# automl/TransformersCanDoBayesianInference

Hardware: AMD Instinct MI355X
Metric: synthetic datasets/sec (GP prior, bptt=2000) (higher is better)
Workload: dtype fp16; 1 GPU; priors.fast_gp, bptt=2000, num_features=18, emsize=512, nhead=4, nhid=1024, nlayers=6, 1000 bars (BASELINE.json configs[1]); per_gpu_batch=64, global_batch=64, aggregate_k_gradients=1, aggregate_streams=0, aggregate_stacked=False, seq_len=2000, parallelism=dp1, micro_batch_streams=2, eval_pos=weighted sampler(2000)

## Files before the change

include/pfn_hip.h:

```cpp
#ifndef PFN_HIP_H
#define PFN_HIP_H

#include <stddef.h>
#include <stdint.h>

#ifdef __cplusplus
extern "C" {
#endif

#define PFN_ABI_VERSION 10

enum {
  PFN_OK = 0,
  PFN_ERR_UNSUPPORTED = -1,
  PFN_ERR_ALIGNMENT = -2,
  PFN_ERR_LAUNCH = -3,
  PFN_ERR_ARGUMENT = -4,
};

enum { PFN_PREC_BF16 = 0,
       PFN_PREC_F32 = 1,
       PFN_PREC_FP16 = 2   };

typedef struct pfn_model_desc {
  int32_t num_features;
  int32_t emsize;
  int32_t nhead;
  int32_t nhid;
  int32_t nlayers;
  int32_t n_out;
  int32_t precision;
  float ln_eps;
  float dropout;
  int32_t schedule;
} pfn_model_desc;
enum { PFN_SCHED_TOP_LAYER_ALL_ROWS = 1,
       PFN_SCHED_FUSE_LN_WIDE = 2,
       PFN_SCHED_SEPARATE_LNBWD = 4,
       PFN_SCHED_NO_KEY_CENTERING = 16,
       PFN_SCHED_KEY_CENTERING = 64,
       PFN_SCHED_F32_RESIDUAL = 128,
       PFN_SCHED_FUSE_Q_PROJECTION = 32,
       PFN_SCHED_DETERMINISTIC = 8        };
int pfn_default_schedule(void);

int pfn_abi_version(void);
const char* pfn_last_error_string(void);
enum { PFN_TUNE_GEMM_NT_KERNEL = 0,
       PFN_TUNE_GEMM_TN_WRAP = 1,
       PFN_TUNE_FUSE_LNBWD = 2,
       PFN_TUNE_ATTN_PINGPONG = 4,
       PFN_TUNE_FUSE_LN_WIDE = 5,
       PFN_TUNE_GP_PLANES = 8,
       PFN_TUNE_FUSE_DELTA = 9,
       PFN_TUNE_GEMM_LN_ROWS = 7,
       PFN_TUNE_ATTN_BWD_GROUP = 10,
       PFN_TUNE_WGRAD_SPLITS = 11,
       PFN_TUNE_WGRAD_WAVES = 14,
       PFN_TUNE_LOSS_SCALE_TARGET = 15,
       PFN_TUNE_RESIDUAL16 = 16,
       PFN_TUNE_FUSE_Q_PROJECTION = 12,
       PFN_TUNE_KEY_CENTERING = 13,
       PFN_TUNE_ATTN_CACHE_SPLITS = 17,
       PFN_TUNE_TOP_LAYER_TEST_ROWS = 6  };
int pfn_set_tuning(int key, int value);
enum { PFN_PROF_ATTN_FWD = 0, PFN_PROF_ATTN_BWD_DELTA = 2, PFN_PROF_ATTN_BWD_KV = 4, PFN_PROF_ATTN_BWD_DQ = 6, PFN_PROF_GEMM_QKV = 8,
       PFN_PROF_GEMM_OUT_LN = 10, PFN_PROF_GEMM_LIN1 = 12, PFN_PROF_GEMM_LIN2_LN = 14, PFN_PROF_GEMM_DHPRE = 16, PFN_PROF_GEMM_DY1 = 18,
       PFN_PROF_GEMM_DCTX = 20, PFN_PROF_GEMM_DX = 22, PFN_PROF_WGRAD = 24, PFN_PROF_SLOTS = 26 };
int pfn_profile_enable(int on);
int pfn_profile_read(int slot, double* total_ms, int64_t* launches);

int pfn_param_layout(const pfn_model_desc* d, int64_t* offsets, int64_t* numels, int max_tensors);
int64_t pfn_param_count(const pfn_model_desc* d);
int64_t pfn_shadow_bytes(const pfn_model_desc* d);
int pfn_prepare_params(const pfn_model_desc* d, const float* params, void* shadow, void* stream);

int64_t pfn_workspace_bytes(const pfn_model_desc* d, int B, int S);
int64_t pfn_top_layer_rows(const pfn_model_desc* d, int B, int S, int sep, int use_dropout);
int pfn_stack_forward(const pfn_model_desc* d, const float* params, const void* shadow,
                      const float* x, int64_t x_st, int64_t x_sb,
                      const float* y, int64_t y_st, int64_t y_sb,
                      const float* src_sbe,
                      int B, int S, int sep,
                      void* workspace, int64_t workspace_bytes,
                      float* logits, void* stream);
int pfn_stack_forward_dropout(const pfn_model_desc* d, const float* params, const void* shadow,
                              const float* x, int64_t x_st, int64_t x_sb,
                              const float* y, int64_t y_st, int64_t y_sb,
                              const float* src_sbe,
                              int B, int S, int sep,
                              void* workspace, int64_t workspace_bytes,
                              float* logits, void* stream, uint64_t dropout_seed);
int pfn_stack_backward(const pfn_model_desc* d, const float* params, const void* shadow,
                       const float* x, int64_t x_st, int64_t x_sb,
                       const float* y, int64_t y_st, int64_t y_sb,
                       int B, int S, int sep,
                       void* workspace, int64_t workspace_bytes,
                       const float* dlogits, float* grads, float* dsrc_sbe, void* stream);
typedef void (*pfn_host_callback)(void* user);
int pfn_stack_backward_split(const pfn_model_desc* d, const float* params, const void* shadow,
                             const float* x, int64_t x_st, int64_t x_sb,
                             const float* y, int64_t y_st, int64_t y_sb,
                             int B, int S, int sep,
                             void* workspace, int64_t workspace_bytes,
                             const float* dlogits, float* grads, float* dsrc_sbe, void* stream,
                             int first_group_layers, pfn_host_callback on_first_group, void* user,
                             int use_dropout, uint64_t dropout_seed);

int pfn_stack_forward_ragged(const pfn_model_desc* d, const float* params, const void* shadow,
                             const float* x, int64_t x_st, int64_t x_sb,
                             const float* y, int64_t y_st, int64_t y_sb,
                             int B, int S, const int32_t* sep_of, const int64_t* row_off, int sep_min, int sep_max, int64_t test_rows,
                             void* workspace, int64_t workspace_bytes, float* logits, void* stream,
                             int use_dropout, uint64_t dropout_seed);
int pfn_stack_backward_ragged(const pfn_model_desc* d, const float* params, const void* shadow,
                              const float* x, int64_t x_st, int64_t x_sb,
                              const float* y, int64_t y_st, int64_t y_sb,
                              int B, int S, const int32_t* sep_of, const int64_t* row_off, int sep_min, int sep_max, int64_t test_rows,
                              void* workspace, int64_t workspace_bytes,
                              const float* dlogits, float* grads, void* stream,
                              int first_group_layers, pfn_host_callback on_first_group, void* user,
                              int use_dropout, uint64_t dropout_seed);

int64_t pfn_context_bytes(const pfn_model_desc* d, int B, int sep);
int pfn_stack_condition(const pfn_model_desc* d, const float* params, const void* shadow,
                        const float* x, int64_t x_st, int64_t x_sb,
                        const float* y, int64_t y_st, int64_t y_sb,
                        int B, int sep,
                        void* workspace, int64_t workspace_bytes,
                        void* context, int64_t context_bytes, void* stream);
int64_t pfn_predict_workspace_bytes(const pfn_model_desc* d, int B, int n);
int pfn_stack_predict(const pfn_model_desc* d, const float* params, const void* shadow,
                      const void* context, int64_t context_bytes, int sep,
                      const float* x, int64_t x_st, int64_t x_sb,
                      int B, int n,
                      void* workspace, int64_t workspace_bytes, float* logits, void* stream);

int64_t pfn_predict_grad_workspace_bytes(const pfn_model_desc* d, int B, int n);
int pfn_stack_predict_saved(const pfn_model_desc* d, const float* params, const void* shadow,
                            const void* context, int64_t context_bytes, int sep,
                            const float* x, int64_t x_st, int64_t x_sb,
                            int B, int n,
                            void* workspace, int64_t workspace_bytes, float* logits, void* stream);
int pfn_stack_predict_backward(const pfn_model_desc* d, const float* params, const void* shadow,
                               const void* context, int64_t context_bytes, int sep, int B, int n,
                               void* workspace, int64_t workspace_bytes, const float* dlogits,
                               float* dx, int64_t dx_st, int64_t dx_sb, void* stream);
int pfn_stack_input_grads(const pfn_model_desc* d, const float* params, int B, int S, int sep,
                          const void* workspace, int64_t workspace_bytes,
                          float* dx, int64_t dx_st, int64_t dx_sb, float* dy, int64_t dy_st, int64_t dy_sb, void* stream);

int pfn_stack_condition_ragged(const pfn_model_desc* d, const float* params, const void* shadow,
                               const float* x, int64_t x_st, int64_t x_sb,
                               const float* y, int64_t y_st, int64_t y_sb,
                               int B, int sep_max, const int32_t* sep_of,
                               void* workspace, int64_t workspace_bytes,
                               void* context, int64_t context_bytes, void* stream);
int pfn_stack_predict_ragged(const pfn_model_desc* d, const float* params, const void* shadow,
                             const void* context, int64_t context_bytes, int sep_max, const int32_t* sep_of,
                             const float* x, int64_t x_st, int64_t x_sb,
                             int B, int n,
                             void* workspace, int64_t workspace_bytes, float* logits, void* stream);
int pfn_stack_predict_saved_ragged(const pfn_model_desc* d, const float* params, const void* shadow,
                                   const void* context, int64_t context_bytes, int sep_max, const int32_t* sep_of,
                                   const float* x, int64_t x_st, int64_t x_sb,
                                   int B, int n,
                                   void* workspace, int64_t workspace_bytes, float* logits, void* stream);
int pfn_stack_predict_backward_ragged(const pfn_model_desc* d, const float* params, const void* shadow,
                                      const void* context, int64_t context_bytes, int sep_max, const int32_t* sep_of, int B, int n,
                                      void* workspace, int64_t workspace_bytes, const float* dlogits,
                                      float* dx, int64_t dx_st, int64_t dx_sb, void* stream);

int pfn_bar_nll_forward(const float* logits, int64_t ld, const float* y, const float* borders,
                        int64_t R, int nbars, int full_support,
                        float* nll, float* lse, int32_t* bucket, void* stream);
int pfn_bar_nll_backward(const float* logits, int64_t ld, const float* lse, const int32_t* bucket,
                         const float* gout, int64_t R, int nbars, float* dlogits, void* stream);
int pfn_bar_mean(const float* logits, int64_t ld, const float* borders, int64_t R, int nbars,
                 int full_support, float* mean, void* stream);
int pfn_bar_mean_backward(const float* logits, int64_t ld, const float* borders, int64_t R, int nbars, int full_support,
                          const float* mean, const float* gout, float* dlogits, void* stream);

#define PFN_BAR_STATS_MAX 16
#define PFN_BAR_STAT_MEAN 0
#define PFN_BAR_STAT_VARIANCE 1
#define PFN_BAR_STAT_MODE 2
#define PFN_BAR_STAT_CDF 3
#define PFN_BAR_STAT_ICDF 4
#define PFN_BAR_STAT_EI_MAX 5
#define PFN_BAR_STAT_EI_MIN 6
int pfn_bar_stats(const float* logits, int64_t ld, const float* borders, int64_t R, int nbars, int full_support,
                  const int32_t* kinds, int K, const float* args, int64_t arg_ld, float* out, void* stream);
int pfn_bar_stats_backward(const float* logits, int64_t ld, const float* borders, int64_t R, int nbars, int full_support,
                           const int32_t* kinds, int K, const float* args, int64_t arg_ld, const float* out, const float* gout,
                           float* dlogits, void* stream);
int pfn_bar_sample(const float* logits, int64_t ld, const float* borders, int64_t R, int nbars, int full_support,
                   int n_samples, uint64_t seed, float* out, void* stream);

int pfn_clip_adam_step(float* params, float* grads, float* exp_avg, float* exp_avg_sq, int64_t n,
                       float lr, float beta1, float beta2, float eps, float max_norm,
                       float grad_scale, int step, int zero_grad, float* scratch, void* stream);

int64_t pfn_gp_workspace_bytes(int B, int S);
int pfn_gp_prior_sample(float* x, float* z, float* y, float* K_ws, int64_t K_ws_bytes,
                        const float* lengthscale, const float* outputscale, const float* noise,
                        int B, int S, int nf, int kernel, int gen_x, int gen_z,
                        uint64_t seed, uint64_t offset, int32_t* info, void* stream);

int pfn_gp_posterior(const float* x, const float* y, float* K_ws, int64_t K_ws_bytes, float* resid_ws, float* w_ws,
                     const float* lengthscale, const float* outputscale, const float* noise,
                     int B, int S, int nf, int kernel, float* nll, float* mean, float* var,
                     int32_t* info, void* stream);

int64_t pfn_gp_fit_workspace_bytes(int P, int S);
int pfn_gp_mll_grad(const float* x, const float* y, const int32_t* n_of, const float* theta, const float* prior,
                    int P, int S, int nf, int kernel, int flags, void* ws, int64_t ws_bytes,
                    float* value, float* grad, int32_t* info, void* stream);
int pfn_gp_fit_predict(const float* x, const float* y, const int32_t* n_of, const float* theta, const float* prior,
                       int P, int S, int nf, int kernel, const float* x_test, int m, void* ws, int64_t ws_bytes,
                       float* mean, float* var, int32_t* info, void* stream);

#define PFN_NUTS_ADAPT_MASS 1
#define PFN_NUTS_KEEP_WARMUP 2
#define PFN_NUTS_MAX_WINDOWS 16
#define PFN_NUTS_INV_MASS_OFFSET 256
int64_t pfn_nuts_workspace_bytes(int C, int D, int max_tree_depth);
int pfn_nuts_init(void* ws, int64_t ws_bytes, int C, int D, int64_t ld, int max_tree_depth, int num_warmup, int num_samples, int flags,
                  const int32_t* window_ends, int n_windows, int window_start, float step_size, float target_accept, uint64_t seed,
                  const int64_t* chain_ids, const float* theta0, const float* inv_mass0, float* trial, int32_t* done_count, void* stream);
int pfn_nuts_advance(void* ws, int64_t ws_bytes, int C, int D, int64_t ld, int max_tree_depth, int num_warmup, int num_samples,
                     const float* value, const float* grad, const int32_t* info, const float* scale, const float* shift, float* trial,
                     float* samples, float* stats, float* warm, int32_t* done_count, void* stream);

int pfn_bnn_logp_grad(const float* x, const float* y, const int32_t* n_of, const float* theta, int64_t ld,
                      int P, int K, int S, int F, int H, int activation,
                      float* value, float* grad, void* stream);
int pfn_bnn_predict(const float* x_test, const float* theta, int64_t ld, int P, int K, int m, int F, int H, int activation,
                    float* prob1, void* stream);

int pfn_bnn_svi_steps(const float* x, const float* y, const int32_t* n_of, float* state, int64_t ld, int P, int S, int F, int H, int activation,
                      int num_particles, int64_t step0, int num_steps, float lr, float beta1, float beta2, float eps, uint64_t seed,
                      const int64_t* problem_ids, float* loss, void* stream);

#define PFN_BNN_SVGD_MAX_PARTICLES 64
int64_t pfn_bnn_svgd_workspace_bytes(int P, int num_particles, int F, int H);
int pfn_bnn_svgd_steps(const float* x, const float* y, const int32_t* n_of, float* state, int64_t ld, int P, int S, int F, int H, int activation,
                       int num_particles, int64_t step0, int num_steps, float lr, float beta1, float beta2, float eps, float bandwidth_factor,
                       void* workspace, int64_t workspace_bytes, float* potential, float* bandwidth, void* stream);

#define PFN_TAB_NORM_WITH_TEST 0
#define PFN_TAB_NORM_TRAIN_ONLY 1
int pfn_tabular_windows(const float* X, const float* y, const int32_t* starts, int64_t N, int F, int F_out, int W, int bptt, int sep, float rescale, int mode,
                        float* x_out, float* y_out, void* stream);
int pfn_auc_counts(const float* scores, const float* labels, int T, int C, int64_t* counts, void* stream);
int pfn_knn_cv(const float* train, const float* labels, const float* test, const int32_t* fold, int P, int n, int T, int F,
               int32_t* cv_correct, int32_t* test_pos, int32_t* test_nbr, void* stream);

int pfn_mlp_prior_forward(const float* weights, const float* biases, const int32_t* model_of, const int32_t* dims,
                          const float* noise_std, float* causes, const float* noise, float* y, float* hidden,
                          int B, int T, int HP, int Lmax, int activation, int gen_causes,
                          uint64_t seed, uint64_t offset, void* stream);

int pfn_op_gemm_nt(const void* A, int64_t lda, const void* B, int64_t ldb, int M, int N, int K,
                   int flags, const float* bias, const void* aux, int64_t ld_aux,
                   const float* resid, int64_t ld_resid, float* out_f32, int64_t ld_out_f32,
                   void* out_t, int64_t ld_out_t, void* out2_t, int64_t ld_out2, int prec, void* stream);
int pfn_op_gemm_tn(const void* A, int64_t lda, const void* B, int64_t ldb, float* C, int64_t ldc,
                   int M, int P, int Q, int atomic, int prec, void* stream);
int pfn_op_gemm_tn_group(int n, const void* const* A, const int64_t* lda, const void* const* B, const int64_t* ldb,
                         float* const* C, const int64_t* ldc, const int32_t* P, const int32_t* Q,
                         float* const* colsum, int M, int splits, int prec, void* stream);
#define PFN_OP_SUMS_16BIT 256
int pfn_op_gemm_ln(const void* A, int64_t lda, const void* B, int64_t ldb, int M, int N, int K, const float* bias,
                   const float* resid, const float* ry, const float* rmean, const float* rrstd,
                   const float* rgamma, const float* rbeta, const float* gamma, const float* beta, float eps,
                   float* y, float* mean, float* rstd, void* x_t, int prec, void* stream);
int pfn_op_gemm_lnbwd(const void* A, int64_t lda, const void* B, int64_t ldb, int M, int N, int K, const void* aux,
                      const float* y, const float* mean, const float* rstd, const float* gamma,
                      void* dx_t, float* dgamma, float* dbeta, int prec, void* stream);
int pfn_op_attention_fwd(const void* qkv, void* ctx, float* lse, int B, int S, int E, int H, int sep,
                         int prec, void* stream);
int64_t pfn_op_attention_bwd_ws_bytes(int B, int S, int H, int prec);
int pfn_op_attention_bwd(const void* qkv, const void* ctx, const float* lse, const void* dctx,
                         void* dqkv, float* delta_ws, void* ds_ws, int B, int S, int E, int H, int sep,
                         int prec, int parts, void* stream);
int pfn_op_attention_fwd_from(const void* qkv, void* ctx, float* lse, int B, int S, int E, int H, int sep, int q_begin,
                              int prec, void* stream);
int pfn_op_attention_bwd_from(const void* qkv, const void* ctx, const float* lse, const void* dctx,
                              void* dqkv, float* delta_ws, void* ds_ws, int B, int S, int E, int H, int sep, int q_begin,
                              int prec, int parts, void* stream);
int pfn_op_gather_rows(const void* src_bs, void* dst_tb, int B, int S, int64_t row_bytes, int sep, void* stream);
int pfn_op_scatter_rows(const void* src_tb, void* dst_bs, int B, int S, int64_t row_bytes, int sep, int zero_from, void* stream);
int pfn_op_layernorm_fwd(const float* x, const float* gamma, const float* beta, float* y_f32, void* y_t,
                         float* mean, float* rstd, int64_t rows, int E, float eps, int prec, void* stream);
int pfn_op_layernorm_bwd(const void* dy, int dy_is_t, const float* x, const float* gamma, const float* mean,
                         const float* rstd, float* dx_f32, void* dx_t, float* dgamma, float* dbeta,
                         float* dbias_extra, int64_t rows, int E, int prec, void* stream);
int pfn_op_cast(const float* src, void* dst, int64_t n, int prec, void* stream);
int pfn_op_qkv_projection(const void* x_t, const void* w_in_t, const float* b_in, void* qkv_t, float* kshift_ws,
                          int B, int S, int E, int sep, const int32_t* sep_of, int center, int prec, void* stream);

#ifdef __cplusplus
}
// ... 3 lines not shown
```

transformerscandobayesianinference_amd/_hip.py:

```python
import ctypes
import os
import subprocess

import torch

_HERE = os.path.dirname(os.path.abspath(__file__))
LIB_PATH = os.path.join(_HERE, 'libpfn_hip.so')
ABI_VERSION = 10

MAX_FEATURES = 1022
PREC_BF16 = 0
PREC_F32 = 1
PREC_FP16 = 2
PRECISIONS = {'bf16': PREC_BF16, 'f32': PREC_F32, 'fp32': PREC_F32, 'fp16': PREC_FP16, 'f16': PREC_FP16}
SCHED_TOP_LAYER_ALL_ROWS, SCHED_FUSE_LN_WIDE, SCHED_SEPARATE_LNBWD, SCHED_DETERMINISTIC, SCHED_NO_KEY_CENTERING, SCHED_FUSE_Q_PROJECTION, SCHED_KEY_CENTERING, SCHED_F32_RESIDUAL = 1, 2, 4, 8, 16, 32, 64, 128
NUTS_ADAPT_MASS, NUTS_KEEP_WARMUP, NUTS_MAX_WINDOWS, NUTS_INV_MASS_OFFSET = 1, 2, 16, 256

EPI_BIAS, EPI_GELU, EPI_GELU_BWD, EPI_RESID, EPI_OUT_F32, EPI_OUT_T, EPI_OUT2_T, EPI_ACCUM, EPI_RESID_T = 1, 2, 4, 8, 16, 32, 64, 128, 256


class HipExtensionError(RuntimeError):
    pass


class ModelDesc(ctypes.Structure):
    _fields_ = [('num_features', ctypes.c_int32), ('emsize', ctypes.c_int32), ('nhead', ctypes.c_int32),
                ('nhid', ctypes.c_int32), ('nlayers', ctypes.c_int32), ('n_out', ctypes.c_int32),
                ('precision', ctypes.c_int32), ('ln_eps', ctypes.c_float), ('dropout', ctypes.c_float), ('schedule', ctypes.c_int32)]

    def key(self):
        return (self.num_features, self.emsize, self.nhead, self.nhid, self.nlayers, self.n_out, self.precision, self.ln_eps, self.dropout, self.schedule)


HOST_CALLBACK = ctypes.CFUNCTYPE(None, ctypes.c_void_p)

_lib = None

_c = ctypes
_P, _I, _L, _F, _U64 = _c.c_void_p, _c.c_int, _c.c_int64, _c.c_float, _c.c_uint64
_D = _c.POINTER(ModelDesc)

SIGNATURES = {
    'pfn_abi_version': (_I, []),
    'pfn_last_error_string': (_c.c_char_p, []),
    'pfn_set_tuning': (_I, [_I, _I]),
    'pfn_default_schedule': (_I, []),
    'pfn_profile_enable': (_I, [_I]),
    'pfn_profile_read': (_I, [_I, _c.POINTER(_c.c_double), _c.POINTER(_L)]),
    'pfn_param_layout': (_I, [_D, _c.POINTER(_L), _c.POINTER(_L), _I]),
    'pfn_param_count': (_L, [_D]),
    'pfn_shadow_bytes': (_L, [_D]),
    'pfn_prepare_params': (_I, [_D, _P, _P, _P]),
    'pfn_workspace_bytes': (_L, [_D, _I, _I]),
    'pfn_top_layer_rows': (_L, [_D, _I, _I, _I, _I]),
    'pfn_stack_forward': (_I, [_D, _P, _P, _P, _L, _L, _P, _L, _L, _P, _I, _I, _I, _P, _L, _P, _P]),
    'pfn_stack_backward': (_I, [_D, _P, _P, _P, _L, _L, _P, _L, _L, _I, _I, _I, _P, _L, _P, _P, _P, _P]),
    'pfn_stack_forward_dropout': (_I, [_D, _P, _P, _P, _L, _L, _P, _L, _L, _P, _I, _I, _I, _P, _L, _P, _P, _U64]),
    'pfn_stack_backward_split': (_I, [_D, _P, _P, _P, _L, _L, _P, _L, _L, _I, _I, _I, _P, _L, _P, _P, _P, _P, _I, _P, _P, _I, _U64]),
    'pfn_stack_forward_ragged': (_I, [_D, _P, _P, _P, _L, _L, _P, _L, _L, _I, _I, _P, _P, _I, _I, _L, _P, _L, _P, _P, _I, _U64]),
    'pfn_stack_backward_ragged': (_I, [_D, _P, _P, _P, _L, _L, _P, _L, _L, _I, _I, _P, _P, _I, _I, _L, _P, _L, _P, _P, _P, _I, _P, _P, _I, _U64]),
    'pfn_context_bytes': (_L, [_D, _I, _I]),
    'pfn_stack_condition': (_I, [_D, _P, _P, _P, _L, _L, _P, _L, _L, _I, _I, _P, _L, _P, _L, _P]),
    'pfn_predict_workspace_bytes': (_L, [_D, _I, _I]),
    'pfn_stack_predict': (_I, [_D, _P, _P, _P, _L, _I, _P, _L, _L, _I, _I, _P, _L, _P, _P]),
    'pfn_predict_grad_workspace_bytes': (_L, [_D, _I, _I]),
    'pfn_stack_predict_saved': (_I, [_D, _P, _P, _P, _L, _I, _P, _L, _L, _I, _I, _P, _L, _P, _P]),
    'pfn_stack_predict_backward': (_I, [_D, _P, _P, _P, _L, _I, _I, _I, _P, _L, _P, _P, _L, _L, _P]),
    'pfn_stack_condition_ragged': (_I, [_D, _P, _P, _P, _L, _L, _P, _L, _L, _I, _I, _P, _P, _L, _P, _L, _P]),
    'pfn_stack_predict_ragged': (_I, [_D, _P, _P, _P, _L, _I, _P, _P, _L, _L, _I, _I, _P, _L, _P, _P]),
    'pfn_stack_predict_saved_ragged': (_I, [_D, _P, _P, _P, _L, _I, _P, _P, _L, _L, _I, _I, _P, _L, _P, _P]),
    'pfn_stack_predict_backward_ragged': (_I, [_D, _P, _P, _P, _L, _I, _P, _I, _I, _P, _L, _P, _P, _L, _L, _P]),
    'pfn_stack_input_grads': (_I, [_D, _P, _I, _I, _I, _P, _L, _P, _L, _L, _P, _L, _L, _P]),
    'pfn_bar_nll_forward': (_I, [_P, _L, _P, _P, _L, _I, _I, _P, _P, _P, _P]),
    'pfn_bar_nll_backward': (_I, [_P, _L, _P, _P, _P, _L, _I, _P, _P]),
    'pfn_bar_mean': (_I, [_P, _L, _P, _L, _I, _I, _P, _P]),
    'pfn_bar_mean_backward': (_I, [_P, _L, _P, _L, _I, _I, _P, _P, _P, _P]),
    'pfn_bar_stats': (_I, [_P, _L, _P, _L, _I, _I, _P, _I, _P, _L, _P, _P]),
    'pfn_bar_stats_backward': (_I, [_P, _L, _P, _L, _I, _I, _P, _I, _P, _L, _P, _P, _P, _P]),
    'pfn_bar_sample': (_I, [_P, _L, _P, _L, _I, _I, _I, _U64, _P, _P]),
    'pfn_clip_adam_step': (_I, [_P, _P, _P, _P, _L, _F, _F, _F, _F, _F, _F, _I, _I, _P, _P]),
    'pfn_gp_workspace_bytes': (_L, [_I, _I]),
    'pfn_gp_prior_sample': (_I, [_P, _P, _P, _P, _L, _P, _P, _P, _I, _I, _I, _I, _I, _I, _U64, _U64, _P, _P]),
    'pfn_gp_posterior': (_I, [_P, _P, _P, _L, _P, _P, _P, _P, _P, _I, _I, _I, _I, _P, _P, _P, _P, _P]),
    'pfn_gp_fit_workspace_bytes': (_L, [_I, _I]),
    'pfn_gp_mll_grad': (_I, [_P, _P, _P, _P, _P, _I, _I, _I, _I, _I, _P, _L, _P, _P, _P, _P]),
    'pfn_gp_fit_predict': (_I, [_P, _P, _P, _P, _P, _I, _I, _I, _I, _P, _I, _P, _L, _P, _P, _P, _P]),
    'pfn_nuts_workspace_bytes': (_L, [_I, _I, _I]),
    'pfn_nuts_init': (_I, [_P, _L, _I, _I, _L, _I, _I, _I, _I, _P, _I, _I, _F, _F, _U64, _P, _P, _P, _P, _P, _P]),
    'pfn_nuts_advance': (_I, [_P, _L, _I, _I, _L, _I, _I, _I, _P, _P, _P, _P, _P, _P, _P, _P, _P, _P, _P]),
    'pfn_bnn_logp_grad': (_I, [_P, _P, _P, _P, _L, _I, _I, _I, _I, _I, _I, _P, _P, _P]),
    'pfn_bnn_predict': (_I, [_P, _P, _L, _I, _I, _I, _I, _I, _I, _P, _P]),
    'pfn_bnn_svi_steps': (_I, [_P, _P, _P, _P, _L, _I, _I, _I, _I, _I, _I, _L, _I, _F, _F, _F, _F, _U64, _P, _P, _P]),
    'pfn_bnn_svgd_workspace_bytes': (_L, [_I, _I, _I, _I]),
    'pfn_bnn_svgd_steps': (_I, [_P, _P, _P, _P, _L, _I, _I, _I, _I, _I, _I, _L, _I, _F, _F, _F, _F, _F, _P, _L, _P, _P, _P]),
    'pfn_tabular_windows': (_I, [_P, _P, _P, _L, _I, _I, _I, _I, _I, _F, _I, _P, _P, _P]),
    'pfn_auc_counts': (_I, [_P, _P, _I, _I, _P, _P]),
    'pfn_knn_cv': (_I, [_P, _P, _P, _P, _I, _I, _I, _I, _P, _P, _P, _P]),
    'pfn_mlp_prior_forward': (_I, [_P, _P, _P, _P, _P, _P, _P, _P, _P, _I, _I, _I, _I, _I, _I, _U64, _U64, _P]),
    'pfn_op_gemm_nt': (_I, [_P, _L, _P, _L, _I, _I, _I, _I, _P, _P, _L, _P, _L, _P, _L, _P, _L, _P, _L, _I, _P]),
    'pfn_op_gemm_tn': (_I, [_P, _L, _P, _L, _P, _L, _I, _I, _I, _I, _I, _P]),
    'pfn_op_gemm_tn_group': (_I, [_I, _P, _P, _P, _P, _P, _P, _P, _P, _P, _I, _I, _I, _P]),
    'pfn_op_gemm_ln': (_I, [_P, _L, _P, _L, _I, _I, _I, _P, _P, _P, _P, _P, _P, _P, _P, _P, _F, _P, _P, _P, _P, _I, _P]),
    'pfn_op_gemm_lnbwd': (_I, [_P, _L, _P, _L, _I, _I, _I, _P, _P, _P, _P, _P, _P, _P, _P, _I, _P]),
    'pfn_op_attention_fwd': (_I, [_P, _P, _P, _I, _I, _I, _I, _I, _I, _P]),
    'pfn_op_attention_bwd_ws_bytes': (_L, [_I, _I, _I, _I]),
    'pfn_op_attention_fwd_from': (_I, [_P, _P, _P, _I, _I, _I, _I, _I, _I, _I, _P]),
    'pfn_op_attention_bwd_from': (_I, [_P, _P, _P, _P, _P, _P, _P, _I, _I, _I, _I, _I, _I, _I, _I, _P]),
    'pfn_op_gather_rows': (_I, [_P, _P, _I, _I, _L, _I, _P]),
    'pfn_op_scatter_rows': (_I, [_P, _P, _I, _I, _L, _I, _I, _P]),
    'pfn_op_attention_bwd': (_I, [_P, _P, _P, _P, _P, _P, _P, _I, _I, _I, _I, _I, _I, _I, _P]),
    'pfn_op_layernorm_fwd': (_I, [_P, _P, _P, _P, _P, _P, _P, _L, _I, _F, _I, _P]),
    'pfn_op_layernorm_bwd': (_I, [_P, _I, _P, _P, _P, _P, _P, _P, _P, _P, _P, _L, _I, _I, _P]),
    'pfn_op_cast': (_I, [_P, _P, _L, _I, _P]),
    'pfn_op_qkv_projection': (_I, [_P, _P, _P, _P, _P, _I, _I, _I, _I, _P, _I, _I, _P]),
}


def build(verbose=False):
    script = os.path.join(_HERE, 'csrc', 'build.sh')
    res = subprocess.run(['bash', script], capture_output=True, text=True)
    if res.returncode != 0 or not os.path.exists(LIB_PATH):
        raise HipExtensionError('building libpfn_hip.so failed:\n' + res.stdout[-4000:] + res.stderr[-8000:])
    if verbose:
        print(res.stdout[-2000:])
    return LIB_PATH


def lib():
    global _lib
    if _lib is None:
        if not os.path.exists(LIB_PATH):
            raise HipExtensionError(
                f'{LIB_PATH} not found. Build it with `python -c "import __graft_entry__ as g; g.build()"` '
                f'(or transformerscandobayesianinference_amd/csrc/build.sh). There is no CPU / PyTorch fallback for the hot path.')
        handle = ctypes.CDLL(LIB_PATH)
        for name, (res, args) in SIGNATURES.items():
            try:
                fn = getattr(handle, name)
            except AttributeError as e:
                raise HipExtensionError(f'libpfn_hip.so does not export {name}') from e
            fn.restype = res
            fn.argtypes = args
        if handle.pfn_abi_version() != ABI_VERSION:
            raise HipExtensionError(f'libpfn_hip.so ABI {handle.pfn_abi_version()} != binding ABI {ABI_VERSION}; rebuild')
        _lib = handle
    return _lib


def check(rc, what):
    if rc < 0:
        msg = lib().pfn_last_error_string()
        raise HipExtensionError(f'{what} failed with code {rc}: {msg.decode() if msg else ""}')
    return rc


def stream_ptr(device=None):
    return torch.cuda.current_stream(device).cuda_stream


def ptr(t):
    return 0 if t is None else t.data_ptr()


def require_gpu_tensor(t, name):
    if not t.is_cuda:
        raise HipExtensionError(
            f'{name} lives on {t.device}: the PFN hot path only runs on an MI355X through libpfn_hip.so; '
            f'move the model and data to a cuda device (there is no CPU fallback in the product path).')
```

transformerscandobayesianinference_amd/csrc/gemm_tn.hip:

```cpp
#include <type_traits>
#include "pfn_device.h"
#include "pfn_kernels.h"

namespace pfn {

PFN_DEV int xcd_remap(int bid, int nwg) {
  const int q = nwg >> 3, r = nwg & 7, xcd = bid & 7;
  return (xcd < r ? xcd * (q + 1) : r * (q + 1) + (xcd - r) * q) + (bid >> 3);
}
typedef __attribute__((address_space(1))) const void gvoid_t;
typedef __attribute__((address_space(3))) void lvoid_t;

constexpr int TN_BMK = 32;

template <typename T>
__global__ __launch_bounds__(256, 2) void gemm_tn_kernel(GemmTN g) {
  constexpr int RB = 128 * sizeof(T);
  constexpr int TILE = TN_BMK * RB;
  extern __shared__ __attribute__((aligned(16))) char smem_raw[];
  LdsPtr smem = lds_cast(smem_raw);
  auto tileA = [&](int buf) { return smem + buf * 2 * TILE; };
  auto tileB = [&](int buf) { return smem + buf * 2 * TILE + TILE; };

  const int p0 = blockIdx.y * 128, q0 = blockIdx.x * 128;
// ... 243 lines not shown
        }
      }
      slot_next = slot;
      slot = slot + 1 == TNB_NS ? 0 : slot + 1;
    }
  };
  if (do_colsum) main_loop(std::true_type{});
  else main_loop(std::false_type{});

  const int pv = pr.Pv > 0 ? pr.Pv : pr.P;
  const float osc = loss_scale_down(g.scale_amax);
  if (do_colsum && (lane & 31) == 0) {
#pragma unroll
    for (int r = 0; r < 16; ++r) {
      const int pp = p0 + wp * 128 + wq * 32 + acc_row(r, lane);
      if (pp < pv) unsafeAtomicAdd(pr.colsum + pp, cs[r] * osc);
    }
  }
  const bool atomic = true;
#pragma unroll
  for (int i = 0; i < 4; ++i)
#pragma unroll
    for (int j = 0; j < 2; ++j)
#pragma unroll
      for (int r = 0; r < 16; ++r) {
        const int pp = p0 + wp * 128 + i * 32 + acc_row(r, lane);
        const int qq = q0 + wq * 64 + j * 32 + (lane & 31);
        float* c = pr.C + (long)pp * pr.ldc + qq;
        if (pp >= pv) continue;
        if (atomic) unsafeAtomicAdd(c, acc[i][j][r] * osc);
        else *c += acc[i][j][r] * osc;
      }
}

#define PFN_TNW_BUILT (PFN_TNB_KT == 64 && PFN_TNB_NS == 2)
#if PFN_TNW_BUILT
constexpr int TNW_NW = 4;
template <typename T>
__global__ __launch_bounds__(TNW_NW * 64, 1) void gemm_tn_wide_kernel(GemmTNGroup g) {
  extern __shared__ __attribute__((aligned(16))) char smem_raw[];
  LdsPtr smem = lds_cast(smem_raw);
  const int ntiles = g.tile_start[g.n];
  const int id = xcd_remap(blockIdx.x, ntiles * g.splits);
  const int split = id / ntiles, tile = id % ntiles;
  int pi = 0;
  while (tile >= g.tile_start[pi + 1]) ++pi;
  const TnProblem& pr = g.p[pi];
  const int tq = pr.Q / 256;
  const int tl = tile - g.tile_start[pi];
  const int p0 = (tl / tq) * 256, q0 = (tl % tq) * 256;
  const long mbeg = (long)split * g.m_chunk;
  const long mend = min((long)g.M, mbeg + g.m_chunk);
  const int rows_total = (int)(mend - mbeg);
  if (rows_total <= 0) return;
  const int wave = __builtin_amdgcn_readfirstlane(threadIdx.x >> 6), lane = threadIdx.x & 63;
  const int wp = wave >> 1, wq = wave & 1;

  TnStager<TNW_NW> stg;
  stg.init(pr, mbeg, rows_total, p0, q0, wave, lane, g.debug_mask);

  f32x16 acc[4][4];
#pragma unroll
  for (int i = 0; i < 4; ++i)
#pragma unroll
    for (int j = 0; j < 4; ++j)
#pragma unroll
      for (int r = 0; r < 16; ++r) acc[i][j][r] = 0.f;
  float cs[2] = {0.f, 0.f};
  const bool do_colsum = pr.colsum != nullptr && q0 == 0;

  const int nt = (rows_total + TNB_KT - 1) / TNB_KT;
  struct Frs { Frag<T> a[4], b[4]; };
  auto main_loop = [&](auto with_colsum) {
    constexpr bool CS = decltype(with_colsum)::value;
    Frs f0, f1;
    auto ld = [&](Frs& f, const lds_char* ta, const lds_char* tb, int ks) {
#pragma unroll
      for (int j = 0; j < 4; ++j) f.b[j] = load_frag_tr<T, 512, 1>(tb, ks, wq * 128 + j * 32);
#pragma unroll
      for (int i = 0; i < 4; ++i) f.a[i] = load_frag_tr<T, 512, 1>(ta, ks, wp * 128 + i * 32);
    };
    auto mm = [&](const Frs& f) {
#pragma unroll
      for (int i = 0; i < 4; ++i)
#pragma unroll
        for (int j = 0; j < 4; ++j) acc[i][j] = mma32(f.a[i], f.b[j], acc[i][j]);
      if constexpr (CS) {
#pragma unroll
        for (int c = 0; c < 2; ++c)
#pragma unroll
          for (int e = 0; e < 8; ++e) cs[c] += (float)(wq ? f.a[2 + c] : f.a[c]).v[e];
      }
    };
    auto enter_stage = [&](int t, int slot) {
      wait_vm_barrier<0>();
      if (t + 1 < nt) stg.issue(smem + (slot ^ 1) * 2 * TNB_TILE);
    };
    int slot = 0;
    enter_stage(0, slot);
    ld(f0, smem, smem + TNB_TILE, 0);
    for (int t = 0; t < nt; ++t) {
      const lds_char* ta = smem + slot * 2 * TNB_TILE;
      const lds_char* tb = ta + TNB_TILE;
      ld(f1, ta, tb, 16);
      PFN_PIN_LDS_MFMA();
      mm(f0);
      PFN_PIN_LDS_MFMA();
      ld(f0, ta, tb, 32);
      PFN_PIN_LDS_MFMA();
      mm(f1);
      PFN_PIN_LDS_MFMA();
      ld(f1, ta, tb, 48);
      PFN_PIN_LDS_MFMA();
      mm(f0);
      PFN_PIN_LDS_MFMA();
      slot ^= 1;
      if (t + 1 < nt) {
        enter_stage(t + 1, slot);
        const lds_char* tan = smem + slot * 2 * TNB_TILE;
        ld(f0, tan, tan + TNB_TILE, 0);
      }
      PFN_PIN_LDS_MFMA();
      mm(f1);
      PFN_PIN_LDS_MFMA();
    }
  };
  stg.issue(smem);
  if (do_colsum) main_loop(std::true_type{});
  else main_loop(std::false_type{});

  const int pv = pr.Pv > 0 ? pr.Pv : pr.P;
  const float osc = loss_scale_down(g.scale_amax);
  if (do_colsum) {
#pragma unroll
    for (int c = 0; c < 2; ++c) {
      const float s = cs[c] + __shfl_xor(cs[c], 32, 64);
      const int pp = p0 + wp * 128 + (2 * wq + c) * 32 + (lane & 31);
      if (lane < 32 && pp < pv) unsafeAtomicAdd(pr.colsum + pp, s * osc);
    }
  }
#pragma unroll
  for (int i = 0; i < 4; ++i)
#pragma unroll
    for (int j = 0; j < 4; ++j)
#pragma unroll
      for (int r = 0; r < 16; ++r) {
        const int pp = p0 + wp * 128 + i * 32 + acc_row(r, lane);
        const int qq = q0 + wq * 128 + j * 32 + (lane & 31);
        if (pp < pv) unsafeAtomicAdd(pr.C + (long)pp * pr.ldc + qq, acc[i][j][r] * osc);
      }
}
#endif

static bool aligned16(const void* p) { return (reinterpret_cast<uintptr_t>(p) & 15) == 0; }

static int g_tn_debug_wrap = 0;
void set_gemm_tn_debug_wrap(int rows) { g_tn_debug_wrap = rows; }
static int g_tn_group_splits = 0;
void set_gemm_tn_group_splits(int splits) { g_tn_group_splits = splits; }
static bool g_tn_wide = false;
void set_gemm_tn_group_waves(int waves) { g_tn_wide = waves == 4; }

int launch_gemm_tn(GemmTN g, int precision, hipStream_t stream) {
  if (g.M <= 0 || g.P <= 0 || g.Q <= 0) return PFN_OK;
  const size_t es = prec_esize(precision);
  if ((g.lda * es) % 16 || (g.ldb * es) % 16 || !aligned16(g.A) || !aligned16(g.B)) return PFN_ERR_ALIGNMENT;
  const int tp = (g.P + 127) / 128, tq = (g.Q + 127) / 128;
  int splits = (1024 + tp * tq - 1) / (tp * tq);
  const int max_splits = (g.M + 4 * TN_BMK - 1) / (4 * TN_BMK);
  if (splits > max_splits) splits = max_splits;
  if (g.max_splits > 0 && splits > g.max_splits) splits = g.max_splits;
  if (splits < 1) splits = 1;
  if (!g.atomic) splits = 1;
  int chunk = (g.M + splits - 1) / splits;
  chunk = (chunk + TN_BMK - 1) / TN_BMK * TN_BMK;
  splits = (g.M + chunk - 1) / chunk;
  g.m_chunk = chunk;
  const size_t lds = 4 * TN_BMK * 128 * es;
  PFN_DISPATCH_OP(precision, hipLaunchKernelGGL(gemm_tn_kernel<T>, dim3(tq, tp, splits), dim3(256), lds, stream, g));
  return hipGetLastError() == hipSuccess ? PFN_OK : PFN_ERR_LAUNCH;
}

bool gemm_tn_group_supported(const TnProblem& p) {
  return p.P % 256 == 0 && p.Q % 256 == 0 && (p.lda * 2) % 16 == 0 && (p.ldb * 2) % 16 == 0 && aligned16(p.A) && aligned16(p.B);
}

int launch_gemm_tn_group(GemmTNGroup g, int precision, hipStream_t stream) {
  if (g.n <= 0 || g.M <= 0) return PFN_OK;
  if (g.n > TN_GROUP_MAX) return PFN_ERR_ARGUMENT;
  if (!prec_is16(precision)) return PFN_ERR_UNSUPPORTED;
  int tiles = 0;
  for (int i = 0; i < g.n; ++i) {
    if (!gemm_tn_group_supported(g.p[i])) return PFN_ERR_UNSUPPORTED;
    g.tile_start[i] = tiles;
    tiles += (g.p[i].P / 256) * (g.p[i].Q / 256);
  }
  g.tile_start[g.n] = tiles;
  int splits = g.splits;
  if (splits <= 0 && g_tn_group_splits > 0) splits = g_tn_group_splits;
  if (splits <= 0) {
    splits = 8;
    for (int sp = 1; sp <= 8; ++sp) {
      const int blocks = tiles * sp, rounds = (blocks + 255) / 256;
      if (blocks >= 0.9 * rounds * 256) { splits = sp; break; }
    }
  }
  const int max_splits = (g.M + 4 * TNB_KT - 1) / (4 * TNB_KT);
  if (splits > max_splits) splits = max_splits;
  int chunk = (g.M + splits - 1) / splits;
  chunk = (chunk + TNB_KT - 1) / TNB_KT * TNB_KT;
  splits = (g.M + chunk - 1) / chunk;
  g.splits = splits;
  g.m_chunk = chunk;
  for (int i = 0; i < g.n; ++i) {
    const TnProblem& p = g.p[i];
    if (p.lda < 256 || p.ldb < 256 || (long)chunk * p.lda * 2 > TN_GROUP_MAX_SPLIT_BYTES || (long)chunk * p.ldb * 2 > TN_GROUP_MAX_SPLIT_BYTES) return PFN_ERR_UNSUPPORTED;
  }
  const int wrap = g_tn_debug_wrap;
  g.debug_mask = wrap >= TNB_KT && (wrap & (wrap - 1)) == 0 ? wrap - 1 : 0x7fffffff;
  if (g_tn_wide) {
#if PFN_TNW_BUILT
    static LdsAllowance allow_w[2];
    if (precision == PFN_PREC_FP16) {
      allow_w[1].ensure(gemm_tn_wide_kernel<f16>, TNB_LDS);
      hipLaunchKernelGGL(gemm_tn_wide_kernel<f16>, dim3(tiles * splits), dim3(TNW_NW * 64), TNB_LDS, stream, g);
    } else {
      allow_w[0].ensure(gemm_tn_wide_kernel<bf16>, TNB_LDS);
      hipLaunchKernelGGL(gemm_tn_wide_kernel<bf16>, dim3(tiles * splits), dim3(TNW_NW * 64), TNB_LDS, stream, g);
    }
    return hipGetLastError() == hipSuccess ? PFN_OK : PFN_ERR_LAUNCH;
#else
    return PFN_ERR_UNSUPPORTED;
#endif
  }
  static LdsAllowance allowance[2];
  if (precision == PFN_PREC_FP16) {
    allowance[1].ensure(gemm_tn_big_kernel<f16>, TNB_LDS);
    hipLaunchKernelGGL(gemm_tn_big_kernel<f16>, dim3(tiles * splits), dim3(512), TNB_LDS, stream, g);
  } else {
    allowance[0].ensure(gemm_tn_big_kernel<bf16>, TNB_LDS);
    hipLaunchKernelGGL(gemm_tn_big_kernel<bf16>, dim3(tiles * splits), dim3(512), TNB_LDS, stream, g);
  }
  return hipGetLastError() == hipSuccess ? PFN_OK : PFN_ERR_LAUNCH;
}

}
```

transformerscandobayesianinference_amd/csrc/pfn_api.hip:

```cpp
#include <algorithm>
#include <cstdarg>
#include <cstdio>
#include <cstring>
#include <mutex>
#include <vector>
#include "pfn_kernels.h"

using namespace pfn;

namespace pfn {
namespace {
struct ProfPair { hipEvent_t a, b; };
std::mutex g_prof_mu;
std::vector<ProfPair> g_prof[PFN_PROF_SLOTS];
std::atomic<int> g_prof_on{0};
}
bool prof_enabled() { return g_prof_on.load(std::memory_order_relaxed) != 0; }
void* prof_begin(int slot, hipStream_t s) {
  const int on = g_prof_on.load(std::memory_order_relaxed);
  if (!on || slot < 0 || slot >= PFN_PROF_SLOTS) return nullptr;
  if (on >= 2 && (slot & ~1) != on - 2) return nullptr;
  ProfPair* p = new ProfPair;
  if (hipEventCreate(&p->a) != hipSuccess || hipEventCreate(&p->b) != hipSuccess) { delete p; return nullptr; }
  (void)hipEventRecord(p->a, s);
// ... 338 lines not shown
    g.x_f32 = last ? u.x2 : nullptr;
    PFN_TRY(launch_gemm_ln(g, prec, s));
    res = Resid{nullptr, u.y2, u.mean2, u.rstd2, params + p.g2, params + p.be2};
  } else {
    {
      GemmNT g = nt(u.h, F, W(m, p.w2), F, rows, E, F, EPI_BIAS | (pdrop > 0.f ? 0 : EPI_RESID) | EPI_OUT_F32);
      g.bias = params + p.b2; g.resid = u.x1; g.ld_resid = E; g.out_f32 = u.y2; g.ld_out_f32 = E;
      if (y16u) { g.flags = EPI_BIAS | EPI_RESID_T | EPI_OUT_T; g.aux = u.x1_t; g.ld_aux = E; g.out_t = u.y2; g.ld_out_t = E; }
      PFN_TRY(launch_gemm_nt(g, prec, s));
      if (pdrop > 0.f) PFN_TRY(launch_dropout_add(u.y2, u.x1, rows, E, seed[3], pdrop, s));
    }
    PFN_TRY(launch_layernorm_fwd(u.y2, params + p.g2, params + p.be2, (y16u && !last) ? nullptr : u.x2, u.x2_t, u.mean2, u.rstd2, rows, E, d.ln_eps, prec, s, y16u));
  }
  return PFN_OK;
}

int decoder_forward(const Model& m, const void* xt_t, char* dt, char* dpre, float* logits, int rows) {
  const int prec = m.d->precision, E = m.d->emsize, F = m.d->nhid, O = m.d->n_out;
  {
    GemmNT g = nt(xt_t, E, W(m, m.L->dec0_w), E, rows, F, E, EPI_BIAS | EPI_GELU | EPI_OUT_T | EPI_OUT2_T);
    g.bias = m.params + m.L->dec0_b; g.out_t = dt; g.ld_out_t = F; g.out2_t = dpre; g.ld_out2 = F;
    PFN_TRY(launch_gemm_nt(g, prec, m.s));
  }
  GemmNT g = nt(dt, F, W(m, m.L->dec2_w), F, rows, O, F, EPI_BIAS | EPI_OUT_F32);
  g.bias = m.params + m.L->dec2_b; g.out_f32 = logits; g.ld_out_f32 = O;
  return launch_gemm_nt(g, prec, m.s);
}
int decoder_backward_data(const Model& m, const void* dlog_t, const void* dpre, char* dd_t, float* dxt, int rows) {
  const int prec = m.d->precision, E = m.d->emsize, F = m.d->nhid, O = m.d->n_out, npad = m.L->n_out_pad;
  {
    GemmNT g = nt(dlog_t, npad, WT(m, m.L->dec2_wt), npad, rows, F, npad % 64 == 0 ? npad : O, EPI_GELU_BWD | EPI_OUT_T);
    g.aux = dpre; g.ld_aux = F; g.out_t = dd_t; g.ld_out_t = F;
    PFN_TRY(launch_gemm_nt(g, prec, m.s));
  }
  GemmNT g = nt(dd_t, F, WT(m, m.L->dec0_wt), F, rows, E, F, EPI_OUT_F32);
  g.out_f32 = dxt; g.ld_out_f32 = E;
  return launch_gemm_nt(g, prec, m.s);
}

bool tn_set_groupable(const std::vector<TnProblem>& probs, int prec) {
  bool grouped = prec_is16(prec);
  for (const TnProblem& t : probs) grouped = grouped && gemm_tn_group_supported(t);
  return grouped;
}
int launch_tn_set(const std::vector<TnProblem>& probs, int rows, int prec, bool det, const float* lsc, int prof_slot, hipStream_t s, bool allow_group = true) {
  auto one_by_one = [&](size_t i0, size_t n) {
    for (size_t i = i0; i < i0 + n; ++i) {
      const TnProblem& t = probs[i];
      GemmTN g = tn(t.A, t.lda, t.B, t.ldb, t.C, t.ldc, rows, t.Pv ? t.Pv : t.P, t.Q, t.colsum);
      if (det) g.max_splits = 1;
      g.scale_amax = lsc;
      PFN_TRY(launch_gemm_tn(g, prec, s));
    }
    return (int)PFN_OK;
  };
  if (!(allow_group && tn_set_groupable(probs, prec))) return one_by_one(0, probs.size());
  for (size_t i0 = 0; i0 < probs.size(); i0 += TN_GROUP_MAX) {
    ProfScope ps(prof_slot, s);
    GemmTNGroup g;
    memset(&g, 0, sizeof(g));
    g.n = (int)std::min<size_t>(TN_GROUP_MAX, probs.size() - i0);
    g.M = rows;
    g.splits = det ? 1 : 0;
    g.scale_amax = lsc;
    for (int i = 0; i < g.n; ++i) g.p[i] = probs[i0 + i];
    const int rc = launch_gemm_tn_group(g, prec, s);
    if (rc == PFN_ERR_UNSUPPORTED) PFN_TRY(one_by_one(i0, g.n));
    else PFN_TRY(rc);
  }
  return PFN_OK;
}

struct LnSinks { float *dgamma, *dbeta, *dbias; };
struct LayerGrads {
  const void* dout; int dout_is_t;
  const void* y2; const float *mean2, *rstd2, *gamma2; const void* y1; const float *mean1, *rstd1, *gamma1; const void* hpre;
  char *dy2_t, *dy2m_t, *dh_t, *dy1_t, *dqkv_t, *dx1_t;
  LnSinks ln2, ln1;
  float* ln_part;
};
GemmLNB lnb(const Model& m, const Plan& pl, const float* lsc, const void* A, long lda, const void* Bw, long ldb, int K, const void* aux, const void* y,
            const float* mean, const float* rstd, const float* gamma, void* dx_t, const LnSinks& sink, int rows) {
  GemmLNB g; memset(&g, 0, sizeof(g));
  g.A = A; g.lda = lda; g.B = Bw; g.ldb = ldb; g.M = rows; g.N = m.d->emsize; g.K = K; g.aux = aux;
  g.y = y; g.mean = mean; g.rstd = rstd; g.gamma = gamma; g.dx_t = dx_t; g.dgamma = sink.dgamma; g.dbeta = sink.dbeta; g.scale_amax = lsc; g.y16 = pl.y16_any;
  return g;
}
GemmLNB lnb_dy1(const Model& m, const Plan& pl, const float* lsc, const LayerP& t, const LayerGrads& g, int rows) {
  const int F = m.d->nhid;
  return lnb(m, pl, lsc, g.dh_t, F, WT(m, t.w1), F, F, g.dy2_t, g.y1, g.mean1, g.rstd1, g.gamma1, g.dy1_t, g.ln1, rows);
}
GemmLNB lnb_dx(const Model& m, const Plan& pl, const float* lsc, const LayerP& t, const char* dqkv_t, const char* dy1_t, const LayerGrads& below, int rows) {
  const int E = m.d->emsize;
  return lnb(m, pl, lsc, dqkv_t, 3 * E, WT(m, t.w_in), 3 * E, 3 * E, dy1_t, below.y2, below.mean2, below.rstd2, below.gamma2, below.dy2_t, below.ln2, rows);
}
bool lnbwd_fusable(const Model& m, const Plan& pl, const float* lsc, const LayerGrads& g0, int rows) {
  const LayerP& t = m.L->layer_t[0];
  return pl.lnb_eligible && gemm_lnbwd_supported(lnb_dy1(m, pl, lsc, t, g0, rows)) && gemm_lnbwd_supported(lnb_dx(m, pl, lsc, t, g0.dqkv_t, g0.dy1_t, g0, rows));
}
int layer_backward_to_dy1(const Model& m, const LayerP& t, const LayerGrads& g, int rows, const Plan& pl, bool fuse_lnb, bool ln2_done, const float* lsc,
                          float pdrop, unsigned seed2, int prof) {
  const int prec = m.d->precision, E = m.d->emsize, F = m.d->nhid;
  hipStream_t s = m.s;
  if (!ln2_done)
    PFN_TRY(launch_layernorm_bwd(g.dout, g.dout_is_t, g.y2, g.gamma2, g.mean2, g.rstd2, nullptr, g.dy2_t, g.ln2.dgamma, g.ln2.dbeta, g.ln2.dbias, rows, E, prec, s,
                                 g.ln_part, lsc, pl.y16_any));
  const char* dy2_op = g.dy2_t;
  if (pdrop > 0.f) { PFN_TRY(launch_dropout_scale(g.dy2_t, g.dy2m_t, nullptr, nullptr, rows, E, seed2, pdrop, prec, s)); dy2_op = g.dy2m_t; }
  {
    ProfScope ps(PFN_PROF_GEMM_DHPRE + prof, s);
    GemmNT gm = nt(dy2_op, E, WT(m, t.w2), E, rows, F, E, EPI_GELU_BWD | EPI_OUT_T);
    gm.aux = g.hpre; gm.ld_aux = F; gm.out_t = g.dh_t; gm.ld_out_t = F;
    PFN_TRY(launch_gemm_nt(gm, prec, s));
  }
  if (fuse_lnb) {
    ProfScope ps(PFN_PROF_GEMM_DY1 + prof, s);
    PFN_TRY(launch_gemm_lnbwd(lnb_dy1(m, pl, lsc, t, g, rows), prec, s));
  } else {
    {
      GemmNT gm = nt(g.dh_t, F, WT(m, t.w1), F, rows, E, F, EPI_RESID_T | EPI_OUT_T);
      gm.aux = g.dy2_t; gm.ld_aux = E; gm.out_t = g.dx1_t; gm.ld_out_t = E;
      PFN_TRY(launch_gemm_nt(gm, prec, s));
    }
    PFN_TRY(launch_layernorm_bwd(g.dx1_t, 1, g.y1, g.gamma1, g.mean1, g.rstd1, nullptr, g.dy1_t, g.ln1.dgamma, g.ln1.dbeta, g.ln1.dbias, rows, E, prec, s,
                                 g.ln_part, lsc, pl.y16_any));
  }
  return PFN_OK;
}
int layer_backward_dx(const Model& m, const LayerP& t, const char* dqkv_t, const char* dy1_t, int rows, const Plan& pl, const float* lsc, const LayerGrads* below,
                      float* gA, char* gA_t, bool out_f32, int prof) {
  const int prec = m.d->precision, E = m.d->emsize;
  if (below) {
    ProfScope ps(PFN_PROF_GEMM_DX + prof, m.s);
    return launch_gemm_lnbwd(lnb_dx(m, pl, lsc, t, dqkv_t, dy1_t, *below, rows), prec, m.s);
  }
  GemmNT g = nt(dqkv_t, 3 * E, WT(m, t.w_in), 3 * E, rows, E, 3 * E, EPI_RESID_T | (out_f32 ? EPI_OUT_F32 : EPI_OUT_T));
  g.aux = dy1_t; g.ld_aux = E; g.out_f32 = gA; g.ld_out_f32 = E; g.out_t = gA_t; g.ld_out_t = E;
  return launch_gemm_nt(g, prec, m.s);
}

}

extern "C" {

static bool g_gp_planes = true;
static bool g_fuse_delta = true;
static int g_default_schedule = 0;
static bool top_layer_on_test_rows(const pfn_model_desc& d, int S, int sep, float pdrop) {
  return !(d.schedule & PFN_SCHED_TOP_LAYER_ALL_ROWS) && d.nlayers > 0 && pdrop == 0.f && d.dropout == 0.f && sep < S && 4L * sep >= S;
}
static bool top_layer_on_test_rows_ragged(const pfn_model_desc& d, int S, const Ragged& rg, float pdrop) {
  return !(d.schedule & PFN_SCHED_TOP_LAYER_ALL_ROWS) && d.nlayers > 0 && pdrop == 0.f && d.dropout == 0.f && rg.test_rows > 0 && 4L * rg.sep_min >= S;
}
int pfn_abi_version(void) { return PFN_ABI_VERSION; }
int pfn_default_schedule(void) { return g_default_schedule; }
int pfn_profile_enable(int on) { g_prof_on.store(on < 0 ? 0 : on); return PFN_OK; }
int pfn_profile_read(int slot, double* total_ms, int64_t* launches) {
  if (slot < 0 || slot >= PFN_PROF_SLOTS) return fail(PFN_ERR_ARGUMENT, "bad profile slot %d", slot);
  std::vector<ProfPair> pairs;
  {
    std::lock_guard<std::mutex> lock(g_prof_mu);
    pairs.swap(g_prof[slot]);
  }
  double ms = 0.0;
  for (ProfPair& p : pairs) {
    float t = 0.f;
    if (hipEventSynchronize(p.b) == hipSuccess && hipEventElapsedTime(&t, p.a, p.b) == hipSuccess) ms += t;
    (void)hipEventDestroy(p.a);
    (void)hipEventDestroy(p.b);
  }
  if (total_ms) *total_ms = ms;
  if (launches) *launches = (int64_t)pairs.size();
  return PFN_OK;
}
int pfn_set_tuning(int key, int value) {
  switch (key) {
    case PFN_TUNE_GEMM_NT_KERNEL: set_gemm_nt_big_mode(value); return PFN_OK;
    case PFN_TUNE_GEMM_TN_WRAP: set_gemm_tn_debug_wrap(value); return PFN_OK;
    case PFN_TUNE_FUSE_LNBWD: g_default_schedule = value ? (g_default_schedule & ~PFN_SCHED_SEPARATE_LNBWD) : (g_default_schedule | PFN_SCHED_SEPARATE_LNBWD); return PFN_OK;
    case PFN_TUNE_ATTN_PINGPONG: set_attn_pingpong(value); return PFN_OK;
    case PFN_TUNE_ATTN_BWD_GROUP: set_attn_bwd_group(value); return PFN_OK;
    case PFN_TUNE_WGRAD_SPLITS: set_gemm_tn_group_splits(value); return PFN_OK;
    case PFN_TUNE_WGRAD_WAVES: set_gemm_tn_group_waves(value); return PFN_OK;
    case PFN_TUNE_LOSS_SCALE_TARGET: return set_loss_scale_target(value);
    case PFN_TUNE_RESIDUAL16: g_default_schedule = value ? (g_default_schedule & ~PFN_SCHED_F32_RESIDUAL) : (g_default_schedule | PFN_SCHED_F32_RESIDUAL); return PFN_OK;
    case PFN_TUNE_FUSE_Q_PROJECTION: g_default_schedule = value ? (g_default_schedule | PFN_SCHED_FUSE_Q_PROJECTION) : (g_default_schedule & ~PFN_SCHED_FUSE_Q_PROJECTION); return PFN_OK;
    case PFN_TUNE_KEY_CENTERING:
      g_default_schedule &= ~(PFN_SCHED_NO_KEY_CENTERING | PFN_SCHED_KEY_CENTERING);
      if (value > 0) g_default_schedule |= PFN_SCHED_KEY_CENTERING; else if (value == 0) g_default_schedule |= PFN_SCHED_NO_KEY_CENTERING;
      return PFN_OK;
    case PFN_TUNE_GEMM_LN_ROWS: set_gemm_ln_rows64(value); return PFN_OK;
    case PFN_TUNE_GP_PLANES: g_gp_planes = value != 0; return PFN_OK;
    case PFN_TUNE_FUSE_DELTA: g_fuse_delta = value != 0; return PFN_OK;
    case PFN_TUNE_ATTN_CACHE_SPLITS: set_attn_cache_split_cap(value); return PFN_OK;
    case PFN_TUNE_FUSE_LN_WIDE: g_default_schedule = value ? (g_default_schedule | PFN_SCHED_FUSE_LN_WIDE) : (g_default_schedule & ~PFN_SCHED_FUSE_LN_WIDE); return PFN_OK;
    case PFN_TUNE_TOP_LAYER_TEST_ROWS: g_default_schedule = value ? (g_default_schedule & ~PFN_SCHED_TOP_LAYER_ALL_ROWS) : (g_default_schedule | PFN_SCHED_TOP_LAYER_ALL_ROWS); return PFN_OK;
    default: return fail(PFN_ERR_ARGUMENT, "unknown tuning key %d", key);
  }
}
const char* pfn_last_error_string(void) { return g_err; }

int pfn_param_layout(const pfn_model_desc* d, int64_t* offsets, int64_t* numels, int max_tensors) {
  int rc = check_desc(d);
  if (rc != PFN_OK) return rc;
  Layout L = make_layout(*d);
  const int n = (int)L.offsets.size();
  if (offsets || numels) {
    if (max_tensors < n) return fail(PFN_ERR_ARGUMENT, "need room for %d tensors, got %d", n, max_tensors);
    for (int i = 0; i < n; ++i) { if (offsets) offsets[i] = L.offsets[i]; if (numels) numels[i] = L.numels[i]; }
  }
  return n;
}
int64_t pfn_param_count(const pfn_model_desc* d) {
  if (check_desc(d) != PFN_OK) return -1;
  return make_layout(*d).total;
}
int64_t pfn_shadow_bytes(const pfn_model_desc* d) {
  if (check_desc(d) != PFN_OK) return -1;
  Layout L = make_layout(*d);
  return (L.total + L.total_t) * esize(d->precision);
}
int64_t pfn_workspace_bytes(const pfn_model_desc* d, int B, int S) {
  if (check_desc(d) != PFN_OK || B < 1 || S < 1) return -1;
  return carve(*d, B, S, nullptr).bytes;
}

int64_t pfn_top_layer_rows(const pfn_model_desc* d, int B, int S, int sep, int use_dropout) {
  if (check_desc(d) != PFN_OK || B < 1 || S < 1 || sep < 0 || sep > S) return -1;
  return top_layer_on_test_rows(*d, S, sep, use_dropout ? d->dropout : 0.f) ? (int64_t)(S - sep) * B : (int64_t)B * S;
}

int pfn_prepare_params(const pfn_model_desc* d, const float* params, void* shadow, void* stream) {
  PFN_TRY(check_desc(d));
  if (!params || !shadow) return fail(PFN_ERR_ARGUMENT, "null pointer");
  hipStream_t s = (hipStream_t)stream;
  Layout L = make_layout(*d);
  const int prec = d->precision, es = esize(prec);
  const int E = d->emsize, F = d->nhid;
  char* sh = (char*)shadow;
  PFN_TRY(launch_cast_params(params, sh, L.total, prec, s));
  char* tr = sh + L.total * es;
  TransposeGroup g;
  auto add = [&](long src_off, long dst_off, int rows, int cols, int ld_dst) -> int {
    if (g.n == TRANSPOSE_GROUP_MAX) {
      PFN_TRY(launch_transpose_cast_group(params, tr, g, prec, s));
      g = TransposeGroup();
    }
    transpose_group_add(g, src_off, dst_off, rows, cols, ld_dst);
    return PFN_OK;
  };
  for (int l = 0; l < d->nlayers; ++l) {
    const LayerP &p = L.layer[l], &t = L.layer_t[l];
    PFN_TRY(add(p.w_in, t.w_in, 3 * E, E, 3 * E));
    PFN_TRY(add(p.w_o, t.w_o, E, E, E));
    PFN_TRY(add(p.w1, t.w1, F, E, F));
    PFN_TRY(add(p.w2, t.w2, E, F, E));
  }
  if (d->n_out > 0) {
    PFN_TRY(add(L.dec0_w, L.dec0_wt, F, E, F));
    PFN_TRY(add(L.dec2_w, L.dec2_wt, d->n_out, F, L.n_out_pad));
  }
  return launch_transpose_cast_group(params, tr, g, prec, s);
}

static int stack_forward_impl(const pfn_model_desc* d, const float* params, const void* shadow,
                              const float* x, int64_t x_st, int64_t x_sb, const float* y, int64_t y_st, int64_t y_sb,
                              const float* src_sbe, int B, int S, int sep, void* workspace, int64_t workspace_bytes,
                              float* logits, void* stream, bool use_dropout, uint64_t dropout_seed, const Ragged* rg = nullptr, const KvSink* sink = nullptr);
int pfn_stack_forward(const pfn_model_desc* d, const float* params, const void* shadow,
                      const float* x, int64_t x_st, int64_t x_sb, const float* y, int64_t y_st, int64_t y_sb,
                      const float* src_sbe, int B, int S, int sep, void* workspace, int64_t workspace_bytes,
                      float* logits, void* stream) {
  return stack_forward_impl(d, params, shadow, x, x_st, x_sb, y, y_st, y_sb, src_sbe, B, S, sep, workspace, workspace_bytes, logits, stream, false, 0);
}
int pfn_stack_forward_dropout(const pfn_model_desc* d, const float* params, const void* shadow,
                              const float* x, int64_t x_st, int64_t x_sb, const float* y, int64_t y_st, int64_t y_sb,
                              const float* src_sbe, int B, int S, int sep, void* workspace, int64_t workspace_bytes,
                              float* logits, void* stream, uint64_t dropout_seed) {
  return stack_forward_impl(d, params, shadow, x, x_st, x_sb, y, y_st, y_sb, src_sbe, B, S, sep, workspace, workspace_bytes, logits, stream, true, dropout_seed);
}
static int stack_forward_impl(const pfn_model_desc* d, const float* params, const void* shadow,
                              const float* x, int64_t x_st, int64_t x_sb, const float* y, int64_t y_st, int64_t y_sb,
                              const float* src_sbe, int B, int S, int sep, void* workspace, int64_t workspace_bytes,
                              float* logits, void* stream, bool use_dropout, uint64_t dropout_seed, const Ragged* rg, const KvSink* sink) {
  PFN_TRY(check_desc(d));
  const float pdrop = use_dropout ? d->dropout : 0.f;
  auto dseed = [&](int layer, int site) { return dropout_site_seed(dropout_seed, layer, site); };
  if (!params || !shadow || !workspace) return fail(PFN_ERR_ARGUMENT, "null pointer");
  if (!src_sbe && (!x || !y)) return fail(PFN_ERR_ARGUMENT, "need x and y (or src_sbe)");
  if (B < 1 || S < 1 || sep < 0 || sep > S) return fail(PFN_ERR_ARGUMENT, "bad B=%d S=%d sep=%d", B, S, sep);
  if (!logits && sep < S) return fail(PFN_ERR_ARGUMENT, "null logits");
  hipStream_t s = (hipStream_t)stream;
  const int prec = d->precision, es = esize(prec);
  const int E = d->emsize, H = d->nhead, O = d->n_out;
  Layout L = make_layout(*d);
  Ws w = carve(*d, B, S, (char*)workspace);
  if (workspace_bytes < w.bytes) return fail(PFN_ERR_ARGUMENT, "workspace too small: %lld < %lld", (long long)workspace_bytes, (long long)w.bytes);
  const int* sep_of = rg ? rg->sep_of : nullptr;
  if (rg && (src_sbe || rg->test_rows < 0 || rg->test_rows > (int64_t)B * S || !rg->sep_of || (!rg->row_off && !(sink && rg->test_rows == 0))))
    return fail(PFN_ERR_ARGUMENT, "bad ragged-batch arguments");
  const int M = B * S, Mt = rg ? (int)rg->test_rows : (S - sep) * B;
  const char* sh = (const char*)shadow;

  if (src_sbe) {
    PFN_TRY(launch_sbe_to_bse(src_sbe, w.x0, w.x0_t, S, B, E, prec, s));
  } else {
    EmbedArgs e;
    e.x = x; e.x_st = x_st; e.x_sb = x_sb; e.y = y; e.y_st = y_st; e.y_sb = y_sb;
    e.wx = params + L.enc_w; e.bx = params + L.enc_b; e.wy = params + L.yenc_w; e.by = params + L.yenc_b;
    e.out_f32 = w.x0; e.out_t = w.x0_t; e.S = S; e.B = B; e.nf = d->num_features; e.E = E; e.sep = sep; e.sep_of = sep_of;
    e.xaug_ld = emb_aug_width(d->num_features);
    e.xaug_t = e.xaug_ld > 0 ? w.xaug_t : nullptr;
    e.xaug_amax = nullptr;
    if (e.xaug_t && prec == PFN_PREC_FP16) {
      PFN_TRY(launch_embed_colmax(e, w.xaug_amax, s));
      e.xaug_amax = w.xaug_amax;
    }
    PFN_TRY(launch_embed_fwd(e, prec, s));
  }
  const float* xin = w.x0;
  const char* xin_t = w.x0_t;
  const Model m = {d, params, sh, &L, s};
  const Plan pl = make_plan(*d, w.x0, w.x0_t, params, sh, M, pdrop);
  Resid res = {w.x0, nullptr, nullptr, nullptr, nullptr, nullptr};
  const bool top_mode = rg ? top_layer_on_test_rows_ragged(*d, S, *rg, pdrop) : top_layer_on_test_rows(*d, S, sep, pdrop);
  const bool fuse_q = (d->schedule & PFN_SCHED_FUSE_Q_PROJECTION) && pdrop == 0.f && attn_fwd_can_fuse_q(E, H, prec);
  auto gather_top = [&](const void* src, void* dst, long row_bytes) {
    return rg ? launch_gather_rows_ragged(src, dst, S, B, row_bytes, rg->sep_of, (const long*)rg->row_off, s) : launch_gather_rows(src, dst, S, B, row_bytes, sep, s);
  };
  for (int l = 0; l < d->nlayers; ++l) {
    const LayerP& p = L.layer[l];
    LayerWs& a = w.layer[l];
    const bool top = top_mode && l == d->nlayers - 1;
    const int Ml = top ? Mt : M;
    {
      ProfScope ps(PFN_PROF_GEMM_QKV, s);
      GemmNT g = nt(xin_t, E, W(m, p.w_in), E, M, 3 * E, E, EPI_BIAS | EPI_OUT_T);
      g.bias = params + p.b_in; g.out_t = a.qkv; g.ld_out_t = 3 * E;
      if (fuse_q) {
        g.B = W(m, p.w_in + (int64_t)E * E); g.N = 2 * E; g.bias = params + p.b_in + E; g.out_t = a.qkv + (int64_t)E * es;
      }
      if (w.kshift && E % 64 == 0) {
        PFN_TRY(launch_key_shift(xin_t, W(m, p.w_in + (int64_t)E * E), w.kshift, B, S, E, sep, sep_of, prec, s));
        g.flags |= EPI_ROWSHIFT; g.rowshift = w.kshift; g.rs_ld = E; g.rs_S = S; g.rs_n0 = fuse_q ? 0 : E; g.rs_n1 = g.rs_n0 + E;
      }
      PFN_TRY(launch_gemm_nt(g, prec, s));
// ... 218 lines not shown
int pfn_stack_predict_backward(const pfn_model_desc* d, const float* params, const void* shadow, const void* context, int64_t context_bytes, int sep, int B, int n,
                               void* workspace, int64_t workspace_bytes, const float* dlogits, float* dx, int64_t dx_st, int64_t dx_sb, void* stream) {
  return stack_predict_backward_impl(d, params, shadow, context, context_bytes, sep, nullptr, B, n, workspace, workspace_bytes, dlogits, dx, dx_st, dx_sb, stream);
}
int pfn_stack_predict_backward_ragged(const pfn_model_desc* d, const float* params, const void* shadow, const void* context, int64_t context_bytes, int sep_max,
                                      const int32_t* sep_of, int B, int n, void* workspace, int64_t workspace_bytes, const float* dlogits, float* dx, int64_t dx_st,
                                      int64_t dx_sb, void* stream) {
  if (!sep_of) return fail(PFN_ERR_ARGUMENT, "null sep_of");
  return stack_predict_backward_impl(d, params, shadow, context, context_bytes, sep_max, sep_of, B, n, workspace, workspace_bytes, dlogits, dx, dx_st, dx_sb, stream);
}
static int stack_predict_backward_impl(const pfn_model_desc* d, const float* params, const void* shadow, const void* context, int64_t context_bytes, int sep,
                                       const int32_t* sep_of, int B, int n, void* workspace, int64_t workspace_bytes, const float* dlogits, float* dx, int64_t dx_st,
                                       int64_t dx_sb, void* stream) {
  PFN_TRY(check_desc(d));
  if (B < 1 || n < 0 || sep < 0) return fail(PFN_ERR_ARGUMENT, "bad B=%d n=%d sep=%d", B, n, sep);
  Context c;
  PFN_TRY(check_context(*d, B, sep, context, context_bytes, &c));
  if (!params || !shadow || !workspace || (n > 0 && (!dlogits || !dx))) return fail(PFN_ERR_ARGUMENT, "null pointer");
  PredictGradWs w = carve_predict_grad(*d, B, n, (char*)workspace);
  if (workspace_bytes < w.bytes) return fail(PFN_ERR_ARGUMENT, "workspace too small: %lld < %lld", (long long)workspace_bytes, (long long)w.bytes);
  if (n == 0) return PFN_OK;
  hipStream_t s = (hipStream_t)stream;
  const int prec = d->precision;
  const int E = d->emsize, H = d->nhead, O = d->n_out, M = B * n;
  Layout L = make_layout(*d);
  const Model m = {d, params, (const char*)shadow, &L, s};
  const Plan pl = make_plan(*d, w.x0, w.x0_t, params, shadow, M, 0.f);
  const LnSinks sink = {w.sink, w.sink + E, w.sink + 2 * E};
  const float* lsc = nullptr;
  if (prec == PFN_PREC_FP16) {
    PFN_TRY(launch_absmax(dlogits, (long)M * (O > 0 ? O : E), w.lscale, s));
    lsc = w.lscale;
  }
  const float* dxt = dlogits;
  if (O == 0) {
    if (lsc) { PFN_TRY(launch_scale_copy(dlogits, w.dxt, (long)M * E, lsc, s)); dxt = w.dxt; }
  } else {
    PFN_TRY(launch_cast_rows(dlogits, O, w.dlog_t, L.n_out_pad, M, O, prec, s, lsc));
    PFN_TRY(decoder_backward_data(m, w.dlog_t, w.dpre, w.dd_t, w.dxt, M));
    dxt = w.dxt;
  }
  PFN_TRY(launch_scatter_test_rows(dxt, w.gA, n, B, E, 0, PFN_PREC_F32, s));
  auto view = [&](int l) {
    const LayerP& p = L.layer[l];
    const PredictLayerWs& a = w.layer[l];
    const bool top = l == d->nlayers - 1;
    return LayerGrads{top ? (const void*)w.gA : (const void*)w.gA_t, top ? 0 : 1, a.y2, a.mean2, a.rstd2, params + p.g2, a.y1, a.mean1, a.rstd1, params + p.g1, a.hpre,
                      w.dy2_t, nullptr, w.dh_t, w.dy1_t, w.dqkv_t, w.gA_t, sink, sink, nullptr};
  };
  const bool fuse_lnb = d->nlayers > 0 && lnbwd_fusable(m, pl, lsc, view(0), M);
  const bool from_t = predict_dsrc_is_t(*d);
  for (int l = d->nlayers - 1; l >= 0; --l) {
    const LayerP& t = L.layer_t[l];
    const PredictLayerWs& a = w.layer[l];
    const char* kv = (const char*)context + l * c.layer_bytes;
    PFN_TRY(layer_backward_to_dy1(m, t, view(l), M, pl, fuse_lnb, fuse_lnb && l < d->nlayers - 1, lsc, 0.f, 0, NO_PROF));
    {
      GemmNT g = nt(w.dy1_t, E, WT(m, t.w_o), E, M, E, E, EPI_OUT_T);
      g.out_t = w.dctx_t; g.ld_out_t = E;
      PFN_TRY(launch_gemm_nt(g, prec, s));
    }
    {
      AttnCacheBwdArgs at; memset(&at, 0, sizeof(at));
      at.qkv = a.qkv; at.ctx = a.ctx; at.lse = a.lse; at.dctx = w.dctx_t; at.dqkv = w.dqkv_t;
      at.kv = kv; at.kv_ld = 2L * E; at.kv_sb = (long)sep * 2 * E; at.part_dq = w.part_o;
      at.B = B; at.S = n; at.E = E; at.H = H; at.sep = sep; at.sep_of = sep_of;
      PFN_TRY(launch_attn_bwd_cache(at, prec, s));
    }
    const LayerGrads below = l > 0 ? view(l - 1) : LayerGrads{};
    PFN_TRY(layer_backward_dx(m, t, w.dqkv_t, w.dy1_t, M, pl, lsc, fuse_lnb && l > 0 ? &below : nullptr, w.gA, w.gA_t, l == 0 && !from_t, NO_PROF));
  }
  EmbedInGradArgs e; memset(&e, 0, sizeof(e));
  e.dsrc = from_t ? (const void*)w.gA_t : (const void*)w.gA; e.dsrc_prec = from_t ? prec : PFN_PREC_F32;
  e.wx = params + L.enc_w; e.wy = params + L.yenc_w; e.dx = dx; e.dx_st = dx_st; e.dx_sb = dx_sb; e.dy = nullptr;
  e.S = n; e.B = B; e.nf = d->num_features; e.E = E; e.sep = 0; e.scale_amax = lsc;
  return launch_embed_input_grad(e, s);
}

int pfn_stack_backward_ragged(const pfn_model_desc* d, const float* params, const void* shadow,
                              const float* x, int64_t x_st, int64_t x_sb, const float* y, int64_t y_st, int64_t y_sb,
                              int B, int S, const int32_t* sep_of, const int64_t* row_off, int sep_min, int sep_max, int64_t test_rows,
                              void* workspace, int64_t workspace_bytes, const float* dlogits, float* grads, void* stream,
                              int first_group_layers, pfn_host_callback on_first_group, void* user, int use_dropout, uint64_t dropout_seed) {
  if (sep_min < 0 || sep_min > sep_max) return fail(PFN_ERR_ARGUMENT, "bad sep_min=%d sep_max=%d", sep_min, sep_max);
  Ragged rg = {sep_of, row_off, test_rows, sep_min};
  return stack_backward_impl(d, params, shadow, x, x_st, x_sb, y, y_st, y_sb, B, S, sep_max, workspace, workspace_bytes, dlogits, grads, nullptr, stream,
                             first_group_layers, on_first_group, user, use_dropout, dropout_seed, &rg);
}
static int stack_backward_impl(const pfn_model_desc* d, const float* params, const void* shadow,
                               const float* x, int64_t x_st, int64_t x_sb, const float* y, int64_t y_st, int64_t y_sb,
                               int B, int S, int sep, void* workspace, int64_t workspace_bytes,
                               const float* dlogits, float* grads, float* dsrc_sbe, void* stream,
                               int first_group_layers, pfn_host_callback on_first_group, void* user, int use_dropout, uint64_t dropout_seed, const Ragged* rg) {
  PFN_TRY(check_desc(d));
  const float pdrop = use_dropout ? d->dropout : 0.f;
  const bool top_mode = rg ? top_layer_on_test_rows_ragged(*d, S, *rg, pdrop) : top_layer_on_test_rows(*d, S, sep, pdrop);
  const int* sep_of = rg ? rg->sep_of : nullptr;
  if (rg && (dsrc_sbe || rg->test_rows < 0 || rg->test_rows > (int64_t)B * S || !rg->sep_of || !rg->row_off)) return fail(PFN_ERR_ARGUMENT, "bad ragged-batch arguments");
  const bool det = (d->schedule & PFN_SCHED_DETERMINISTIC) != 0;
  const float* lsc = nullptr;
  auto dseed = [&](int layer, int site) { return dropout_site_seed(dropout_seed, layer, site); };
  if (!params || !shadow || !workspace || !grads) return fail(PFN_ERR_ARGUMENT, "null pointer");
  if (!dsrc_sbe && (!x || !y)) return fail(PFN_ERR_ARGUMENT, "need x and y (or dsrc_sbe)");
  if (B < 1 || S < 1 || sep < 0 || sep > S) return fail(PFN_ERR_ARGUMENT, "bad B=%d S=%d sep=%d", B, S, sep);
  hipStream_t s = (hipStream_t)stream;
  const int prec = d->precision, es = esize(prec);
  const int E = d->emsize, F = d->nhid, H = d->nhead, O = d->n_out;
  Layout L = make_layout(*d);
  Ws w = carve(*d, B, S, (char*)workspace);
  if (workspace_bytes < w.bytes) return fail(PFN_ERR_ARGUMENT, "workspace too small");
  const int M = B * S, Mt = rg ? (int)rg->test_rows : (S - sep) * B, npad = L.n_out_pad;
  const char* sh = (const char*)shadow;
  const Model m = {d, params, sh, &L, s};
  const Plan pl = make_plan(*d, w.x0, w.x0_t, params, sh, M, pdrop);

  if (prec == PFN_PREC_FP16 && Mt > 0) {
    if (!dlogits) return fail(PFN_ERR_ARGUMENT, "null dlogits");
    PFN_TRY(launch_absmax(dlogits, (long)Mt * (O > 0 ? O : E), w.lscale, s));
    lsc = w.lscale;
  }
  const float* dxt = w.dxt;
  const char* xt_t = top_mode ? w.layer[d->nlayers - 1].x2_t : w.xt_t;
  if (Mt > 0 && O == 0) {
    if (!dlogits) return fail(PFN_ERR_ARGUMENT, "null dlogits");
    dxt = dlogits;
    if (lsc) { PFN_TRY(launch_scale_copy(dlogits, w.dxt, (long)Mt * E, lsc, s)); dxt = w.dxt; }
  } else if (Mt > 0) {
    if (!dlogits) return fail(PFN_ERR_ARGUMENT, "null dlogits");
    PFN_TRY(launch_cast_rows(dlogits, O, w.dlog_t, npad, Mt, O, prec, s, lsc));
    TnProblem dp2; memset(&dp2, 0, sizeof(dp2));
    dp2.A = w.dlog_t; dp2.lda = npad; dp2.B = w.dt; dp2.ldb = F; dp2.C = grads + L.dec2_w; dp2.ldc = F; dp2.P = npad; dp2.Q = F; dp2.Pv = O;
    dp2.colsum = grads + L.dec2_b;
    TnProblem dp0; memset(&dp0, 0, sizeof(dp0));
    dp0.A = w.dd_t; dp0.lda = F; dp0.B = xt_t; dp0.ldb = E; dp0.C = grads + L.dec0_w; dp0.ldc = E; dp0.P = F; dp0.Q = E; dp0.colsum = grads + L.dec0_b;
    const std::vector<TnProblem> dec = {dp2, dp0};
    const bool dec_grouped = tn_set_groupable(dec, prec);
    if (!dec_grouped) PFN_TRY(launch_tn_set({dp2}, Mt, prec, det, lsc, NO_PROF, s, false));
    PFN_TRY(decoder_backward_data(m, w.dlog_t, w.dpre, w.dd_t, w.dxt, Mt));
    PFN_TRY(launch_tn_set(dec_grouped ? dec : std::vector<TnProblem>{dp0}, Mt, prec, det, lsc, NO_PROF, s, dec_grouped));
  }
  if (top_mode) {}
  else if (rg) PFN_TRY(launch_scatter_test_rows_ragged(dxt, d->nlayers > 0 ? (void*)w.gA_t : (void*)w.gA, S, B, E, rg->sep_of, (const long*)rg->row_off, d->nlayers > 0 ? prec : PFN_PREC_F32, s));
  else PFN_TRY(launch_scatter_test_rows(dxt, d->nlayers > 0 ? (void*)w.gA_t : (void*)w.gA, S, B, E, sep, d->nlayers > 0 ? prec : PFN_PREC_F32, s));

  auto view = [&](int l, bool compact) {
    const LayerP& p = L.layer[l];
    LayerWs& a = w.layer[l];
    float *db2 = pdrop > 0.f ? nullptr : grads + p.b2, *dbo = pdrop > 0.f ? nullptr : grads + p.b_o;
    return LayerGrads{compact ? (const void*)dxt : (const void*)w.gA_t, compact ? 0 : 1, a.y2, a.mean2, a.rstd2, params + p.g2, a.y1, a.mean1, a.rstd1, params + p.g1, a.hpre,
                      a.dy2_t, a.dy2m_t, a.dh_t, compact ? w.top_dy1_t : a.dy1_t, a.dqkv_t, w.gA_t,
                      LnSinks{grads + p.g2, grads + p.be2, db2}, LnSinks{grads + p.g1, grads + p.be1, dbo}, w.ln_part};
  };
  const bool emb_t = emb_gemm(*d, dsrc_sbe != nullptr);
  const bool fuse_lnb = d->nlayers > 0 && lnbwd_fusable(m, pl, lsc, view(0, false), M);
  auto launch_weight_gradients = [&](int l_hi, int l_lo) -> int {
    std::vector<TnProblem> probs, probs_top;
    auto add = [&](const void* A, long lda, const void* Bm, long ldb, float* C, long ldc, int P, int Q, float* colsum, bool compact = false) {
      TnProblem t; memset(&t, 0, sizeof(t)); t.A = A; t.lda = lda; t.B = Bm; t.ldb = ldb; t.C = C; t.ldc = ldc; t.P = P; t.Q = Q; t.colsum = colsum;
      (compact ? probs_top : probs).push_back(t);
    };
    for (int l = l_hi; l >= l_lo; --l) {
      const LayerP& p = L.layer[l];
      LayerWs& a = w.layer[l];
      const char* xin_t = (l == 0) ? w.x0_t : w.layer[l - 1].x2_t;
      const bool drop = pdrop > 0.f;
      const bool top = top_mode && l == d->nlayers - 1;
      add(drop ? a.dy2m_t : a.dy2_t, E, a.h, F, grads + p.w2, F, E, F, (drop || (fuse_lnb && l < d->nlayers - 1)) ? grads + p.b2 : nullptr, top);
      add(a.dh_t, F, a.x1_t, E, grads + p.w1, E, F, E, grads + p.b1, top);
      add(drop ? a.dy1m_t : (top ? w.top_dy1_t : a.dy1_t), E, top ? w.top_ctx_t : a.ctx, E, grads + p.w_o, E, E, E, (drop || fuse_lnb) ? grads + p.b_o : nullptr, top);
      add(a.dqkv_t, 3 * E, xin_t, E, grads + p.w_in, E, 3 * E, E, grads + p.b_in);
    }
    PFN_TRY(launch_tn_set(probs_top, Mt, prec, det, lsc, PFN_PROF_WGRAD + 1, s));
    PFN_TRY(launch_tn_set(probs, M, prec, det, lsc, PFN_PROF_WGRAD, s));
    return PFN_OK;
  };
  const int split_at = (on_first_group && first_group_layers > 0 && first_group_layers < d->nlayers) ? d->nlayers - first_group_layers : -1;
  bool delta_zeroed = false;
  for (int l = d->nlayers - 1; l >= 0; --l) {
    const LayerP& t = L.layer_t[l];
    LayerWs& a = w.layer[l];
    const bool top = top_mode && l == d->nlayers - 1;
    const int Ml = top ? Mt : M;
    char* dy1_t = top ? w.top_dy1_t : a.dy1_t;
    PFN_TRY(layer_backward_to_dy1(m, t, view(l, top), Ml, pl, fuse_lnb, fuse_lnb && l < d->nlayers - 1, lsc, pdrop, dseed(l, 3), top ? 1 : 0));
    const char* dy1_op = dy1_t;
    bool delta_fused = false;
    if (pdrop > 0.f) { PFN_TRY(launch_dropout_scale(a.dy1_t, a.dy1m_t, nullptr, nullptr, M, E, dseed(l, 1), pdrop, prec, s)); dy1_op = a.dy1m_t; }
    {
      ProfScope ps(PFN_PROF_GEMM_DCTX + (top ? 1 : 0), s);
      GemmNT g = nt(dy1_op, E, WT(m, t.w_o), E, Ml, E, E, EPI_OUT_T);
      g.out_t = top ? w.top_dctx_t : w.dctx_t; g.ld_out_t = E;
      if (!top && !det && g_fuse_delta) {
        GemmNT gd = g;
        gd.flags |= EPI_ROWDOT; gd.aux = a.ctx; gd.ld_aux = E;
        gd.rowdot = w.delta; gd.rd_lse = a.lse; gd.rd_lse2_off = (long)B * H * S; gd.rd_S = S; gd.rd_H = H; gd.rd_D = E / H;
        if (gemm_nt_rowdot_fused(gd, prec)) {
          if (!delta_zeroed && hipMemsetAsync(w.delta, 0, sizeof(float) * B * H * S, s) != hipSuccess) return fail(PFN_ERR_LAUNCH, "hipMemsetAsync(delta)");
          delta_zeroed = true;
          g = gd; delta_fused = true;
        }
      }
      PFN_TRY(launch_gemm_nt(g, prec, s));
    }
    if (top) {
      if (rg) {
        PFN_TRY(launch_scatter_rows_ragged(w.top_dctx_t, w.dctx_t, S, B, (long)E * es, rg->sep_of, (const long*)rg->row_off, 1, s));
        PFN_TRY(launch_scatter_rows_ragged(w.top_dy1_t, a.dy1_t, S, B, (long)E * es, rg->sep_of, (const long*)rg->row_off, 0, s));
      } else {
        PFN_TRY(launch_scatter_rows(w.top_dctx_t, w.dctx_t, S, B, (long)E * es, sep, sep / 256 * 256, s));
        PFN_TRY(launch_scatter_rows(w.top_dy1_t, a.dy1_t, S, B, (long)E * es, sep, 0, s));
      }
    }
    {
      AttnArgs at; memset(&at, 0, sizeof(at));
      at.qkv = a.qkv; at.ctx = a.ctx; at.lse = a.lse; at.B = B; at.S = S; at.E = E; at.H = H; at.sep = sep; at.sep_of = sep_of;
      at.dctx = w.dctx_t; at.dqkv = a.dqkv_t; at.delta = w.delta; at.ds = w.ds;
      at.p_drop = pdrop; at.drop_seed = dseed(l, 0);
      at.q_begin = top ? (rg ? rg->sep_min : sep) : 0;
      at.q_from_sep = (top && rg) ? 1 : 0;
      if (delta_fused) at.parts = ATTN_BWD_KV | ATTN_BWD_DQ;
      at.zero_delta = delta_zeroed ? 1 : 0;
      PFN_TRY(launch_attn_bwd(at, prec, s));
    }
    const LayerGrads below = l > 0 ? view(l - 1, false) : LayerGrads{};
    PFN_TRY(layer_backward_dx(m, t, a.dqkv_t, a.dy1_t, M, pl, lsc, fuse_lnb && l > 0 ? &below : nullptr, w.gA, w.gA_t, l == 0 && !emb_t, 0));
    if (l == split_at) {
      PFN_TRY(launch_weight_gradients(d->nlayers - 1, split_at));
      on_first_group(user);
    }
  }
  if (d->nlayers > 0) PFN_TRY(launch_weight_gradients(split_at >= 0 ? split_at - 1 : d->nlayers - 1, 0));
  const int aug = emb_aug_width(d->num_features);
  if (dsrc_sbe) {
    PFN_TRY(launch_bse_to_sbe(w.gA, dsrc_sbe, S, B, E, s, lsc));
  } else if (emb_t) {
    if (hipMemsetAsync(w.embacc, 0, sizeof(float) * E * aug, s) != hipSuccess) return fail(PFN_ERR_LAUNCH, "memset");
    GemmTN g = tn(w.gA_t, E, w.xaug_t, aug, w.embacc, aug, M, E, aug, grads + L.enc_b);
    g.scale_amax = lsc;
    g.max_splits = det ? 1 : 128;
    PFN_TRY(launch_gemm_tn(g, prec, s));
    PFN_TRY(launch_embed_grad_scatter(w.embacc, grads + L.enc_w, grads + L.yenc_w, grads + L.yenc_b, E, d->num_features, prec == PFN_PREC_FP16 ? w.xaug_amax : nullptr, s));
  } else {
    EmbedBwdArgs e;
    e.dsrc = w.gA; e.x = x; e.x_st = x_st; e.x_sb = x_sb; e.y = y; e.y_st = y_st; e.y_sb = y_sb;
    e.dwx = grads + L.enc_w; e.dbx = grads + L.enc_b; e.dwy = grads + L.yenc_w; e.dby = grads + L.yenc_b;
    e.S = S; e.B = B; e.nf = d->num_features; e.E = E; e.sep = sep; e.sep_of = sep_of; e.single_block = det ? 1 : 0; e.scale_amax = lsc;
    PFN_TRY(launch_embed_bwd(e, s));
  }
  return PFN_OK;
}

int pfn_stack_input_grads(const pfn_model_desc* d, const float* params, int B, int S, int sep, const void* workspace, int64_t workspace_bytes,
                          float* dx, int64_t dx_st, int64_t dx_sb, float* dy, int64_t dy_st, int64_t dy_sb, void* stream) {
  PFN_TRY(check_desc(d));
  if (B < 1 || S < 1 || sep < 0 || sep > S) return fail(PFN_ERR_ARGUMENT, "bad B=%d S=%d sep=%d", B, S, sep);
  if (!params || !workspace || !dx) return fail(PFN_ERR_ARGUMENT, "null pointer");
  Ws w = carve(*d, B, S, (char*)workspace);
  if (workspace_bytes < w.bytes) return fail(PFN_ERR_ARGUMENT, "workspace too small: %lld < %lld", (long long)workspace_bytes, (long long)w.bytes);
  const int prec = d->precision, E = d->emsize;
  const Layout L = make_layout(*d);
  hipStream_t s = (hipStream_t)stream;
  const bool emb_t = emb_gemm(*d, false);
  EmbedInGradArgs e; memset(&e, 0, sizeof(e));
  e.dsrc = emb_t ? (const void*)w.gA_t : (const void*)w.gA; e.dsrc_prec = emb_t ? prec : PFN_PREC_F32;
  e.wx = params + L.enc_w; e.wy = params + L.yenc_w;
  e.dx = dx; e.dx_st = dx_st; e.dx_sb = dx_sb; e.dy = dy; e.dy_st = dy_st; e.dy_sb = dy_sb;
  e.S = S; e.B = B; e.nf = d->num_features; e.E = E; e.sep = sep;
  e.scale_amax = (prec == PFN_PREC_FP16 && sep < S) ? w.lscale : nullptr;
  return launch_embed_input_grad(e, s);
}

int pfn_bar_mean_backward(const float* logits, int64_t ld, const float* borders, int64_t R, int nbars, int full_support, const float* mean, const float* gout,
                          float* dlogits, void* stream) {
  if (R < 0 || nbars < 1 || (R > 0 && (!logits || !borders || !mean || !gout || !dlogits))) return fail(PFN_ERR_ARGUMENT, "bad bar_mean_backward arguments");
  BarArgs a; memset(&a, 0, sizeof(a));
  a.logits = logits; a.ld = ld; a.borders = borders; a.R = R; a.nbars = nbars; a.full_support = full_support;
  a.mean_out = const_cast<float*>(mean); a.gout = gout; a.dlogits = dlogits;
  PFN_TRY(launch_bar_mean_bwd(a, (hipStream_t)stream));
  return PFN_OK;
}

int pfn_bar_nll_forward(const float* logits, int64_t ld, const float* y, const float* borders, int64_t R, int nbars,
                        int full_support, float* nll, float* lse, int32_t* bucket, void* stream) {
  if (R < 0 || nbars < 1 || (R > 0 && (!logits || !y || !borders || !nll || !lse || !bucket))) return fail(PFN_ERR_ARGUMENT, "bad bar_nll_forward arguments");
  BarArgs a; memset(&a, 0, sizeof(a));
  a.logits = logits; a.ld = ld; a.y = y; a.borders = borders; a.R = R; a.nbars = nbars; a.full_support = full_support;
  a.nll = nll; a.lse = lse; a.bucket = bucket;
  PFN_TRY(launch_bar_nll_fwd(a, (hipStream_t)stream));
  return PFN_OK;
}
int pfn_bar_nll_backward(const float* logits, int64_t ld, const float* lse, const int32_t* bucket, const float* gout,
                         int64_t R, int nbars, float* dlogits, void* stream) {
  if (R < 0 || nbars < 1 || (R > 0 && (!logits || !lse || !bucket || !gout || !dlogits))) return fail(PFN_ERR_ARGUMENT, "bad bar_nll_backward arguments");
  BarArgs a; memset(&a, 0, sizeof(a));
  a.logits = logits; a.ld = ld; a.R = R; a.nbars = nbars; a.lse = const_cast<float*>(lse); a.bucket = const_cast<int*>(bucket);
  a.gout = gout; a.dlogits = dlogits;
  PFN_TRY(launch_bar_nll_bwd(a, (hipStream_t)stream));
  return PFN_OK;
}
int pfn_bar_mean(const float* logits, int64_t ld, const float* borders, int64_t R, int nbars, int full_support, float* mean, void* stream) {
  if (R < 0 || nbars < 1 || (R > 0 && (!logits || !borders || !mean))) return fail(PFN_ERR_ARGUMENT, "bad bar_mean arguments");
  BarArgs a; memset(&a, 0, sizeof(a));
  a.logits = logits; a.ld = ld; a.borders = borders; a.R = R; a.nbars = nbars; a.full_support = full_support; a.mean_out = mean;
  PFN_TRY(launch_bar_mean(a, (hipStream_t)stream));
  return PFN_OK;
}

static int bar_stats_common(BarStatsArgs& a, const char* what, const float* logits, int64_t ld, const float* borders, int64_t R, int nbars, int full_support) {
  if (R < 0) return fail(PFN_ERR_ARGUMENT, "%s: R = %lld", what, (long long)R);
  if (nbars < 1 || (full_support && nbars < 2)) return fail(PFN_ERR_ARGUMENT, "%s: nbars = %d%s", what, nbars, full_support ? " (full support needs two buckets)" : "");
  if (ld < nbars) return fail(PFN_ERR_ARGUMENT, "%s: ld %lld < nbars %d", what, (long long)ld, nbars);
  if (!logits || !borders) return fail(PFN_ERR_ARGUMENT, "%s: null pointer", what);
  memset(&a, 0, sizeof(a));
  a.logits = logits; a.ld = ld; a.borders = borders; a.R = R; a.nbars = nbars; a.full_support = full_support ? 1 : 0;
  return PFN_OK;
}
static int bar_stats_spec(BarStatsArgs& a, const char* what, const int32_t* kinds, int K, const float* args, int64_t arg_ld) {
  if (K < 1 || K > PFN_BAR_STATS_MAX) return fail(PFN_ERR_ARGUMENT, "%s: K = %d outside 1 .. %d", what, K, PFN_BAR_STATS_MAX);
  if (!kinds || !args) return fail(PFN_ERR_ARGUMENT, "%s: null pointer", what);
  if (arg_ld != 0 && arg_ld < K) return fail(PFN_ERR_ARGUMENT, "%s: arg_ld %lld < K %d", what, (long long)arg_ld, K);
  for (int k = 0; k < K; ++k) {
    if (kinds[k] < PFN_BAR_STAT_MEAN || kinds[k] > PFN_BAR_STAT_EI_MIN) return fail(PFN_ERR_ARGUMENT, "%s: unknown statistic %d at position %d", what, (int)kinds[k], k);
    a.kinds[k] = kinds[k];
    a.has_var |= kinds[k] == PFN_BAR_STAT_VARIANCE; a.has_icdf |= kinds[k] == PFN_BAR_STAT_ICDF;
  }
  a.K = K; a.args = args; a.arg_ld = arg_ld;
  return PFN_OK;
}
int pfn_bar_stats(const float* logits, int64_t ld, const float* borders, int64_t R, int nbars, int full_support,
                  const int32_t* kinds, int K, const float* args, int64_t arg_ld, float* out, void* stream) {
  BarStatsArgs a;
  PFN_TRY(bar_stats_common(a, "pfn_bar_stats", logits, ld, borders, R, nbars, full_support));
  PFN_TRY(bar_stats_spec(a, "pfn_bar_stats", kinds, K, args, arg_ld));
  if (!out) return fail(PFN_ERR_ARGUMENT, "pfn_bar_stats: null pointer");
  a.out = out;
  PFN_TRY(launch_bar_stats(a, (hipStream_t)stream));
  return PFN_OK;
}
int pfn_bar_stats_backward(const float* logits, int64_t ld, const float* borders, int64_t R, int nbars, int full_support,
                           const int32_t* kinds, int K, const float* args, int64_t arg_ld, const float* out, const float* gout,
                           float* dlogits, void* stream) {
  BarStatsArgs a;
  PFN_TRY(bar_stats_common(a, "pfn_bar_stats_backward", logits, ld, borders, R, nbars, full_support));
  PFN_TRY(bar_stats_spec(a, "pfn_bar_stats_backward", kinds, K, args, arg_ld));
  if (!out || !gout || !dlogits) return fail(PFN_ERR_ARGUMENT, "pfn_bar_stats_backward: null pointer");
  a.out = const_cast<float*>(out); a.gout = gout; a.dlogits = dlogits;
  PFN_TRY(launch_bar_stats_bwd(a, (hipStream_t)stream));
  return PFN_OK;
}
int pfn_bar_sample(const float* logits, int64_t ld, const float* borders, int64_t R, int nbars, int full_support,
                   int n_samples, uint64_t seed, float* out, void* stream) {
  BarStatsArgs a;
  PFN_TRY(bar_stats_common(a, "pfn_bar_sample", logits, ld, borders, R, nbars, full_support));
  if (n_samples < 0) return fail(PFN_ERR_ARGUMENT, "pfn_bar_sample: n_samples = %d", n_samples);
  if (!out) return fail(PFN_ERR_ARGUMENT, "pfn_bar_sample: null pointer");
  a.n_samples = n_samples; a.seed = seed; a.samples = out;
  PFN_TRY(launch_bar_sample(a, (hipStream_t)stream));
  return PFN_OK;
}

int pfn_clip_adam_step(float* params, float* grads, float* exp_avg, float* exp_avg_sq, int64_t n, float lr, float beta1,
                       float beta2, float eps, float max_norm, float grad_scale, int step, int zero_grad, float* scratch, void* stream) {
  if (!params || !grads || !exp_avg || !exp_avg_sq || !scratch || n < 0 || step < 1) return fail(PFN_ERR_ARGUMENT, "bad clip_adam arguments");
  AdamArgs a;
  a.p = params; a.g = grads; a.m = exp_avg; a.v = exp_avg_sq; a.n = n; a.lr = lr; a.beta1 = beta1; a.beta2 = beta2; a.eps = eps;
  a.max_norm = max_norm; a.grad_scale = grad_scale; a.step = step; a.zero_grad = zero_grad; a.scratch = scratch;
  PFN_TRY(launch_clip_adam(a, (hipStream_t)stream));
  return PFN_OK;
}

int64_t pfn_gp_workspace_bytes(int B, int S) {
  if (B < 1 || S < 1) return -1;
  return gp_workspace_bytes(B, S);
}
static int gp_check_workspace(GpArgs& a, int64_t K_ws_bytes) {
  a.planes = nullptr; a.plane_rows = 0;
  if (K_ws_bytes < (int64_t)a.B * a.S * a.S * 4) return fail(PFN_ERR_ARGUMENT, "K_ws_bytes %lld < B*S*S*4 = %lld", (long long)K_ws_bytes, (long long)a.B * a.S * a.S * 4);
  if (g_gp_planes && K_ws_bytes >= gp_workspace_bytes(a.B, a.S)) gp_attach_planes(a);
  return PFN_OK;
}
int pfn_gp_prior_sample(float* x, float* z, float* y, float* K_ws, int64_t K_ws_bytes, const float* lengthscale, const float* outputscale,
                        const float* noise, int B, int S, int nf, int kernel, int gen_x, int gen_z, uint64_t seed, uint64_t offset,
                        int32_t* info, void* stream) {
  if (!x || !z || !y || !K_ws || !lengthscale || !outputscale || !noise || !info || B < 1 || S < 1 || nf < 1) return fail(PFN_ERR_ARGUMENT, "bad gp_prior_sample arguments");
  if (kernel < 0 || kernel > 3) return fail(PFN_ERR_UNSUPPORTED, "kernel %d (0 = RBF, 1 / 2 / 3 = Matern nu 5/2, 3/2, 1/2)", kernel);
  GpArgs a;
  a.x = x; a.z = z; a.y = y; a.K = K_ws; a.lengthscale = lengthscale; a.outputscale = outputscale; a.noise = noise;
  a.B = B; a.S = S; a.nf = nf; a.kernel = kernel; a.seed = seed; a.offset = offset; a.gen_x = gen_x; a.gen_z = gen_z; a.info = info;
  a.w = nullptr;
  if (int rc = gp_check_workspace(a, K_ws_bytes)) return rc;
  PFN_TRY(launch_gp_sample(a, (hipStream_t)stream));
  return PFN_OK;
}

int pfn_gp_posterior(const float* x, const float* y, float* K_ws, int64_t K_ws_bytes, float* resid_ws, float* w_ws, const float* lengthscale,
                     const float* outputscale, const float* noise, int B, int S, int nf, int kernel, float* nll, float* mean,
                     float* var, int32_t* info, void* stream) {
  if (!x || !y || !K_ws || !resid_ws || !w_ws || !lengthscale || !outputscale || !noise || !info || B < 1 || S < 1 || nf < 1)
    return fail(PFN_ERR_ARGUMENT, "bad gp_posterior arguments");
  if (kernel < 0 || kernel > 3) return fail(PFN_ERR_UNSUPPORTED, "kernel %d (0 = RBF, 1 / 2 / 3 = Matern nu 5/2, 3/2, 1/2)", kernel);
  GpArgs a;
  a.x = const_cast<float*>(x); a.z = nullptr; a.y = resid_ws; a.K = K_ws; a.lengthscale = lengthscale; a.outputscale = outputscale;
  a.noise = noise; a.B = B; a.S = S; a.nf = nf; a.kernel = kernel; a.seed = 0; a.offset = 0; a.gen_x = 0; a.gen_z = 0; a.info = info;
  a.w = w_ws;
  if (int rc = gp_check_workspace(a, K_ws_bytes)) return rc;
  PFN_TRY(launch_gp_posterior(a, y, nll, mean, var, (hipStream_t)stream));
  return PFN_OK;
}

int64_t pfn_gp_fit_workspace_bytes(int P, int S) {
  if (P < 1 || S < 1) return -1;
  return gp_fit_workspace_bytes(P, S);
}
static int gp_fit_check(const float* x, const float* y, const float* theta, const float* prior, int P, int S, int nf, int kernel, void* ws, int64_t ws_bytes, int32_t* info) {
  if (!x || !y || !theta || !prior || !ws || !info || P < 1 || S < 1 || nf < 1) return fail(PFN_ERR_ARGUMENT, "bad gp_fit arguments");
  if (P > 65535) return fail(PFN_ERR_UNSUPPORTED, "P %d > 65535 problems per call", P);
  if (S % 4) return fail(PFN_ERR_UNSUPPORTED, "S %d is not a multiple of 4", S);
  if (nf > 126) return fail(PFN_ERR_UNSUPPORTED, "nf %d > 126 (the tiles stage 128 rows of x in 64 KB of LDS)", nf);
  if (kernel < 0 || kernel > 3) return fail(PFN_ERR_UNSUPPORTED, "kernel %d (0 = RBF, 1 / 2 / 3 = Matern nu 5/2, 3/2, 1/2)", kernel);
  if (ws_bytes < gp_fit_workspace_bytes(P, S)) return fail(PFN_ERR_ARGUMENT, "ws_bytes %lld < pfn_gp_fit_workspace_bytes = %lld", (long long)ws_bytes, (long long)gp_fit_workspace_bytes(P, S));
  return PFN_OK;
}
// ... 54 lines not shown
  a.trial = trial; a.samples = samples; a.stats = stats; a.warm = warm; a.done_count = done_count;
  PFN_TRY(launch_nuts_advance(a, (hipStream_t)stream));
  return PFN_OK;
}

static int bnn_limits(int F, int H, int activation) {
  if (F < 1 || F > 16) return fail(PFN_ERR_UNSUPPORTED, "F %d outside 1 .. 16 (a lane keeps its row of W1 in registers)", F);
  if (H < 1 || H > 64) return fail(PFN_ERR_UNSUPPORTED, "H %d outside 1 .. 64 (lane = hidden unit, one wave per chain at most)", H);
  if (activation < 0 || activation > 1) return fail(PFN_ERR_UNSUPPORTED, "activation %d (0 identity, 1 tanh)", activation);
  return PFN_OK;
}
static int bnn_batch(int P, int K, int F, int H, int64_t ld) {
  if (P < 1 || K < 1 || (int64_t)P * K > 0x7fffffff) return fail(PFN_ERR_ARGUMENT, "P %d x K %d chains: need P >= 1, K >= 1, P K < 2^31", P, K);
  if (ld < (int64_t)H * (F + 3) + 2) return fail(PFN_ERR_ARGUMENT, "ld %lld < D = H (F + 3) + 2 = %d", (long long)ld, H * (F + 3) + 2);
  return PFN_OK;
}
static int bnn_check(int P, int K, int F, int H, int activation, int64_t ld) {
  if (int rc = bnn_limits(F, H, activation)) return rc;
  return bnn_batch(P, K, F, H, ld);
}
static int bnn_steps_check(const char* fn, int P, int S, int F, int H, int64_t ld, int64_t step0, int num_steps, const void* x, const void* y, const void* state, float lr,
                           float beta1, float beta2, float eps) {
  if (P < 1 || S < 1 || step0 < 0 || num_steps < 0 || !x || !y || !state)
    return fail(PFN_ERR_ARGUMENT, "bad %s arguments (P %d >= 1, S %d >= 1, step0 %lld >= 0, num_steps %d >= 0, x, y, state not NULL)", fn, P, S, (long long)step0, num_steps);
  if (int rc = bnn_batch(P, 1, F, H, ld)) return rc;
  if (!(lr >= 0.f) || !(beta1 >= 0.f && beta1 < 1.f) || !(beta2 >= 0.f && beta2 < 1.f) || !(eps >= 0.f))
    return fail(PFN_ERR_ARGUMENT, "bad %s arguments (lr %g >= 0, beta1 %g and beta2 %g in [0, 1), eps %g >= 0)", fn, lr, beta1, beta2, eps);
  return PFN_OK;
}
int pfn_bnn_logp_grad(const float* x, const float* y, const int32_t* n_of, const float* theta, int64_t ld, int P, int K, int S, int F, int H, int activation,
                      float* value, float* grad, void* stream) {
  if (int rc = bnn_check(P, K, F, H, activation, ld)) return rc;
  if (S < 1 || !x || !y || !theta || !value) return fail(PFN_ERR_ARGUMENT, "bad bnn_logp_grad arguments (S %d >= 1, x, y, theta, value not NULL)", S);
  BnnArgs a{};
  a.x = x; a.y = y; a.n_of = n_of; a.theta = theta; a.ld = ld; a.P = P; a.K = K; a.S = S; a.F = F; a.H = H; a.activation = activation; a.value = value; a.grad = grad;
  PFN_TRY(launch_bnn_logp_grad(a, (hipStream_t)stream));
  return PFN_OK;
}
int pfn_bnn_predict(const float* x_test, const float* theta, int64_t ld, int P, int K, int m, int F, int H, int activation, float* prob1, void* stream) {
  if (int rc = bnn_check(P, K, F, H, activation, ld)) return rc;
  if (m < 0 || !theta || (m > 0 && (!x_test || !prob1))) return fail(PFN_ERR_ARGUMENT, "bad bnn_predict arguments (m %d >= 0, x_test, theta, prob1 not NULL)", m);
  if (m == 0) return PFN_OK;
  BnnArgs a{};
  a.theta = theta; a.ld = ld; a.P = P; a.K = K; a.F = F; a.H = H; a.activation = activation; a.x_test = x_test; a.m = m; a.prob1 = prob1;
  PFN_TRY(launch_bnn_predict(a, (hipStream_t)stream));
  return PFN_OK;
}

int pfn_bnn_svi_steps(const float* x, const float* y, const int32_t* n_of, float* state, int64_t ld, int P, int S, int F, int H, int activation, int num_particles,
                      int64_t step0, int num_steps, float lr, float beta1, float beta2, float eps, uint64_t seed, const int64_t* problem_ids, float* loss, void* stream) {
  if (int rc = bnn_limits(F, H, activation)) return rc;
  if (int rc = bnn_steps_check("bnn_svi_steps", P, S, F, H, ld, step0, num_steps, x, y, state, lr, beta1, beta2, eps)) return rc;
  if (num_particles < 1) return fail(PFN_ERR_ARGUMENT, "bad bnn_svi_steps arguments (num_particles %d >= 1)", num_particles);
  if (step0 > (int64_t)1 << 40 || (step0 + num_steps + 1) * (int64_t)num_particles >= (int64_t)1 << 53)
    return fail(PFN_ERR_ARGUMENT, "step0 %lld must not exceed 2^40 and (step0 + num_steps + 1) num_particles must stay below 2^53 (the Philox counter of a particle's noise)", (long long)step0);
  if (num_steps == 0) return PFN_OK;
  BnnSviArgs a{};
  a.x = x; a.y = y; a.n_of = n_of; a.state = state; a.ld = ld; a.P = P; a.S = S; a.F = F; a.H = H; a.activation = activation; a.K = num_particles; a.step0 = step0;
  a.num_steps = num_steps; a.lr = lr; a.beta1 = beta1; a.beta2 = beta2; a.eps = eps; a.seed = seed; a.problem_ids = problem_ids; a.loss = loss;
  PFN_TRY(launch_bnn_svi_steps(a, (hipStream_t)stream));
  return PFN_OK;
}

static int bnn_svgd_limits(int F, int H, int activation, int N) {
  if (int rc = bnn_limits(F, H, activation)) return rc;
  if (N < 2 || N > PFN_BNN_SVGD_MAX_PARTICLES)
    return fail(PFN_ERR_UNSUPPORTED, "num_particles %d outside 2 .. %d (lane = particle in the Stein step; the median needs a pair)", N, PFN_BNN_SVGD_MAX_PARTICLES);
  return PFN_OK;
}
int64_t pfn_bnn_svgd_workspace_bytes(int P, int num_particles, int F, int H) {
  if (P < 1 || bnn_svgd_limits(F, H, 0, num_particles)) return -1;
  return bnn_svgd_workspace_bytes(P, num_particles, H * (F + 3) + 2);
}
int pfn_bnn_svgd_steps(const float* x, const float* y, const int32_t* n_of, float* state, int64_t ld, int P, int S, int F, int H, int activation, int num_particles,
                       int64_t step0, int num_steps, float lr, float beta1, float beta2, float eps, float bandwidth_factor, void* workspace,
                       int64_t workspace_bytes, float* potential, float* bandwidth, void* stream) {
  if (int rc = bnn_svgd_limits(F, H, activation, num_particles)) return rc;
  if (int rc = bnn_steps_check("bnn_svgd_steps", P, S, F, H, ld, step0, num_steps, x, y, state, lr, beta1, beta2, eps)) return rc;
  if (!(lr <= 3.4e38f) || !(bandwidth_factor > 0.f)) return fail(PFN_ERR_ARGUMENT, "bad bnn_svgd_steps arguments (lr %g finite, bandwidth_factor %g > 0)", lr, bandwidth_factor);
  const int D = H * (F + 3) + 2;
  const int64_t need = bnn_svgd_workspace_bytes(P, num_particles, D);
  if (workspace_bytes < need || (need > 0 && !workspace))
    return fail(PFN_ERR_ARGUMENT, "workspace_bytes %lld < pfn_bnn_svgd_workspace_bytes = %lld (or a NULL workspace)", (long long)workspace_bytes, (long long)need);
  if (num_steps == 0) return PFN_OK;
  BnnSvgdArgs a{};
  a.x = x; a.y = y; a.n_of = n_of; a.state = state; a.ld = ld; a.P = P; a.S = S; a.F = F; a.H = H; a.activation = activation; a.N = num_particles; a.step0 = step0;
  a.num_steps = num_steps; a.lr = lr; a.beta1 = beta1; a.beta2 = beta2; a.eps = eps; a.bandwidth_factor = bandwidth_factor;
  a.grads = need > 0 ? (float*)workspace : nullptr; a.potential = potential; a.bandwidth = bandwidth;
  PFN_TRY(launch_bnn_svgd_steps(a, (hipStream_t)stream));
  return PFN_OK;
}

int pfn_tabular_windows(const float* X, const float* y, const int32_t* starts, int64_t N, int F, int F_out, int W, int bptt, int sep, float rescale, int mode,
                        float* x_out, float* y_out, void* stream) {
  if (F < 1 || F > TAB_MAX_FEATURES || F_out < F)
    return fail(PFN_ERR_UNSUPPORTED, "F %d outside 1 .. %d or F_out %d < F (a block keeps one window's per-feature statistics in LDS)", F, TAB_MAX_FEATURES, F_out);
  if (mode != PFN_TAB_NORM_WITH_TEST && mode != PFN_TAB_NORM_TRAIN_ONLY) return fail(PFN_ERR_ARGUMENT, "unknown tabular_windows mode %d", mode);
  if (N < 1 || W < 1 || sep < 1 || sep > bptt || (mode == PFN_TAB_NORM_WITH_TEST && sep == bptt) || bptt > 65536 || !(rescale > 0.f))
    return fail(PFN_ERR_ARGUMENT, "bad tabular_windows arguments (N %lld >= 1, W %d >= 1, 1 <= sep %d <%s bptt %d <= 65536, rescale %g > 0)", (long long)N, W, sep,
                mode == PFN_TAB_NORM_WITH_TEST ? "" : "=", bptt, (double)rescale);
  if (!X || !y || !starts || !x_out) return fail(PFN_ERR_ARGUMENT, "bad tabular_windows arguments (X, y, starts, x_out not NULL)");
  if ((uintptr_t)x_out % 16) return fail(PFN_ERR_ALIGNMENT, "tabular_windows: x_out must be 16-byte aligned");
  TabWindowsArgs a{};
  a.X = X; a.y = y; a.starts = starts; a.N = N; a.F = F; a.F_out = F_out; a.W = W; a.bptt = bptt; a.sep = sep; a.mode = mode; a.rescale = rescale;
  a.x_out = x_out; a.y_out = y_out;
  PFN_TRY(launch_tab_windows(a, (hipStream_t)stream));
  return PFN_OK;
}
int pfn_auc_counts(const float* scores, const float* labels, int T, int C, int64_t* counts, void* stream) {
  if (T < 1 || T > 4096) return fail(PFN_ERR_UNSUPPORTED, "auc_counts: T %d outside 1 .. 4096 (a block stages one column in LDS)", T);
  if (C < 1 || !scores || !labels || !counts) return fail(PFN_ERR_ARGUMENT, "bad auc_counts arguments (C %d >= 1, scores, labels, counts not NULL)", C);
  PFN_TRY(launch_auc_counts(scores, labels, T, C, counts, (hipStream_t)stream));
  return PFN_OK;
}
int pfn_knn_cv(const float* train, const float* labels, const float* test, const int32_t* fold, int P, int n, int T, int F, int32_t* cv_correct, int32_t* test_pos,
               int32_t* test_nbr, void* stream) {
  if (n < 4 || n > 128 || T < 1 || T > 128 || F < 1 || F > 128)
    return fail(PFN_ERR_UNSUPPORTED, "knn_cv: n %d outside 4 .. 128, T %d outside 1 .. 128 or F %d outside 1 .. 128 (one thread per query, every row in LDS)", n, T, F);
  if (P < 1 || !train || !labels || !test || !fold || !cv_correct || !test_pos || !test_nbr)
    return fail(PFN_ERR_ARGUMENT, "bad knn_cv arguments (P %d >= 1, train, labels, test, fold, cv_correct, test_pos, test_nbr not NULL)", P);
  KnnCvArgs a{};
  a.train = train; a.labels = labels; a.test = test; a.fold = fold; a.P = P; a.n = n; a.T = T; a.F = F; a.cv_correct = cv_correct; a.test_pos = test_pos; a.test_nbr = test_nbr;
  PFN_TRY(launch_knn_cv(a, (hipStream_t)stream));
  return PFN_OK;
}

int pfn_mlp_prior_forward(const float* weights, const float* biases, const int32_t* model_of, const int32_t* dims, const float* noise_std,
                          float* causes, const float* noise, float* y, float* hidden, int B, int T, int HP, int Lmax, int activation, int gen_causes,
                          uint64_t seed, uint64_t offset, void* stream) {
  if (!weights || !biases || !model_of || !dims || !noise_std || !causes || !y) return fail(PFN_ERR_ARGUMENT, "bad mlp_prior_forward arguments");
  if (activation < 0 || activation > 3) return fail(PFN_ERR_UNSUPPORTED, "activation %d (0 identity, 1 relu, 2 tanh, 3 sigmoid)", activation);
  MlpPriorArgs a;
  a.weights = weights; a.biases = biases; a.model_of = model_of; a.dims = dims; a.noise_std = noise_std; a.causes = causes; a.noise = noise; a.y = y; a.hidden = hidden;
  a.B = B; a.T = T; a.HP = HP; a.Lmax = Lmax; a.activation = activation; a.gen_causes = gen_causes; a.seed = seed; a.offset = offset;
  PFN_TRY(launch_mlp_prior(a, (hipStream_t)stream));
  return PFN_OK;
}

int pfn_op_gemm_nt(const void* A, int64_t lda, const void* B, int64_t ldb, int M, int N, int K, int flags, const float* bias,
                   const void* aux, int64_t ld_aux, const float* resid, int64_t ld_resid, float* out_f32, int64_t ld_out_f32,
                   void* out_t, int64_t ld_out_t, void* out2_t, int64_t ld_out2, int prec, void* stream) {
  GemmNT g = nt(A, lda, B, ldb, M, N, K, flags);
  g.bias = bias; g.aux = aux; g.ld_aux = ld_aux; g.resid = resid; g.ld_resid = ld_resid; g.out_f32 = out_f32; g.ld_out_f32 = ld_out_f32;
  g.out_t = out_t; g.ld_out_t = ld_out_t; g.out2_t = out2_t; g.ld_out2 = ld_out2;
  PFN_TRY(launch_gemm_nt(g, prec, (hipStream_t)stream));
  return PFN_OK;
}
int pfn_op_gemm_tn(const void* A, int64_t lda, const void* B, int64_t ldb, float* C, int64_t ldc, int M, int P, int Q, int atomic, int prec, void* stream) {
  GemmTN g = tn(A, lda, B, ldb, C, ldc, M, P, Q);
  g.atomic = atomic;
  PFN_TRY(launch_gemm_tn(g, prec, (hipStream_t)stream));
  return PFN_OK;
}
int pfn_op_gemm_tn_group(int n, const void* const* A, const int64_t* lda, const void* const* B, const int64_t* ldb, float* const* C,
                         const int64_t* ldc, const int32_t* P, const int32_t* Q, float* const* colsum, int M, int splits, int prec, void* stream) {
  if (n < 1 || n > TN_GROUP_MAX || !A || !lda || !B || !ldb || !C || !ldc || !P || !Q) return fail(PFN_ERR_ARGUMENT, "bad gemm_tn_group arguments");
  GemmTNGroup g;
  memset(&g, 0, sizeof(g));
  g.n = n; g.M = M; g.splits = splits;
  for (int i = 0; i < n; ++i) {
    TnProblem& t = g.p[i];
    t.A = A[i]; t.lda = lda[i]; t.B = B[i]; t.ldb = ldb[i]; t.C = C[i]; t.ldc = ldc[i]; t.P = P[i]; t.Q = Q[i];
    t.colsum = colsum ? colsum[i] : nullptr;
  }
  PFN_TRY(launch_gemm_tn_group(g, prec, (hipStream_t)stream));
  return PFN_OK;
}
int pfn_op_gemm_ln(const void* A, int64_t lda, const void* B, int64_t ldb, int M, int N, int K, const float* bias,
                   const float* resid, const float* ry, const float* rmean, const float* rrstd, const float* rgamma, const float* rbeta,
                   const float* gamma, const float* beta, float eps, float* y, float* mean, float* rstd, void* x_t, int prec, void* stream) {
  GemmLN g;
  memset(&g, 0, sizeof(g));
  g.A = A; g.lda = lda; g.B = B; g.ldb = ldb; g.M = M; g.N = N; g.K = K; g.bias = bias; g.resid = resid;
  g.ry = ry; g.rmean = rmean; g.rrstd = rrstd; g.rgamma = rgamma; g.rbeta = rbeta; g.gamma = gamma; g.beta = beta; g.eps = eps;
  g.y = y; g.mean = mean; g.rstd = rstd; g.x_t = x_t; g.y16 = (prec & PFN_OP_SUMS_16BIT) ? 1 : 0;
  PFN_TRY(launch_gemm_ln(g, prec & ~PFN_OP_SUMS_16BIT, (hipStream_t)stream));
  return PFN_OK;
}
int pfn_op_gemm_lnbwd(const void* A, int64_t lda, const void* B, int64_t ldb, int M, int N, int K, const void* aux,
                      const float* y, const float* mean, const float* rstd, const float* gamma,
                      void* dx_t, float* dgamma, float* dbeta, int prec, void* stream) {
  GemmLNB g;
  memset(&g, 0, sizeof(g));
  g.A = A; g.lda = lda; g.B = B; g.ldb = ldb; g.M = M; g.N = N; g.K = K; g.aux = aux;
  g.y = y; g.mean = mean; g.rstd = rstd; g.gamma = gamma; g.dx_t = dx_t; g.dgamma = dgamma; g.dbeta = dbeta; g.y16 = (prec & PFN_OP_SUMS_16BIT) ? 1 : 0;
  PFN_TRY(launch_gemm_lnbwd(g, prec & ~PFN_OP_SUMS_16BIT, (hipStream_t)stream));
  return PFN_OK;
}
int pfn_op_attention_fwd(const void* qkv, void* ctx, float* lse, int B, int S, int E, int H, int sep, int prec, void* stream) {
  AttnArgs at; memset(&at, 0, sizeof(at));
  at.qkv = qkv; at.ctx = ctx; at.lse = lse; at.B = B; at.S = S; at.E = E; at.H = H; at.sep = sep;
  PFN_TRY(launch_attn_fwd(at, prec, (hipStream_t)stream));
  return PFN_OK;
}
int pfn_op_attention_fwd_from(const void* qkv, void* ctx, float* lse, int B, int S, int E, int H, int sep, int q_begin, int prec, void* stream) {
  AttnArgs at; memset(&at, 0, sizeof(at));
  at.qkv = qkv; at.ctx = ctx; at.lse = lse; at.B = B; at.S = S; at.E = E; at.H = H; at.sep = sep; at.q_begin = q_begin;
  PFN_TRY(launch_attn_fwd(at, prec, (hipStream_t)stream));
  return PFN_OK;
}
int pfn_op_attention_bwd_from(const void* qkv, const void* ctx, const float* lse, const void* dctx, void* dqkv, float* delta_ws, void* ds_ws,
                              int B, int S, int E, int H, int sep, int q_begin, int prec, int parts, void* stream) {
  AttnArgs at; memset(&at, 0, sizeof(at));
  at.qkv = qkv; at.ctx = const_cast<void*>(ctx); at.lse = const_cast<float*>(lse); at.B = B; at.S = S; at.E = E; at.H = H; at.sep = sep;
  at.dctx = dctx; at.dqkv = dqkv; at.delta = delta_ws; at.ds = ds_ws; at.parts = parts; at.q_begin = q_begin;
  PFN_TRY(launch_attn_bwd(at, prec, (hipStream_t)stream));
  return PFN_OK;
}
int pfn_op_gather_rows(const void* src_bs, void* dst_tb, int B, int S, int64_t row_bytes, int sep, void* stream) {
  if (!src_bs || !dst_tb || B < 1 || S < 1 || sep < 0 || sep > S) return fail(PFN_ERR_ARGUMENT, "bad gather_rows arguments");
  PFN_TRY(launch_gather_rows(src_bs, dst_tb, S, B, row_bytes, sep, (hipStream_t)stream));
  return PFN_OK;
}
int pfn_op_scatter_rows(const void* src_tb, void* dst_bs, int B, int S, int64_t row_bytes, int sep, int zero_from, void* stream) {
  if (!src_tb || !dst_bs || B < 1 || S < 1 || sep < 0 || sep > S) return fail(PFN_ERR_ARGUMENT, "bad scatter_rows arguments");
  PFN_TRY(launch_scatter_rows(src_tb, dst_bs, S, B, row_bytes, sep, zero_from, (hipStream_t)stream));
  return PFN_OK;
}
int64_t pfn_op_attention_bwd_ws_bytes(int B, int S, int H, int prec) {
  if (B < 1 || S < 1 || H < 1) return -1;
  return attn_bwd_ds_bytes(B, S, H, prec);
}
int pfn_op_attention_bwd(const void* qkv, const void* ctx, const float* lse, const void* dctx, void* dqkv, float* delta_ws, void* ds_ws,
                         int B, int S, int E, int H, int sep, int prec, int parts, void* stream) {
  AttnArgs at; memset(&at, 0, sizeof(at));
  at.qkv = qkv; at.ctx = const_cast<void*>(ctx); at.lse = const_cast<float*>(lse); at.B = B; at.S = S; at.E = E; at.H = H; at.sep = sep;
  at.dctx = dctx; at.dqkv = dqkv; at.delta = delta_ws; at.ds = ds_ws; at.parts = parts;
  PFN_TRY(launch_attn_bwd(at, prec, (hipStream_t)stream));
  return PFN_OK;
}
int pfn_op_layernorm_fwd(const float* x, const float* gamma, const float* beta, float* y_f32, void* y_t, float* mean, float* rstd,
                         int64_t rows, int E, float eps, int prec, void* stream) {
  PFN_TRY(launch_layernorm_fwd(x, gamma, beta, y_f32, y_t, mean, rstd, rows, E, eps, prec, (hipStream_t)stream));
  return PFN_OK;
}
int pfn_op_layernorm_bwd(const void* dy, int dy_is_t, const float* x, const float* gamma, const float* mean, const float* rstd, float* dx_f32,
                         void* dx_t, float* dgamma, float* dbeta, float* dbias_extra, int64_t rows, int E, int prec, void* stream) {
  PFN_TRY(launch_layernorm_bwd(dy, dy_is_t, x, gamma, mean, rstd, dx_f32, dx_t, dgamma, dbeta, dbias_extra, rows, E, prec, (hipStream_t)stream));
  return PFN_OK;
}
int pfn_op_qkv_projection(const void* x_t, const void* w_in_t, const float* b_in, void* qkv_t, float* kshift_ws,
                          int B, int S, int E, int sep, const int32_t* sep_of, int center, int prec, void* stream) {
  if (!x_t || !w_in_t || !b_in || !qkv_t || B < 1 || S < 1 || E < 8 || sep < 0 || sep > S) return fail(PFN_ERR_ARGUMENT, "bad qkv_projection arguments");
  GemmNT g = nt(x_t, E, w_in_t, E, B * S, 3 * E, E, EPI_BIAS | EPI_OUT_T);
  g.bias = b_in; g.out_t = qkv_t; g.ld_out_t = 3 * E;
  if (center) {
    if (!prec_is16(prec) || E % 64 || !kshift_ws) return fail(PFN_ERR_UNSUPPORTED, "key centring: 16-bit operands, emsize a multiple of 64, scratch of B * E floats");
    PFN_TRY(launch_key_shift(x_t, (const char*)w_in_t + (int64_t)E * E * esize(prec), kshift_ws, B, S, E, sep, sep_of, prec, (hipStream_t)stream));
    g.flags |= EPI_ROWSHIFT; g.rowshift = kshift_ws; g.rs_ld = E; g.rs_S = S; g.rs_n0 = E; g.rs_n1 = 2 * E;
  }
  PFN_TRY(launch_gemm_nt(g, prec, (hipStream_t)stream));
  return PFN_OK;
}
int pfn_op_cast(const float* src, void* dst, int64_t n, int prec, void* stream) {
  PFN_TRY(launch_cast_params(src, dst, n, prec, (hipStream_t)stream));
  return PFN_OK;
}

}
```

transformerscandobayesianinference_amd/csrc/pfn_kernels.h:

```cpp
#pragma once
#include <hip/hip_runtime.h>
#include <stdint.h>
#include <atomic>
#include "../../include/pfn_hip.h"

namespace pfn {

struct LdsAllowance {
  std::atomic<size_t> granted[16];
  template <typename K> void ensure(K kernel, size_t bytes) {
    int dev = 0;
    (void)hipGetDevice(&dev);
    std::atomic<size_t>& g = granted[dev & 15];
    if (bytes <= g.load(std::memory_order_acquire)) return;
    (void)hipFuncSetAttribute(reinterpret_cast<const void*>(kernel), hipFuncAttributeMaxDynamicSharedMemorySize, (int)bytes);
    size_t cur = g.load(std::memory_order_relaxed);
    while (cur < bytes && !g.compare_exchange_weak(cur, bytes, std::memory_order_release)) {}
  }
};

inline bool prec_is16(int p) { return p == PFN_PREC_BF16 || p == PFN_PREC_FP16; }
inline int prec_esize(int p) { return prec_is16(p) ? 2 : 4; }
#define PFN_DISPATCH_OP(prec, ...)                                                          \
  do {                                                                                      \
    if ((prec) == PFN_PREC_BF16) { using T = ::pfn::bf16_t; __VA_ARGS__; }                  \
    else if ((prec) == PFN_PREC_FP16) { using T = ::pfn::f16_t; __VA_ARGS__; }              \
    else { using T = float; __VA_ARGS__; }                                                  \
  } while (0)
typedef __bf16 bf16_t;
typedef _Float16 f16_t;

bool prof_enabled();
void* prof_begin(int slot, hipStream_t s);
void prof_end(void* token, int slot, hipStream_t s);
struct ProfScope {
  void* token; int slot; hipStream_t s;
  ProfScope(int slot_, hipStream_t s_) : token(prof_begin(slot_, s_)), slot(slot_), s(s_) {}
  ~ProfScope() { prof_end(token, slot, s); }
  ProfScope(const ProfScope&) = delete;
  ProfScope& operator=(const ProfScope&) = delete;
};

__host__ __device__ inline unsigned mix32(unsigned h) {
  h ^= h >> 16; h *= 0x7feb352du; h ^= h >> 15; h *= 0x846ca68bu; h ^= h >> 16;
  return h;
}
__host__ __device__ inline unsigned dropout_site_seed(unsigned long long seed, int layer, int site) {
  return mix32(mix32((unsigned)seed ^ (0x9E3779B1u * (unsigned)(layer * 4 + site + 1))) ^ (unsigned)(seed >> 32));
}
__host__ __device__ inline unsigned dropout_pair_seed(unsigned site_seed, int pair) { return mix32(site_seed ^ (0xC2B2AE35u * (unsigned)(pair + 1))); }
__host__ __device__ inline unsigned dropout_threshold(float p) {
  const double t = (double)p * 4294967296.0;
  return t >= 4294967295.0 ? 0xffffffffu : (unsigned)t;
}
__host__ __device__ inline bool dropout_keep(unsigned s, unsigned i, unsigned j, unsigned thr) {
  return mix32(s ^ (i * 0x9E3779B1u) ^ (j * 0x85EBCA77u)) >= thr;
}

enum : int {
  EPI_BIAS = 1,
  EPI_GELU = 2,
  EPI_GELU_BWD = 4,
  EPI_RESID = 8,
  EPI_OUT_F32 = 16,
  EPI_OUT_T = 32,
  EPI_OUT2_T = 64,
  EPI_ACCUM = 128,
  EPI_RESID_T = 256,
  EPI_ROWDOT = 512,
  EPI_ROWSHIFT = 1024,
};

struct GemmNT {
  const void* A; long lda;
  const void* B; long ldb;
  int M, N, K;
  int flags;
  const float* bias;
  const void* aux; long ld_aux;
  const float* resid; long ld_resid;
  float* out_f32; long ld_out_f32;
  void* out_t; long ld_out_t;
  void* out2_t; long ld_out2;
  int vec_ok;
  int wide_t;
  float* rowdot; const float* rd_lse; long rd_lse2_off; int rd_S, rd_H, rd_D;
  const float* rowshift; long rs_ld; int rs_S, rs_n0, rs_n1;
};
int launch_key_shift(const void* x_t, const void* w_k_t, float* kshift, int B, int S, int E, int sep, const int* sep_of, int precision, hipStream_t s);
int launch_gemm_nt(const GemmNT& g, int precision, hipStream_t stream);
bool gemm_nt_rowdot_fused(const GemmNT& g, int precision);
void set_gemm_nt_big_mode(int mode);
void set_gemm_ln_rows64(int on);

struct GemmTN {
  const void* A; long lda;
  const void* B; long ldb;
  float* C; long ldc;
  int M, P, Q;
  int atomic;
  int m_chunk;
  float* colsum;
  int max_splits;
  const float* scale_amax;
};
int launch_gemm_tn(GemmTN g, int precision, hipStream_t stream);

constexpr int TN_GROUP_MAX = 26;
struct TnProblem {
  const void* A; const void* B; float* C; float* colsum;
  long lda, ldb, ldc;
  int P, Q;
  int Pv;
};
struct GemmTNGroup {
  TnProblem p[TN_GROUP_MAX];
  int tile_start[TN_GROUP_MAX + 1];
  int n, M, splits, m_chunk;
  int debug_mask;
  const float* scale_amax;
};
void set_gemm_tn_debug_wrap(int rows);
void set_gemm_tn_group_waves(int waves);
void set_gemm_tn_group_splits(int splits);
struct GemmLN {
  const void* A; long lda;
  const void* B; long ldb;
  int M, N, K;
  const float* bias;
  const float* resid;
  const void* ry; const float* rmean; const float* rrstd; const float* rgamma; const float* rbeta;
  const float* gamma; const float* beta; float eps;
  void* y; float* mean; float* rstd; void* x_t;
  float* x_f32;
  int y16;
};
bool gemm_ln_supported(const GemmLN& g);
int launch_gemm_ln(const GemmLN& g, int precision, hipStream_t stream);

struct GemmLNB {
  const void* A; long lda;
  const void* B; long ldb;
  int M, N, K;
  const void* aux;
  const void* y; const float* mean; const float* rstd; const float* gamma;
  void* dx_t;
  float* dgamma; float* dbeta;
  const float* scale_amax;
  int y16;
};
bool gemm_lnbwd_supported(const GemmLNB& g);
int launch_gemm_lnbwd(const GemmLNB& g, int precision, hipStream_t stream);

bool gemm_tn_group_supported(const TnProblem& p);
int launch_gemm_tn_group(GemmTNGroup g, int precision, hipStream_t stream);

struct AttnArgs {
  const void* qkv; void* ctx; float* lse;
  int B, S, E, H, sep;
  const int* sep_of;
  int q_from_sep;
  union {
    struct {
      const void* dctx; void* dqkv; float* delta;
      void* ds;
      int ds_rows, ds_ld;
      int parts;
      int zero_delta;
    };
    struct {
      const void* kv; long kv_ld, kv_sb;
      float* part_o;
      float* part_ml;
      int split_keys;
    };
  };
  int pingpong;
  int b0, bg;
  const void* xq;
  const void* wq;
  const float* bq;
  int q_store;
  int q_begin;
  float p_drop;
  unsigned drop_seed;
};
int attn_cache_splits(int B, int n, int E, int H, int sep, int precision);
int launch_attn_fwd_cache(const AttnArgs& a, int precision, hipStream_t stream);
void set_attn_cache_split_cap(int splits);
struct AttnCacheBwdArgs {
  const void* qkv;
  const void* ctx;
  const float* lse;
  const void* dctx;
  void* dqkv;
  const void* kv; long kv_ld, kv_sb;
  float* part_dq;
  int B, S, E, H, sep;
  int split_keys;
  const int* sep_of;
};
int launch_clamp_sep_of(const int* src, int* dst, int B, int hi, hipStream_t stream);
int launch_attn_bwd_cache(const AttnCacheBwdArgs& a, int precision, hipStream_t stream);
void set_attn_pingpong(int mask);
void set_attn_bwd_group(int datasets);
enum : int { ATTN_BWD_DELTA = 1, ATTN_BWD_KV = 2, ATTN_BWD_DQ = 4 };
int64_t attn_bwd_ds_bytes(int B, int S, int H, int precision);
int launch_attn_fwd(const AttnArgs& a, int precision, hipStream_t stream);
bool attn_fwd_can_fuse_q(int E, int H, int precision);
int launch_attn_bwd(const AttnArgs& a, int precision, hipStream_t stream);

int launch_cast_params(const float* src, void* dst_t, long n, int precision, hipStream_t s);
constexpr int TRANSPOSE_GROUP_MAX = 64;
struct TransposeGroup {
  int n = 0, blocks = 0;
  long src_off[TRANSPOSE_GROUP_MAX], dst_off[TRANSPOSE_GROUP_MAX];
  int rows[TRANSPOSE_GROUP_MAX], cols[TRANSPOSE_GROUP_MAX], ld_dst[TRANSPOSE_GROUP_MAX], first_block[TRANSPOSE_GROUP_MAX];
};
void transpose_group_add(TransposeGroup& g, long src_off, long dst_off, int rows, int cols, int ld_dst);
int launch_transpose_cast_group(const float* src, void* dst, const TransposeGroup& g, int precision, hipStream_t s);
int launch_transpose_cast(const float* src, void* dst_t, int rows, int cols, long ld_dst, int precision, hipStream_t s);
int launch_cast_rows(const float* src, long ld_src, void* dst_t, long ld_dst, long R, int C, int precision, hipStream_t s, const float* scale_amax = nullptr);
int launch_absmax(const float* x, long n, float* amax, hipStream_t s);
int set_loss_scale_target(int log2_target);
int launch_scale_copy(const float* src, float* dst, long n, const float* scale_amax, hipStream_t s);

struct EmbedArgs {
  const float* x; long x_st, x_sb;
  const float* y; long y_st, y_sb;
  const float* wx; const float* bx;
  const float* wy; const float* by;
  float* out_f32; void* out_t;
  void* xaug_t;
  int xaug_ld;
  const float* xaug_amax;
  int S, B, nf, E, sep;
  const int* sep_of;
};
constexpr int EMB_MAX_FEATURES = 1022;
__host__ __device__ inline int emb_aug_width(int nf) { return nf + 2 <= 32 ? 32 : nf + 2 <= 64 ? 64 : nf + 2 <= 128 ? 128 : 0; }
int launch_embed_fwd(const EmbedArgs& a, int precision, hipStream_t s);
int launch_embed_colmax(const EmbedArgs& a, float* amax, hipStream_t s);
__device__ inline int xaug_col_exp(const float* amax, int f) {
  if (!amax) return 0;
  const float m = amax[f];
  if (!(m > 0.f) || !(m <= 3.402823466e38f)) return 0;
  const int e = ilogbf(m);
  return e < -126 ? -126 : e;
}
struct EmbedBwdArgs {
  const float* dsrc; const float* x; long x_st, x_sb; const float* y; long y_st, y_sb;
  float* dwx; float* dbx; float* dwy; float* dby;
  int S, B, nf, E, sep;
  const int* sep_of;
  int single_block;
  const float* scale_amax;
};
int launch_embed_bwd(const EmbedBwdArgs& a, hipStream_t s);
int launch_embed_grad_scatter(const float* acc, float* dwx, float* dwy, float* dby, int E, int nf, const float* xaug_amax, hipStream_t s);
// ... 229 lines not shown
```

transformerscandobayesianinference_amd/hipops.py:

```python
import ctypes
import math

import torch

from transformerscandobayesianinference_amd import _hip

TDT = {_hip.PREC_BF16: torch.bfloat16, _hip.PREC_F32: torch.float32, _hip.PREC_FP16: torch.float16}
PREC_OF = {v: k for k, v in TDT.items()}
MANGLED_OPERAND = {_hip.PREC_BF16: 'DF16b', _hip.PREC_FP16: 'DF16_', _hip.PREC_F32: 'f'}


def sp():
    return _hip.stream_ptr()


def gemm_nt(A, B, flags, prec, bias=None, aux=None, resid=None, out_f32=None, out_t=None, out2_t=None):
    M, K = A.shape
    N = B.shape[0]
    p = _hip.ptr
    ld = lambda t: 0 if t is None else t.stride(0)
    _hip.check(_hip.lib().pfn_op_gemm_nt(p(A), A.stride(0), p(B), B.stride(0), M, N, K, flags, p(bias), p(aux), ld(aux),
                                         p(resid), ld(resid), p(out_f32), ld(out_f32), p(out_t), ld(out_t), p(out2_t), ld(out2_t),
                                         prec, sp()), 'pfn_op_gemm_nt')


def gemm_tn(A, B, C, prec, atomic=1):
    M, P = A.shape
    Q = B.shape[1]
    _hip.check(_hip.lib().pfn_op_gemm_tn(A.data_ptr(), A.stride(0), B.data_ptr(), B.stride(0), C.data_ptr(), C.stride(0), M, P, Q,
                                         atomic, prec, sp()), 'pfn_op_gemm_tn')


def gemm_tn_group(problems, splits=0):
    import ctypes
    n = len(problems)
    M = problems[0][0].shape[0]
    VP, L, I = ctypes.c_void_p * n, ctypes.c_int64 * n, ctypes.c_int32 * n
    A = VP(*[p[0].data_ptr() for p in problems]); lda = L(*[p[0].stride(0) for p in problems])
    B = VP(*[p[1].data_ptr() for p in problems]); ldb = L(*[p[1].stride(0) for p in problems])
    C = VP(*[p[2].data_ptr() for p in problems]); ldc = L(*[p[2].stride(0) for p in problems])
    P = I(*[p[0].shape[1] for p in problems]); Q = I(*[p[1].shape[1] for p in problems])
    cs = VP(*[(p[3].data_ptr() if p[3] is not None else None) for p in problems])
    _hip.check(_hip.lib().pfn_op_gemm_tn_group(n, A, lda, B, ldb, C, ldc, P, Q, cs, M, splits, PREC_OF[problems[0][0].dtype], sp()), 'pfn_op_gemm_tn_group')


SUMS_16BIT = 256


def gemm_ln(A, B, bias, gamma, beta, eps, resid=None, prev=None, out=None, sums16=False):
    M, K = A.shape
    N = B.shape[0]
    dev = A.device
    if out is None:
        y = torch.full((M + 2, N), float('nan'), dtype=A.dtype if sums16 else torch.float32, device=dev)
        x_t = torch.empty(M, N, dtype=A.dtype, device=dev)
        mean, rstd = torch.empty(M, device=dev), torch.empty(M, device=dev)
    else:
        y, x_t, mean, rstd = out
    p = _hip.ptr
    pv = prev if prev is not None else (None,) * 5
    assert y.dtype == (A.dtype if sums16 else torch.float32) and (pv[0] is None or pv[0].dtype == y.dtype)
    _hip.check(_hip.lib().pfn_op_gemm_ln(p(A), A.stride(0), p(B), B.stride(0), M, N, K, p(bias), p(resid), p(pv[0]), p(pv[1]), p(pv[2]), p(pv[3]), p(pv[4]),
                                         p(gamma), p(beta), eps, p(y), p(mean), p(rstd), p(x_t), PREC_OF[A.dtype] | (SUMS_16BIT if sums16 else 0), sp()), 'pfn_op_gemm_ln')
    if out is None:
        assert torch.isnan(y[M:]).all()
    return y[:M], x_t, mean, rstd


def attention_fwd(qkv, H, sep, prec, q_begin=0, out=None):
    B, S, E3 = qkv.shape
    E = E3 // 3
    if q_begin:
        if out is not None:
            ctx, lse = out
        else:
            ctx = torch.full((B, S, E), float('nan'), dtype=qkv.dtype, device=qkv.device)
            lse = torch.full((B, H, S), float('nan'), dtype=torch.float32, device=qkv.device)
        _hip.check(_hip.lib().pfn_op_attention_fwd_from(qkv.data_ptr(), ctx.data_ptr(), lse.data_ptr(), B, S, E, H, sep, q_begin, prec, sp()), 'attn fwd')
        return ctx, lse
    ctx = torch.empty(B, S, E, dtype=qkv.dtype, device=qkv.device)
    lse = torch.empty(B, H, S, dtype=torch.float32, device=qkv.device)
    _hip.check(_hip.lib().pfn_op_attention_fwd(qkv.data_ptr(), ctx.data_ptr(), lse.data_ptr(), B, S, E, H, sep, prec, sp()), 'attn fwd')
    return ctx, lse


def gather_rows(src, sep, out=None):
    B, S, W = src.shape
    dst = out if out is not None else torch.empty((S - sep) * B, W, dtype=src.dtype, device=src.device)
    _hip.check(_hip.lib().pfn_op_gather_rows(src.data_ptr(), dst.data_ptr(), B, S, W * src.element_size(), sep, sp()), 'gather rows')
    return dst


def scatter_rows(src, B, S, sep, zero_from, fill=float('nan'), out=None):
    W = src.shape[1]
    dst = out if out is not None else torch.full((B, S, W), fill, dtype=src.dtype, device=src.device)
    _hip.check(_hip.lib().pfn_op_scatter_rows(src.data_ptr(), dst.data_ptr(), B, S, W * src.element_size(), sep, zero_from, sp()), 'scatter rows')
    return dst


def gemm_lnbwd(A, B, aux, y, mean, rstd, gamma, out=None):
    M, K = A.shape
    N = B.shape[0]
    if out is None:
        out = (torch.full((M + 2, N), float('nan'), dtype=A.dtype, device=A.device), torch.zeros(N, device=A.device), torch.zeros(N, device=A.device))
    dx_t, dgamma, dbeta = out
    p = _hip.ptr
    _hip.check(_hip.lib().pfn_op_gemm_lnbwd(p(A), A.stride(0), p(B), B.stride(0), M, N, K, p(aux), p(y), p(mean), p(rstd), p(gamma),
                                            p(dx_t), p(dgamma), p(dbeta), PREC_OF[A.dtype] | (SUMS_16BIT if y.dtype == A.dtype else 0), sp()), 'pfn_op_gemm_lnbwd')
    return dx_t, dgamma, dbeta


ATTENTION_BWD_PARTS = [
    ('attn_bwd: delta = rowsum(dO * O)', '_ZN3pfn17attn_delta_kernelI{T}EEvNS_8AttnArgsEi', 1, 0.0, 0.0),
    ('attn_bwd: key-block pass (S, dP, dV, dK products; stores dS^T)', '_ZN3pfn18attn_bwd_kv_kernelI{T}Li{D}ELi0ELb0', 2, 3.0, 4.0),
    ('attn_bwd: query-block pass (dQ = dS K from the stored dS^T)', '_ZN3pfn18attn_bwd_dq_kernelI{T}Li{D}ELb0', 4, 1.0, 1.0),
]
ATTENTION_FWD_ROCPROF = '_ZN3pfn15attn_fwd_kernelI{T}Li{D}ELb0'
ATTENTION_BWD_KV_EXECUTED_UNITS = {}
_bwd_scratch = {}


def attention_bwd(qkv, ctx, lse, dctx, H, sep, prec, parts=0, q_begin=0):
    B, S, E3 = qkv.shape
    E = E3 // 3
    key = (tuple(qkv.shape), qkv.dtype, qkv.device, H)
    if key not in _bwd_scratch:
        _bwd_scratch.clear()
        ws = _hip.check(_hip.lib().pfn_op_attention_bwd_ws_bytes(B, S, H, prec), 'attn bwd ws')
        _bwd_scratch[key] = (torch.zeros_like(qkv), torch.zeros(2, B, H, S, dtype=torch.float32, device=qkv.device),
                             torch.empty(ws, dtype=torch.uint8, device=qkv.device))
    dqkv, delta, ds = _bwd_scratch[key]
    if not parts:
        dqkv = torch.full_like(qkv, float('nan'))
        ds.fill_(0xff)
    if q_begin:
        _hip.check(_hip.lib().pfn_op_attention_bwd_from(qkv.data_ptr(), ctx.data_ptr(), lse.data_ptr(), dctx.data_ptr(), dqkv.data_ptr(),
                                                        delta.data_ptr(), ds.data_ptr(), B, S, E, H, sep, q_begin, prec, parts, sp()), 'attn bwd')
        return dqkv
    _hip.check(_hip.lib().pfn_op_attention_bwd(qkv.data_ptr(), ctx.data_ptr(), lse.data_ptr(), dctx.data_ptr(), dqkv.data_ptr(),
                                               delta.data_ptr(), ds.data_ptr(), B, S, E, H, sep, prec, parts, sp()), 'attn bwd')
    return dqkv


def layernorm_fwd(x, gamma, beta, eps, prec):
    rows, E = x.shape
    y32 = torch.empty_like(x)
    yt = torch.empty(rows, E, dtype=TDT[prec], device=x.device)
    mean = torch.empty(rows, device=x.device)
    rstd = torch.empty(rows, device=x.device)
    _hip.check(_hip.lib().pfn_op_layernorm_fwd(x.data_ptr(), gamma.data_ptr(), beta.data_ptr(), y32.data_ptr(), yt.data_ptr(),
                                               mean.data_ptr(), rstd.data_ptr(), rows, E, eps, prec, sp()), 'ln fwd')
    return y32, yt, mean, rstd


def layernorm_bwd(dy, x, gamma, mean, rstd, prec, want_f32=True):
    rows, E = x.shape
    dy_is_t = int(dy.dtype != torch.float32)
    dx32 = torch.empty_like(x) if want_f32 else None
    dxt = torch.empty(rows, E, dtype=TDT[prec], device=x.device)
    dg = torch.zeros(E, device=x.device)
    db = torch.zeros(E, device=x.device)
    dbias = torch.zeros(E, device=x.device)
    _hip.check(_hip.lib().pfn_op_layernorm_bwd(dy.data_ptr(), dy_is_t, x.data_ptr(), gamma.data_ptr(), mean.data_ptr(), rstd.data_ptr(),
                                               dx32.data_ptr() if want_f32 else 0, dxt.data_ptr(), dg.data_ptr(), db.data_ptr(), dbias.data_ptr(),
                                               rows, E, prec, sp()), 'ln bwd')
    return dx32, dxt, dg, db, dbias


def qkv_projection(x, w_in, b_in, sep, center=True, sep_of=None):
    B, S, E = x.shape
    qkv = torch.full((B, S, 3 * E), float('nan'), dtype=x.dtype, device=x.device)
    ks = torch.full((B, E), float('nan'), dtype=torch.float32, device=x.device)
    _hip.check(_hip.lib().pfn_op_qkv_projection(x.data_ptr(), w_in.data_ptr(), b_in.data_ptr(), qkv.data_ptr(), ks.data_ptr(), B, S, E, sep,
                                                _hip.ptr(sep_of), int(center), PREC_OF[x.dtype], sp()), 'pfn_op_qkv_projection')
    return qkv, ks


def gp_fit_workspace(P, S, device):
    return torch.empty(int(_hip.lib().pfn_gp_fit_workspace_bytes(P, S)), dtype=torch.uint8, device=device)


def _gp_fit_inputs(x, y, theta, prior, n_of):
    _hip.require_gpu_tensor(x, 'x')
    P, S, F = x.shape
    assert S % 4 == 0, 'S must be a multiple of 4 (pad and mask the padding through n_of)'
    assert y.shape == (P, S) and theta.shape == (P, F + 3) and prior.shape == (8,)
    for t in (x, y, theta, prior):
        assert t.dtype == torch.float32 and t.is_contiguous() and t.device == x.device
    if n_of is not None:
        assert n_of.dtype == torch.int32 and n_of.shape == (P,) and n_of.is_contiguous() and n_of.device == x.device
    return P, S, F


def gp_mll_grad(x, y, theta, prior, kernel, n_of=None, flags=0, want_grad=True, ws=None):
    P, S, F = _gp_fit_inputs(x, y, theta, prior, n_of)
    ws = gp_fit_workspace(P, S, x.device) if ws is None else ws
# ... 287 lines not shown
```

transformerscandobayesianinference_amd/transformer.py:

```python
import ctypes

import torch
from torch import nn

from transformerscandobayesianinference_amd import _hip
from transformerscandobayesianinference_amd.positional_encodings import NoPositionalEncoding
from transformerscandobayesianinference_amd.utils import SeqBN

_ALIGN = 64


class _SelfAttentionParams(nn.Module):

    def __init__(self, emsize):
        super().__init__()
        self.in_proj_weight = nn.Parameter(torch.empty(3 * emsize, emsize))
        self.in_proj_bias = nn.Parameter(torch.zeros(3 * emsize))
        self.out_proj = nn.Linear(emsize, emsize)
        nn.init.xavier_uniform_(self.in_proj_weight)
        nn.init.zeros_(self.out_proj.bias)


class _EncoderLayerParams(nn.Module):

    def __init__(self, emsize, nhid):
        super().__init__()
        self.self_attn = _SelfAttentionParams(emsize)
        self.linear1 = nn.Linear(emsize, nhid)
        self.linear2 = nn.Linear(nhid, emsize)
        self.norm1 = nn.LayerNorm(emsize, eps=1e-5)
        self.norm2 = nn.LayerNorm(emsize, eps=1e-5)


class _EncoderParams(nn.Module):
    def __init__(self, emsize, nhid, nlayers):
        super().__init__()
        self.layers = nn.ModuleList([_EncoderLayerParams(emsize, nhid) for _ in range(nlayers)])


class _StackFunction(torch.autograd.Function):

    @staticmethod
    def forward(ctx, flat_params, model, x, y, src, sep, inference, ragged=None):
        lib = _hip.lib()
        dev = flat_params.device
        stream = _hip.stream_ptr(dev)
        desc, shadow = model._operands(stream, inference)
        if src is not None:
            src = src.contiguous().float()
            if src.data_ptr() % 16:
                src = src.clone()
            S, B = src.shape[0], src.shape[1]
            xs = ys = None
            x_ptr = y_ptr = 0
            x_st = x_sb = y_st = y_sb = 0
        else:
            if x.dtype != torch.float32 or x.stride(-1) != 1:
                x = x.float().contiguous()
            if y.dtype != torch.float32:
                y = y.float()
            S, B = x.shape[0], x.shape[1]
            x_ptr, y_ptr = x.data_ptr(), y.data_ptr()
            x_st, x_sb = x.stride(0), x.stride(1)
            y_st, y_sb = y.stride(0), y.stride(1)
        ws_bytes = lib.pfn_workspace_bytes(ctypes.byref(desc), B, S)
        _hip.check(ws_bytes, 'pfn_workspace_bytes')
        ws = torch.empty(ws_bytes, dtype=torch.uint8, device=dev)
        ctx.ragged = ragged
        if ragged is not None:
            sep_of, row_off, sep_min, sep_max, test_rows = ragged
            logits = torch.empty((test_rows, desc.n_out or desc.emsize), dtype=torch.float32, device=dev)
            ctx.dropout_seed = model._next_dropout_seed() if (model.training and desc.dropout > 0) else None
            _hip.check(lib.pfn_stack_forward_ragged(ctypes.byref(desc), flat_params.data_ptr(), shadow.data_ptr(), x_ptr, x_st, x_sb, y_ptr, y_st, y_sb, B, S,
                                                    sep_of.data_ptr(), row_off.data_ptr(), sep_min, sep_max, test_rows, ws.data_ptr(), ws_bytes, logits.data_ptr(), stream,
                                                    int(ctx.dropout_seed is not None), ctx.dropout_seed or 0), 'pfn_stack_forward_ragged')
            ctx.model, ctx.ws, ctx.dims = model, ws, (B, S, sep_max)
            ctx.operands = (desc, shadow)
            ctx.inputs = (x, y, None)
            ctx.src_needs_grad = False
            return logits
        logits = torch.empty((S - sep, B, desc.n_out or desc.emsize), dtype=torch.float32, device=dev)
        ctx.dropout_seed = None
        if model.training and desc.dropout > 0:
            ctx.dropout_seed = model._next_dropout_seed()
            _hip.check(lib.pfn_stack_forward_dropout(ctypes.byref(desc), flat_params.data_ptr(), shadow.data_ptr(),
                                                     x_ptr, x_st, x_sb, y_ptr, y_st, y_sb, _hip.ptr(src), B, S, sep,
                                                     ws.data_ptr(), ws_bytes, logits.data_ptr(), stream, ctx.dropout_seed), 'pfn_stack_forward_dropout')
        else:
            _hip.check(lib.pfn_stack_forward(ctypes.byref(desc), flat_params.data_ptr(), shadow.data_ptr(),
                                             x_ptr, x_st, x_sb, y_ptr, y_st, y_sb, _hip.ptr(src), B, S, sep,
                                             ws.data_ptr(), ws_bytes, logits.data_ptr(), stream), 'pfn_stack_forward')
        ctx.model, ctx.ws, ctx.dims = model, ws, (B, S, sep)
        ctx.operands = (desc, shadow)
        ctx.inputs = (x, y, src)
        ctx.src_needs_grad = src is not None and ctx.needs_input_grad[4]
        return logits

    @staticmethod
    def backward(ctx, dlogits):
        lib = _hip.lib()
        model, ws = ctx.model, ctx.ws
        B, S, sep = ctx.dims
        x, y, src = ctx.inputs
        dev = ws.device
        stream = _hip.stream_ptr(dev)
        desc, shadow = ctx.operands
        if desc is not model._desc:
            raise RuntimeError('backward through an inference-precision forward: the forward of this graph ran the eval_precision kernels')
        model._attach_grads()
        dlogits = dlogits.contiguous().float()
        dsrc = None
        if src is not None:
            dsrc = torch.empty_like(src)
            args = (0, 0, 0, 0, 0, 0)
        else:
            args = (x.data_ptr(), x.stride(0), x.stride(1), y.data_ptr(), y.stride(0), y.stride(1))
        hook = model._first_group_hook
        split = hook is not None and hook.armed()
        if ctx.ragged is not None:
            sep_of, row_off, sep_min, sep_max, test_rows = ctx.ragged
            cb = _hip.HOST_CALLBACK(lambda user: hook.first_group_launched()) if split else None
            _hip.check(lib.pfn_stack_backward_ragged(ctypes.byref(desc), model._flat.data_ptr(), shadow.data_ptr(), *args, B, S,
                                                     sep_of.data_ptr(), row_off.data_ptr(), sep_min, sep_max, test_rows, ws.data_ptr(), ws.numel(), dlogits.data_ptr(),
                                                     model._flat_grad.data_ptr(), stream, hook.first_group_layers if split else 0, cb, None,
                                                     int(ctx.dropout_seed is not None), ctx.dropout_seed or 0), 'pfn_stack_backward_ragged')
            ctx.ws = None
            return None, None, None, None, None, None, None, None
        if split or ctx.dropout_seed is not None:
            cb = _hip.HOST_CALLBACK(lambda user: hook.first_group_launched()) if split else None
            _hip.check(lib.pfn_stack_backward_split(ctypes.byref(desc), model._flat.data_ptr(), shadow.data_ptr(), *args,
                                                    B, S, sep, ws.data_ptr(), ws.numel(), dlogits.data_ptr(),
                                                    model._flat_grad.data_ptr(), _hip.ptr(dsrc), stream,
                                                    hook.first_group_layers if split else 0, cb, None,
                                                    int(ctx.dropout_seed is not None), ctx.dropout_seed or 0),
                       'pfn_stack_backward_split')
        else:
            _hip.check(lib.pfn_stack_backward(ctypes.byref(desc), model._flat.data_ptr(), shadow.data_ptr(), *args,
                                              B, S, sep, ws.data_ptr(), ws.numel(), dlogits.data_ptr(),
                                              model._flat_grad.data_ptr(), _hip.ptr(dsrc), stream), 'pfn_stack_backward')
        dx = dy = None
        if src is None and (ctx.needs_input_grad[2] or ctx.needs_input_grad[3]):
            dx = torch.empty((S, B, x.shape[2]), dtype=torch.float32, device=dev)
            dy = torch.empty((S, B), dtype=torch.float32, device=dev) if ctx.needs_input_grad[3] else None
            if sep == S:
                dx.zero_()
                if dy is not None:
                    dy.zero_()
            else:
                _hip.check(lib.pfn_stack_input_grads(ctypes.byref(desc), model._flat.data_ptr(), B, S, sep, ws.data_ptr(), ws.numel(),
                                                     dx.data_ptr(), dx.stride(0), dx.stride(1), _hip.ptr(dy), B, 1, stream),
                           'pfn_stack_input_grads')
        ctx.ws = None
        return (None, None, dx if ctx.needs_input_grad[2] else None, dy, (dsrc if ctx.src_needs_grad else None), None, None, None)


class _PredictFunction(torch.autograd.Function):

    @staticmethod
    def forward(ctx, x, model, context, desc, shadow):
        lib = _hip.lib()
        dev = x.device
        stream = _hip.stream_ptr(dev)
        n, B, _ = x.shape
        ws_bytes = _hip.check(lib.pfn_predict_grad_workspace_bytes(ctypes.byref(desc), B, n), 'pfn_predict_grad_workspace_bytes')
        ws = torch.empty(ws_bytes, dtype=torch.uint8, device=dev)
        out = torch.empty((n, B, desc.n_out or desc.emsize), dtype=torch.float32, device=dev)
        if context.lengths is not None:
            _hip.check(lib.pfn_stack_predict_saved_ragged(ctypes.byref(desc), model._flat.data_ptr(), shadow.data_ptr(), context.buffer.data_ptr(),
                                                          context.buffer.numel(), context.sep, context.sep_of.data_ptr(), x.data_ptr(), x.stride(0), x.stride(1),
                                                          B, n, ws.data_ptr(), ws_bytes, out.data_ptr(), stream), 'pfn_stack_predict_saved_ragged')
        else:
            _hip.check(lib.pfn_stack_predict_saved(ctypes.byref(desc), model._flat.data_ptr(), shadow.data_ptr(), context.buffer.data_ptr(), context.buffer.numel(),
                                                   context.sep, x.data_ptr(), x.stride(0), x.stride(1), B, n, ws.data_ptr(), ws_bytes, out.data_ptr(), stream),
                       'pfn_stack_predict_saved')
        ctx.state = (model, context, desc, shadow, ws, x.shape)
        return out

    @staticmethod
    def backward(ctx, dout):
        model, context, desc, shadow, ws, (n, B, F) = ctx.state
        lib = _hip.lib()
        dout = dout.contiguous().float()
        dx = torch.empty((n, B, F), dtype=torch.float32, device=dout.device)
        if context.lengths is not None:
            _hip.check(lib.pfn_stack_predict_backward_ragged(ctypes.byref(desc), model._flat.data_ptr(), shadow.data_ptr(), context.buffer.data_ptr(),
                                                             context.buffer.numel(), context.sep, context.sep_of.data_ptr(), B, n, ws.data_ptr(), ws.numel(),
                                                             dout.data_ptr(), dx.data_ptr(), dx.stride(0), dx.stride(1), _hip.stream_ptr(dout.device)),
                       'pfn_stack_predict_backward_ragged')
        else:
            _hip.check(lib.pfn_stack_predict_backward(ctypes.byref(desc), model._flat.data_ptr(), shadow.data_ptr(), context.buffer.data_ptr(), context.buffer.numel(),
                                                      context.sep, B, n, ws.data_ptr(), ws.numel(), dout.data_ptr(), dx.data_ptr(), dx.stride(0), dx.stride(1),
                                                      _hip.stream_ptr(dout.device)), 'pfn_stack_predict_backward')
        ctx.state = None
        return dx, None, None, None, None


def ragged_layout(T, widths, single_eval_positions):
    seps = []
    for sep in single_eval_positions:
        sep = int(sep)
        seps.append(max(0, min(T, sep + T if sep < 0 else sep)))
    per_dataset = [s for s, w in zip(seps, widths) for _ in range(w)]
    offs = [0]
    for s in per_dataset:
        offs.append(offs[-1] + T - s)
    return seps, per_dataset, offs


def check_train_lengths(train_lengths, B, sep_max):
    if isinstance(train_lengths, torch.Tensor):
        if train_lengths.dim() != 1 or train_lengths.dtype.is_floating_point or train_lengths.dtype in (torch.bool, torch.complex64, torch.complex128):
            raise ValueError(f'train_lengths: expected an integer tensor [B], got {train_lengths.dtype} of shape {tuple(train_lengths.shape)}')
        train_lengths = train_lengths.tolist()
    lengths = []
    for v in train_lengths:
        if isinstance(v, bool) or int(v) != v:
            raise ValueError(f'train_lengths: {v!r} is not an integer')
        lengths.append(int(v))
    if len(lengths) != B:
        raise ValueError(f'train_lengths has {len(lengths)} entries, the batch has B={B} datasets')
    for b, v in enumerate(lengths):
        if v < 0 or v > sep_max:
            raise ValueError(f'train_lengths[{b}] = {v} is outside [0, {sep_max}] (the rows of the padded training set)')
    return tuple(lengths)


def pad_datasets(datasets):
    if len(datasets) == 0:
        raise ValueError('pad_datasets: no dataset')
    x0 = datasets[0][0]
    if x0.dim() != 2:
        raise ValueError(f'pad_datasets: x of dataset 0 has shape {tuple(x0.shape)}, expected [s, F]')
    F = x0.shape[1]
    lengths = []
    for b, (xb, yb) in enumerate(datasets):
        if xb.dim() != 2 or xb.shape[1] != F or tuple(yb.shape) != (xb.shape[0],):
            raise ValueError(f'pad_datasets: dataset {b} has x {tuple(xb.shape)} and y {tuple(yb.shape)}, expected [s, {F}] and [s]')
        lengths.append(xb.shape[0])
    sep_max = max(lengths)
    x = x0.new_zeros((sep_max, len(datasets), F))
    y = datasets[0][1].new_zeros((sep_max, len(datasets)))
    for b, (xb, yb) in enumerate(datasets):
        x[:lengths[b], b] = xb
        y[:lengths[b], b] = yb
    return x, y, tuple(lengths)


class PredictContext:

    def __init__(self, buffer, param_version, desc_key, B, F, sep, device, lengths=None, sep_of=None):
        self.buffer, self.param_version, self.desc_key = buffer, param_version, desc_key
        self.B, self.F, self.sep, self.device = B, F, sep, device
        self.lengths, self.sep_of = lengths, sep_of

    def __repr__(self):
        ragged = '' if self.lengths is None else f', lengths {min(self.lengths)}..{max(self.lengths)}'
        return f'PredictContext(B={self.B}, F={self.F}, sep={self.sep}{ragged}, {self.buffer.numel()} bytes on {self.device})'


class TransformerModel(nn.Module):
    requires_gpu = True

    def __init__(self, encoder, n_out, ninp, nhead, nhid, nlayers, dropout=0.0, y_encoder=None, pos_encoder=None,
                 decoder=None, input_normalization=False, precision='fp16', eval_precision='f32', deterministic=False):
        super().__init__()
        self.model_type = 'Transformer'
        self.transformer_encoder = _EncoderParams(ninp, nhid, nlayers)
        self.ninp, self.nhead, self.nhid, self.nlayers, self.n_out = ninp, nhead, nhid, nlayers, n_out
        self.dropout = dropout
        self.encoder = encoder
        self.y_encoder = y_encoder
        self.pos_encoder = pos_encoder
        self._custom_decoder = decoder is not None
        self.decoder = decoder(ninp, nhid, n_out) if decoder is not None else nn.Sequential(nn.Linear(ninp, nhid), nn.GELU(), nn.Linear(nhid, n_out))
        self.input_ln = SeqBN(ninp) if input_normalization else None
        if self._fused_embedding() and encoder.in_features > _hip.MAX_FEATURES:
            raise ValueError(f'{encoder.in_features} features: the fused embedding takes at most {_hip.MAX_FEATURES} (include/pfn_hip.h num_features)')
        self.precision = precision
        self.eval_precision = eval_precision
        self._flat = self._flat_grad = self._shadow = None
        self.schedule = None
        if deterministic:
            self.schedule = _hip.SCHED_DETERMINISTIC
        self._shadow_version = None
        self._desc = None
        self._eval_desc = self._eval_shadow = self._eval_shadow_version = None
        self._first_group_hook = None
        self._views = []
        self.init_weights()
        self.register_load_state_dict_post_hook(lambda module, incompatible: module.mark_params_updated())

    @staticmethod
    def generate_square_subsequent_mask(sz):
        allowed = torch.tril(torch.ones(sz, sz, dtype=torch.bool))
        return torch.zeros(sz, sz).masked_fill(~allowed, float('-inf'))

    @staticmethod
    def generate_D_q_matrix(sz, query_size):
        train_size = sz - query_size
        allowed = torch.zeros(sz, sz, dtype=torch.bool)
        allowed[:, :train_size] = True
        allowed |= torch.eye(sz, dtype=torch.bool)
        return torch.zeros(sz, sz).masked_fill(~allowed, float('-inf'))

# ... 336 lines not shown
```

Measured before the change: 2579 datasets/s.

## Fold first-layer input-gradient GEMM into embedding weight-gradient via associativity

```diff
diff --git a/include/pfn_hip.h b/include/pfn_hip.h
--- a/include/pfn_hip.h
+++ b/include/pfn_hip.h
@@ -62,6 +62,7 @@
        PFN_TUNE_FUSE_Q_PROJECTION = 12,
        PFN_TUNE_KEY_CENTERING = 13,
        PFN_TUNE_ATTN_CACHE_SPLITS = 17,
+       PFN_TUNE_EMBED_FIRST_LAYER = 18,
        PFN_TUNE_TOP_LAYER_TEST_ROWS = 6  };
 int pfn_set_tuning(int key, int value);
 enum { PFN_PROF_ATTN_FWD = 0, PFN_PROF_ATTN_BWD_DELTA = 2, PFN_PROF_ATTN_BWD_KV = 4, PFN_PROF_ATTN_BWD_DQ = 6, PFN_PROF_GEMM_QKV = 8,
@@ -149,6 +150,14 @@
 int pfn_stack_input_grads(const pfn_model_desc* d, const float* params, int B, int S, int sep,
                           const void* workspace, int64_t workspace_bytes,
                           float* dx, int64_t dx_st, int64_t dx_sb, float* dy, int64_t dy_st, int64_t dy_sb, void* stream);
+int pfn_stack_input_grads_shadow(const pfn_model_desc* d, const float* params, const void* shadow, int B, int S, int sep,
+                                 void* workspace, int64_t workspace_bytes,
+                                 float* dx, int64_t dx_st, int64_t dx_sb, float* dy, int64_t dy_st, int64_t dy_sb, void* stream);
+int pfn_embed_first_layer_skipped(const pfn_model_desc* d, int B, int S);
+int64_t pfn_embed_grad_launches(int which);
+int64_t pfn_op_embed_first_layer_scratch_floats(int precision, int64_t M, int P, int64_t w0, int64_t ldz0, int64_t w1, int64_t ldz1, int deterministic);
+int pfn_op_embed_first_layer(int precision, const void* A, int64_t lda, int P, const void* Z0, int64_t ldz0, int64_t w0, const void* Z1, int64_t ldz1, int64_t w1,
+                             int64_t M, const void* W, int64_t ldw, float* scratch, int64_t scratch_floats, int deterministic, float* G, void* stream);
 
 int pfn_stack_condition_ragged(const pfn_model_desc* d, const float* params, const void* shadow,
                                const float* x, int64_t x_st, int64_t x_sb,
diff --git a/transformerscandobayesianinference_amd/_hip.py b/transformerscandobayesianinference_amd/_hip.py
--- a/transformerscandobayesianinference_amd/_hip.py
+++ b/transformerscandobayesianinference_amd/_hip.py
@@ -71,6 +71,11 @@
     'pfn_stack_predict_saved_ragged': (_I, [_D, _P, _P, _P, _L, _I, _P, _P, _L, _L, _I, _I, _P, _L, _P, _P]),
     'pfn_stack_predict_backward_ragged': (_I, [_D, _P, _P, _P, _L, _I, _P, _I, _I, _P, _L, _P, _P, _L, _L, _P]),
     'pfn_stack_input_grads': (_I, [_D, _P, _I, _I, _I, _P, _L, _P, _L, _L, _P, _L, _L, _P]),
+    'pfn_stack_input_grads_shadow': (_I, [_D, _P, _P, _I, _I, _I, _P, _L, _P, _L, _L, _P, _L, _L, _P]),
+    'pfn_embed_first_layer_skipped': (_I, [_D, _I, _I]),
+    'pfn_embed_grad_launches': (_L, [_I]),
+    'pfn_op_embed_first_layer_scratch_floats': (_L, [_I, _L, _I, _L, _L, _L, _L, _I]),
+    'pfn_op_embed_first_layer': (_I, [_I, _P, _L, _I, _P, _L, _L, _P, _L, _L, _L, _P, _L, _P, _L, _I, _P, _P]),
     'pfn_bar_nll_forward': (_I, [_P, _L, _P, _P, _L, _I, _I, _P, _P, _P, _P]),
     'pfn_bar_nll_backward': (_I, [_P, _L, _P, _P, _P, _L, _I, _P, _P]),
     'pfn_bar_mean': (_I, [_P, _L, _P, _L, _I, _I, _P, _P]),
diff --git a/transformerscandobayesianinference_amd/csrc/embed_tn_plan.h b/transformerscandobayesianinference_amd/csrc/embed_tn_plan.h
--- /dev/null
+++ b/transformerscandobayesianinference_amd/csrc/embed_tn_plan.h
@@ -0,0 +1,70 @@
+#pragma once
+#include <stdint.h>
+
+namespace pfn {
+
+constexpr int ETN_KT = 64;
+constexpr int ETN_ROW_BYTES = 512;
+constexpr int ETN_TARGET_WGS = 512;
+constexpr int ETN_DET_MAX_SPLITS = 16;
+constexpr int ETN_MAX_P = 64;
+constexpr int64_t ETN_MAX_SPLIT_BYTES = 0x7ffffff0LL - 16;
+
+struct EmbedTnPlan {
+  int ok;
+  int aug;
+  int rows;
+  int cb_cols;
+  int cb[2];
+  int splits, chunk;
+  int planes;
+  int64_t q;
+  int64_t plane_floats;
+  int64_t scratch_floats;
+};
+
+inline int64_t etn_div_up(int64_t a, int64_t b) { return (a + b - 1) / b; }
+
+inline EmbedTnPlan embed_tn_plan(int64_t M, int P, int64_t w0, int64_t ld0, int64_t w1, int64_t ld1, int es, int deterministic, int64_t scratch_avail) {
+  EmbedTnPlan p = {};
+  if (es != 2 && es != 4) return p;
+  const int epc = 16 / es;
+  if (M < 1 || M > 0x7fffffff || P < 1 || P > ETN_MAX_P || w0 < 1 || w1 < 0) return p;
+  if (w0 % epc || w1 % epc || ld0 < w0 || (w1 > 0 && ld1 < w1) || w0 + w1 > (1 << 20) || ld0 > (1 << 24) || ld1 > (1 << 24)) return p;
+  p.aug = P <= 32 ? 32 : 64;
+  p.rows = P + 1;
+  p.cb_cols = ETN_ROW_BYTES / es;
+  p.cb[0] = (int)etn_div_up(w0, p.cb_cols);
+  p.cb[1] = (int)etn_div_up(w1, p.cb_cols);
+  p.q = w0 + w1;
+  p.plane_floats = (int64_t)p.rows * p.q;
+  const int blocks = p.cb[0] + p.cb[1];
+  int64_t splits = ETN_TARGET_WGS / blocks;
+  if (splits < 1) splits = 1;
+  if (deterministic && splits > ETN_DET_MAX_SPLITS) splits = ETN_DET_MAX_SPLITS;
+  if (scratch_avail >= 0) {
+    const int64_t fit = scratch_avail / p.plane_floats;
+    if (fit < 1) return p;
+    if (deterministic && splits > fit) splits = fit;
+  }
+  const int64_t stages = etn_div_up(M, ETN_KT);
+  if (splits > stages) splits = stages;
+  const int64_t chunk = etn_div_up(etn_div_up(M, splits), ETN_KT) * ETN_KT;
+  splits = etn_div_up(M, chunk);
+  const int64_t ldmax = ld0 > ld1 ? ld0 : ld1;
+  if ((chunk + ETN_KT) * ldmax * es > ETN_MAX_SPLIT_BYTES) return p;
+  p.splits = (int)splits;
+  p.chunk = (int)chunk;
+  p.planes = deterministic ? p.splits : 1;
+  p.scratch_floats = p.planes * p.plane_floats;
+  p.ok = 1;
+  return p;
+}
+inline int64_t embed_tn_split_begin(const EmbedTnPlan& p, int s) { return (int64_t)s * p.chunk; }
+inline int64_t embed_tn_split_rows(const EmbedTnPlan& p, int64_t M, int s) {
+  const int64_t b = embed_tn_split_begin(p, s), e = b + p.chunk < M ? b + p.chunk : M;
+  return e > b ? e - b : 0;
+}
+inline int64_t embed_tn_plane_offset(const EmbedTnPlan& p, int s) { return p.planes > 1 ? (int64_t)s * p.plane_floats : 0; }
+
+}
diff --git a/transformerscandobayesianinference_amd/csrc/gemm_tn.hip b/transformerscandobayesianinference_amd/csrc/gemm_tn.hip
--- a/transformerscandobayesianinference_amd/csrc/gemm_tn.hip
+++ b/transformerscandobayesianinference_amd/csrc/gemm_tn.hip
@@ -419,7 +419,194 @@
 }
 #endif
 
+template <typename T, int AUG>
+__global__ __launch_bounds__(256, 2) void embed_tn_kernel(EmbedTN g, EmbedTnPlan pl) {
+  constexpr int ES = sizeof(T);
+  constexpr int RBA = AUG * ES;
+  constexpr int SA = PadStride<RBA>::COL, SZ = PadStride<ETN_ROW_BYTES>::COL;
+  constexpr int NB = AUG / 32;
+  constexpr int CPW = ETN_ROW_BYTES / ES / 4;
+  constexpr int CT = CPW / 32;
+  __shared__ __attribute__((aligned(16))) char smem_raw[ETN_KT * (SA + SZ)];
+  LdsPtr ta = lds_cast(smem_raw), tz = ta + ETN_KT * SA;
+
+  const int part = (int)blockIdx.x >= pl.cb[0] ? 1 : 0;
+  const int q0 = ((int)blockIdx.x - (part ? pl.cb[0] : 0)) * pl.cb_cols;
+  const int wvalid = min(pl.cb_cols, g.w[part] - q0);
+  const long mbeg = (long)blockIdx.y * pl.chunk;
+  const int rows = (int)min((long)pl.chunk, g.M - mbeg);
+  if (rows <= 0 || wvalid <= 0) return;
+  const long lda_b = g.lda * ES, ldz_b = g.ldz[part] * ES;
+  const BufRsrc ra = make_rsrc(reinterpret_cast<const char*>(g.A) + mbeg * lda_b, (rows - 1) * lda_b + RBA);
+  const BufRsrc rz = make_rsrc(reinterpret_cast<const char*>(g.Z[part]) + mbeg * ldz_b + (long)q0 * ES, (rows - 1) * ldz_b + (long)wvalid * ES);
+  TileStageBuf<T, ETN_KT, RBA, 256> sa;
+  TileStageBuf<T, ETN_KT, ETN_ROW_BYTES, 256> sz;
+  sa.init((int)lda_b);
+  sz.init((int)ldz_b);
+
+  const int wave = threadIdx.x >> 6, lane = threadIdx.x & 63;
+  f32x16 acc[NB + 1][CT];
+#pragma unroll
+  for (int i = 0; i <= NB; ++i)
+#pragma unroll
+    for (int j = 0; j < CT; ++j)
+#pragma unroll
+      for (int r = 0; r < 16; ++r) acc[i][j][r] = 0.f;
+  Frag<T> ones;
+#pragma unroll
+  for (int e = 0; e < 8; ++e) ones.set(e, 1.f);
+
+  const int nst = (rows + ETN_KT - 1) / ETN_KT;
+  sa.issue(ra, 0);
+  sz.issue(rz, 0);
+  for (int t = 0; t < nst; ++t) {
+    sa.template commit_p<SA>(ta);
+    sz.template commit_p<SZ>(tz);
+    __syncthreads();
+    if (t + 1 < nst) {
+      sa.issue(ra, (t + 1) * ETN_KT * (int)lda_b);
+      sz.issue(rz, (t + 1) * ETN_KT * (int)ldz_b);
+    }
+#pragma unroll
+    for (int ks = 0; ks < ETN_KT; ks += 16) {
+      Frag<T> fa[NB], fz[CT];
+#pragma unroll
+      for (int i = 0; i < NB; ++i) fa[i] = load_frag_tr_p<T, SA, 1>(ta, ks, i * 32);
+#pragma unroll
+      for (int j = 0; j < CT; ++j) fz[j] = load_frag_tr_p<T, SZ, 1>(tz, ks, wave * CPW + j * 32);
+#pragma unroll
+      for (int j = 0; j < CT; ++j) {
+#pragma unroll
+        for (int i = 0; i < NB; ++i) acc[i][j] = mma32(fa[i], fz[j], acc[i][j]);
+        acc[NB][j] = mma32(ones, fz[j], acc[NB][j]);
+      }
+    }
+    __syncthreads();
+  }
+
+  float* Tp = g.T + (pl.planes > 1 ? (long)blockIdx.y * pl.plane_floats : 0L);
+  const long qoff = (part ? g.w[0] : 0) + q0;
+#pragma unroll
+  for (int i = 0; i <= NB; ++i)
+#pragma unroll
+    for (int j = 0; j < CT; ++j)
+#pragma unroll
+      for (int r = 0; r < 16; ++r) {
+        const int ar = acc_row(r, lane);
+        const int row = i < NB ? i * 32 + ar : g.P;
+        const bool valid = i < NB ? row < g.P : ar == 0;
+        const int col = wave * CPW + j * 32 + (lane & 31);
+        if (valid && col < wvalid) {
+          float* c = Tp + (long)row * pl.q + qoff + col;
+          if (pl.planes > 1) *c = acc[i][j][r];
+          else unsafeAtomicAdd(c, acc[i][j][r]);
+        }
+      }
+}
+__global__ __launch_bounds__(256) void embed_tn_reduce_kernel(float* T, long plane_floats, int planes) {
+  const long i = (long)blockIdx.x * 256 + threadIdx.x;
+  if (i >= plane_floats) return;
+  float v = T[i];
+  for (int p = 1; p < planes; ++p) v += T[p * plane_floats + i];
+  T[i] = v;
+}
+
+template <typename T, int EB>
+__global__ __launch_bounds__(256) void embed_finish_kernel(EmbedFinish f) {
+  extern __shared__ __attribute__((aligned(16))) char smem_raw[];
+  T* wl = reinterpret_cast<T*>(smem_raw);
+  const int e0 = blockIdx.x * EB;
+  const T* W = reinterpret_cast<const T*>(f.W);
+  constexpr int EPC = 16 / sizeof(T);
+  const int cpr = f.K / EPC;
+  for (int i = threadIdx.x; i < EB * cpr; i += 256) {
+    const int e = i / cpr, c = i - e * cpr;
+    u32x4 v = {0u, 0u, 0u, 0u};
+    if (e0 + e < f.E) v = *reinterpret_cast<const u32x4*>(W + (long)(e0 + e) * f.ldw + c * EPC);
+    *reinterpret_cast<u32x4*>(wl + e * f.K + c * EPC) = v;
+  }
+  __syncthreads();
+  const int wave = threadIdx.x >> 6, lane = threadIdx.x & 63;
+  const long q = (long)f.K + f.E;
+  const float osc = loss_scale_down(f.scale_amax);
+  const int r = blockIdx.y * 4 + wave;
+  if (r < f.rows) {
+    const float* tr = f.T + r * q;
+    float acc[EB];
+#pragma unroll
+    for (int e = 0; e < EB; ++e) acc[e] = 0.f;
+    for (int k0 = lane; k0 < f.K; k0 += 8 * 64) {
+      float t[8];
+#pragma unroll
+      for (int u = 0; u < 8; ++u) t[u] = k0 + u * 64 < f.K ? tr[k0 + u * 64] : 0.f;
+#pragma unroll
+      for (int u = 0; u < 8; ++u) {
+        const int k = k0 + u * 64 < f.K ? k0 + u * 64 : 0;
+#pragma unroll
+        for (int e = 0; e < EB; ++e) acc[e] += t[u] * (float)wl[e * f.K + k];
+      }
+    }
+    float mine = 0.f;
+#pragma unroll
+    for (int e = 0; e < EB; ++e) {
+      const float s = wave_sum(acc[e]);
+      if (lane == e) mine = s;
+    }
+    const int e = e0 + lane;
+    if (lane < EB && e < f.E) {
+      float v = mine + tr[f.K + e];
+      if (f.G) f.G[(long)r * f.E + e] = v;
+      if (f.dwx) {
+        v *= osc;
+        if (r < f.rows - 1) v = ldexpf(v, xaug_col_exp(f.xaug_amax, r));
+        if (r < f.nf) unsafeAtomicAdd(f.dwx + (long)e * f.nf + r, v);
+        else if (r == f.nf) unsafeAtomicAdd(f.dwy + e, v);
+        else if (r == f.nf + 1) unsafeAtomicAdd(f.dby + e, v);
+        else unsafeAtomicAdd(f.dbx + e, v);
+      }
+    }
+  }
+}
+
 static bool aligned16(const void* p) { return (reinterpret_cast<uintptr_t>(p) & 15) == 0; }
+
+EmbedTnPlan embed_tn_plan_of(const EmbedTN& g, int precision) {
+  const int es = prec_esize(precision);
+  EmbedTnPlan pl = embed_tn_plan(g.M, g.P, g.w[0], g.ldz[0], g.w[1], g.ldz[1], es, g.deterministic, g.scratch_floats);
+  if (!pl.ok) return pl;
+  const bool aligned = aligned16(g.A) && aligned16(g.Z[0]) && (g.w[1] == 0 || aligned16(g.Z[1])) && (g.lda * es) % 16 == 0 && (g.ldz[0] * es) % 16 == 0 &&
+                       (g.w[1] == 0 || (g.ldz[1] * es) % 16 == 0);
+  if (!aligned || g.lda < pl.aug || (long)(pl.chunk + ETN_KT) * g.lda * es > ETN_MAX_SPLIT_BYTES) pl.ok = 0;
+  return pl;
+}
+int launch_embed_tn(const EmbedTN& g, int precision, hipStream_t stream) {
+  const EmbedTnPlan pl = embed_tn_plan_of(g, precision);
+  if (!pl.ok || !g.T) return PFN_ERR_UNSUPPORTED;
+  if (pl.planes == 1 && hipMemsetAsync(g.T, 0, sizeof(float) * pl.plane_floats, stream) != hipSuccess) return PFN_ERR_LAUNCH;
+  const dim3 grid(pl.cb[0] + pl.cb[1], pl.splits);
+  if (pl.aug == 32) PFN_DISPATCH_OP(precision, hipLaunchKernelGGL((embed_tn_kernel<T, 32>), grid, dim3(256), 0, stream, g, pl));
+  else PFN_DISPATCH_OP(precision, hipLaunchKernelGGL((embed_tn_kernel<T, 64>), grid, dim3(256), 0, stream, g, pl));
+  if (pl.planes > 1) hipLaunchKernelGGL(embed_tn_reduce_kernel, dim3((unsigned)((pl.plane_floats + 255) / 256)), dim3(256), 0, stream, g.T, (long)pl.plane_floats, pl.planes);
+  return hipGetLastError() == hipSuccess ? PFN_OK : PFN_ERR_LAUNCH;
+}
+template <typename T, int EB> static int launch_embed_finish_eb(const EmbedFinish& f, hipStream_t stream) {
+  static LdsAllowance allowance;
+  const size_t lds = (size_t)EB * f.K * sizeof(T);
+  allowance.ensure(embed_finish_kernel<T, EB>, lds);
+  hipLaunchKernelGGL((embed_finish_kernel<T, EB>), dim3((f.E + EB - 1) / EB, (f.rows + 3) / 4), dim3(256), lds, stream, f);
+  return hipGetLastError() == hipSuccess ? PFN_OK : PFN_ERR_LAUNCH;
+}
+int launch_embed_finish(const EmbedFinish& f, int precision, hipStream_t stream) {
+  if (f.rows < 1 || f.E < 1 || f.K < 1 || !f.T || !f.W || (!f.G && !f.dwx)) return PFN_ERR_ARGUMENT;
+  if (f.dwx && (f.rows != f.nf + 3 || !f.dbx || !f.dwy || !f.dby)) return PFN_ERR_ARGUMENT;
+  const size_t row = (size_t)f.K * prec_esize(precision);
+  if (row % 16 || (f.ldw * prec_esize(precision)) % 16 || !aligned16(f.W)) return PFN_ERR_ALIGNMENT;
+  if (4 * row > 96 * 1024) return PFN_ERR_UNSUPPORTED;
+  int rc = PFN_OK;
+  if (8 * row <= 96 * 1024) PFN_DISPATCH_OP(precision, rc = launch_embed_finish_eb<T, 8>(f, stream));
+  else PFN_DISPATCH_OP(precision, rc = launch_embed_finish_eb<T, 4>(f, stream));
+  return rc;
+}
 
 static int g_tn_debug_wrap = 0;
 void set_gemm_tn_debug_wrap(int rows) { g_tn_debug_wrap = rows; }
diff --git a/transformerscandobayesianinference_amd/csrc/pfn_api.hip b/transformerscandobayesianinference_amd/csrc/pfn_api.hip
--- a/transformerscandobayesianinference_amd/csrc/pfn_api.hip
+++ b/transformerscandobayesianinference_amd/csrc/pfn_api.hip
@@ -514,6 +514,29 @@
 static bool top_layer_on_test_rows_ragged(const pfn_model_desc& d, int S, const Ragged& rg, float pdrop) {
   return !(d.schedule & PFN_SCHED_TOP_LAYER_ALL_ROWS) && d.nlayers > 0 && pdrop == 0.f && d.dropout == 0.f && rg.test_rows > 0 && 4L * rg.sep_min >= S;
 }
+static bool g_embed_first_layer = true;
+static std::atomic<int64_t> g_embed_grad_launches[2];
+static bool embed_first_layer_plan(const pfn_model_desc& d, const Ws& w, int M, bool custom_encoder, EmbedTN* out) {
+  if (!g_embed_first_layer || !emb_gemm(d, custom_encoder)) return false;
+  const int aug = emb_aug_width(d.num_features), E = d.emsize;
+  if (aug > ETN_MAX_P || 4L * 3 * E * esize(d.precision) > 96 * 1024) return false;
+  EmbedTN g; memset(&g, 0, sizeof(g));
+  g.A = w.xaug_t; g.lda = aug; g.P = d.num_features + 2;
+  g.Z[0] = w.layer[0].dqkv_t; g.ldz[0] = 3L * E; g.w[0] = 3 * E;
+  g.Z[1] = w.layer[0].dy1_t; g.ldz[1] = E; g.w[1] = E;
+  g.T = w.gA; g.scratch_floats = (long)M * E; g.M = M;
+  g.deterministic = (d.schedule & PFN_SCHED_DETERMINISTIC) ? 1 : 0;
+  if (!embed_tn_plan_of(g, d.precision).ok) return false;
+  if (out) *out = g;
+  return true;
+}
+int pfn_embed_first_layer_skipped(const pfn_model_desc* d, int B, int S) {
+  PFN_TRY(check_desc(d));
+  if (B < 1 || S < 1) return fail(PFN_ERR_ARGUMENT, "bad B=%d S=%d", B, S);
+  const Ws w = carve(*d, B, S, nullptr);
+  return embed_first_layer_plan(*d, w, B * S, false, nullptr) ? 1 : 0;
+}
+int64_t pfn_embed_grad_launches(int which) { return which == 0 || which == 1 ? g_embed_grad_launches[which].exchange(0) : -1; }
 int pfn_abi_version(void) { return PFN_ABI_VERSION; }
 int pfn_default_schedule(void) { return g_default_schedule; }
 int pfn_profile_enable(int on) { g_prof_on.store(on < 0 ? 0 : on); return PFN_OK; }
@@ -554,6 +577,7 @@
     case PFN_TUNE_GEMM_LN_ROWS: set_gemm_ln_rows64(value); return PFN_OK;
     case PFN_TUNE_GP_PLANES: g_gp_planes = value != 0; return PFN_OK;
     case PFN_TUNE_FUSE_DELTA: g_fuse_delta = value != 0; return PFN_OK;
+    case PFN_TUNE_EMBED_FIRST_LAYER: g_embed_first_layer = value != 0; return PFN_OK;
     case PFN_TUNE_ATTN_CACHE_SPLITS: set_attn_cache_split_cap(value); return PFN_OK;
     case PFN_TUNE_FUSE_LN_WIDE: g_default_schedule = value ? (g_default_schedule | PFN_SCHED_FUSE_LN_WIDE) : (g_default_schedule & ~PFN_SCHED_FUSE_LN_WIDE); return PFN_OK;
     case PFN_TUNE_TOP_LAYER_TEST_ROWS: g_default_schedule = value ? (g_default_schedule & ~PFN_SCHED_TOP_LAYER_ALL_ROWS) : (g_default_schedule | PFN_SCHED_TOP_LAYER_ALL_ROWS); return PFN_OK;
@@ -1078,6 +1102,8 @@
                       LnSinks{grads + p.g2, grads + p.be2, db2}, LnSinks{grads + p.g1, grads + p.be1, dbo}, w.ln_part};
   };
   const bool emb_t = emb_gemm(*d, dsrc_sbe != nullptr);
+  EmbedTN emb_tn;
+  const bool emb_skip = embed_first_layer_plan(*d, w, M, dsrc_sbe != nullptr, &emb_tn);
   const bool fuse_lnb = d->nlayers > 0 && lnbwd_fusable(m, pl, lsc, view(0, false), M);
   auto launch_weight_gradients = [&](int l_hi, int l_lo) -> int {
     std::vector<TnProblem> probs, probs_top;
@@ -1149,7 +1175,7 @@
       PFN_TRY(launch_attn_bwd(at, prec, s));
     }
     const LayerGrads below = l > 0 ? view(l - 1, false) : LayerGrads{};
-    PFN_TRY(layer_backward_dx(m, t, a.dqkv_t, a.dy1_t, M, pl, lsc, fuse_lnb && l > 0 ? &below : nullptr, w.gA, w.gA_t, l == 0 && !emb_t, 0));
+    if (!(l == 0 && emb_skip)) PFN_TRY(layer_backward_dx(m, t, a.dqkv_t, a.dy1_t, M, pl, lsc, fuse_lnb && l > 0 ? &below : nullptr, w.gA, w.gA_t, l == 0 && !emb_t, 0));
     if (l == split_at) {
       PFN_TRY(launch_weight_gradients(d->nlayers - 1, split_at));
       on_first_group(user);
@@ -1159,7 +1185,16 @@
   const int aug = emb_aug_width(d->num_features);
   if (dsrc_sbe) {
     PFN_TRY(launch_bse_to_sbe(w.gA, dsrc_sbe, S, B, E, s, lsc));
+  } else if (emb_skip) {
+    PFN_TRY(launch_embed_tn(emb_tn, prec, s));
+    EmbedFinish f; memset(&f, 0, sizeof(f));
+    f.T = emb_tn.T; f.rows = d->num_features + 3; f.E = E; f.K = 3 * E; f.W = WT(m, L.layer_t[0].w_in); f.ldw = 3L * E;
+    f.dwx = grads + L.enc_w; f.dbx = grads + L.enc_b; f.dwy = grads + L.yenc_w; f.dby = grads + L.yenc_b; f.nf = d->num_features;
+    f.scale_amax = lsc; f.xaug_amax = prec == PFN_PREC_FP16 ? w.xaug_amax : nullptr;
+    PFN_TRY(launch_embed_finish(f, prec, s));
+    g_embed_grad_launches[0].fetch_add(1, std::memory_order_relaxed);
   } else if (emb_t) {
+    g_embed_grad_launches[1].fetch_add(1, std::memory_order_relaxed);
     if (hipMemsetAsync(w.embacc, 0, sizeof(float) * E * aug, s) != hipSuccess) return fail(PFN_ERR_LAUNCH, "memset");
     GemmTN g = tn(w.gA_t, E, w.xaug_t, aug, w.embacc, aug, M, E, aug, grads + L.enc_b);
     g.scale_amax = lsc;
@@ -1176,17 +1211,24 @@
   return PFN_OK;
 }
 
-int pfn_stack_input_grads(const pfn_model_desc* d, const float* params, int B, int S, int sep, const void* workspace, int64_t workspace_bytes,
-                          float* dx, int64_t dx_st, int64_t dx_sb, float* dy, int64_t dy_st, int64_t dy_sb, void* stream) {
+static int stack_input_grads_impl(const pfn_model_desc* d, const float* params, const void* shadow, bool with_shadow, int B, int S, int sep, void* workspace,
+                                  int64_t workspace_bytes, float* dx, int64_t dx_st, int64_t dx_sb, float* dy, int64_t dy_st, int64_t dy_sb, void* stream) {
   PFN_TRY(check_desc(d));
   if (B < 1 || S < 1 || sep < 0 || sep > S) return fail(PFN_ERR_ARGUMENT, "bad B=%d S=%d sep=%d", B, S, sep);
-  if (!params || !workspace || !dx) return fail(PFN_ERR_ARGUMENT, "null pointer");
+  if (!params || !workspace || !dx || (with_shadow && !shadow)) return fail(PFN_ERR_ARGUMENT, "null pointer");
   Ws w = carve(*d, B, S, (char*)workspace);
   if (workspace_bytes < w.bytes) return fail(PFN_ERR_ARGUMENT, "workspace too small: %lld < %lld", (long long)workspace_bytes, (long long)w.bytes);
   const int prec = d->precision, E = d->emsize;
   const Layout L = make_layout(*d);
   hipStream_t s = (hipStream_t)stream;
   const bool emb_t = emb_gemm(*d, false);
+  if (embed_first_layer_plan(*d, w, B * S, false, nullptr)) {
+    if (!with_shadow) return fail(PFN_ERR_UNSUPPORTED, "the backward left no d(src) in the workspace (PFN_TUNE_EMBED_FIRST_LAYER): call pfn_stack_input_grads_shadow");
+    const Model m = {d, params, (const char*)shadow, &L, s};
+    GemmNT g = nt(w.layer[0].dqkv_t, 3 * E, WT(m, L.layer_t[0].w_in), 3 * E, B * S, E, 3 * E, EPI_RESID_T | EPI_OUT_T);
+    g.aux = w.layer[0].dy1_t; g.ld_aux = E; g.out_t = w.gA_t; g.ld_out_t = E;
+    PFN_TRY(launch_gemm_nt(g, prec, s));
+  }
   EmbedInGradArgs e; memset(&e, 0, sizeof(e));
   e.dsrc = emb_t ? (const void*)w.gA_t : (const void*)w.gA; e.dsrc_prec = emb_t ? prec : PFN_PREC_F32;
   e.wx = params + L.enc_w; e.wy = params + L.yenc_w;
@@ -1194,6 +1236,14 @@
   e.S = S; e.B = B; e.nf = d->num_features; e.E = E; e.sep = sep;
   e.scale_amax = (prec == PFN_PREC_FP16 && sep < S) ? w.lscale : nullptr;
   return launch_embed_input_grad(e, s);
+}
+int pfn_stack_input_grads(const pfn_model_desc* d, const float* params, int B, int S, int sep, const void* workspace, int64_t workspace_bytes,
+                          float* dx, int64_t dx_st, int64_t dx_sb, float* dy, int64_t dy_st, int64_t dy_sb, void* stream) {
+  return stack_input_grads_impl(d, params, nullptr, false, B, S, sep, const_cast<void*>(workspace), workspace_bytes, dx, dx_st, dx_sb, dy, dy_st, dy_sb, stream);
+}
+int pfn_stack_input_grads_shadow(const pfn_model_desc* d, const float* params, const void* shadow, int B, int S, int sep, void* workspace, int64_t workspace_bytes,
+                                 float* dx, int64_t dx_st, int64_t dx_sb, float* dy, int64_t dy_st, int64_t dy_sb, void* stream) {
+  return stack_input_grads_impl(d, params, shadow, true, B, S, sep, workspace, workspace_bytes, dx, dx_st, dx_sb, dy, dy_st, dy_sb, stream);
 }
 
 int pfn_bar_mean_backward(const float* logits, int64_t ld, const float* borders, int64_t R, int nbars, int full_support, const float* mean, const float* gout,
@@ -1554,6 +1604,33 @@
   PFN_TRY(launch_gemm_tn(g, prec, (hipStream_t)stream));
   return PFN_OK;
 }
+static EmbedTN op_embed_tn(const void* A, int64_t lda, int P, const void* Z0, int64_t ldz0, int64_t w0, const void* Z1, int64_t ldz1, int64_t w1, int64_t M,
+                           float* scratch, int64_t scratch_floats, int deterministic) {
+  EmbedTN g; memset(&g, 0, sizeof(g));
+  g.A = A; g.lda = lda; g.P = P; g.Z[0] = Z0; g.ldz[0] = ldz0; g.w[0] = (int)w0; g.Z[1] = Z1; g.ldz[1] = ldz1; g.w[1] = (int)w1;
+  g.T = scratch; g.scratch_floats = scratch_floats; g.M = M; g.deterministic = deterministic ? 1 : 0;
+  return g;
+}
+int64_t pfn_op_embed_first_layer_scratch_floats(int precision, int64_t M, int P, int64_t w0, int64_t ldz0, int64_t w1, int64_t ldz1, int deterministic) {
+  if (precision != PFN_PREC_BF16 && precision != PFN_PREC_F32 && precision != PFN_PREC_FP16) return fail(PFN_ERR_ARGUMENT, "bad precision %d", precision);
+  const EmbedTnPlan pl = embed_tn_plan(M, P, w0, ldz0, w1, ldz1, esize(precision), deterministic, -1);
+  if (!pl.ok) return fail(PFN_ERR_UNSUPPORTED, "embed_first_layer: shape outside the kernel");
+  return pl.scratch_floats;
+}
+int pfn_op_embed_first_layer(int precision, const void* A, int64_t lda, int P, const void* Z0, int64_t ldz0, int64_t w0, const void* Z1, int64_t ldz1, int64_t w1,
+                             int64_t M, const void* W, int64_t ldw, float* scratch, int64_t scratch_floats, int deterministic, float* G, void* stream) {
+  if (precision != PFN_PREC_BF16 && precision != PFN_PREC_F32 && precision != PFN_PREC_FP16) return fail(PFN_ERR_ARGUMENT, "bad precision %d", precision);
+  if (!A || !Z0 || !Z1 || !W || !scratch || !G || w1 < 1 || ldw < w0) return fail(PFN_ERR_ARGUMENT, "bad embed_first_layer arguments");
+  const int64_t need = pfn_op_embed_first_layer_scratch_floats(precision, M, P, w0, ldz0, w1, ldz1, deterministic);
+  if (need < 0) return (int)need;
+  if (scratch_floats < need) return fail(PFN_ERR_ARGUMENT, "scratch too small: %lld < %lld", (long long)scratch_floats, (long long)need);
+  const EmbedTN g = op_embed_tn(A, lda, P, Z0, ldz0, w0, Z1, ldz1, w1, M, scratch, need, deterministic);
+  PFN_TRY(launch_embed_tn(g, precision, (hipStream_t)stream));
+  EmbedFinish f; memset(&f, 0, sizeof(f));
+  f.T = scratch; f.rows = P + 1; f.E = (int)w1; f.K = (int)w0; f.W = W; f.ldw = ldw; f.G = G;
+  PFN_TRY(launch_embed_finish(f, precision, (hipStream_t)stream));
+  return PFN_OK;
+}
 int pfn_op_gemm_tn_group(int n, const void* const* A, const int64_t* lda, const void* const* B, const int64_t* ldb, float* const* C,
                          const int64_t* ldc, const int32_t* P, const int32_t* Q, float* const* colsum, int M, int splits, int prec, void* stream) {
   if (n < 1 || n > TN_GROUP_MAX || !A || !lda || !B || !ldb || !C || !ldc || !P || !Q) return fail(PFN_ERR_ARGUMENT, "bad gemm_tn_group arguments");
diff --git a/transformerscandobayesianinference_amd/csrc/pfn_kernels.h b/transformerscandobayesianinference_amd/csrc/pfn_kernels.h
--- a/transformerscandobayesianinference_amd/csrc/pfn_kernels.h
+++ b/transformerscandobayesianinference_amd/csrc/pfn_kernels.h
@@ -3,6 +3,7 @@
 #include <stdint.h>
 #include <atomic>
 #include "../../include/pfn_hip.h"
+#include "embed_tn_plan.h"
 
 namespace pfn {
 
@@ -105,6 +106,25 @@
   const float* scale_amax;
 };
 int launch_gemm_tn(GemmTN g, int precision, hipStream_t stream);
+
+struct EmbedTN {
+  const void* A; long lda; int P;
+  const void* Z[2]; long ldz[2]; int w[2];
+  float* T; long scratch_floats;
+  long M;
+  int deterministic;
+};
+EmbedTnPlan embed_tn_plan_of(const EmbedTN& g, int precision);
+int launch_embed_tn(const EmbedTN& g, int precision, hipStream_t stream);
+struct EmbedFinish {
+  const float* T; int rows, E, K;
+  const void* W; long ldw;
+  float* G;
+  float *dwx, *dbx, *dwy, *dby; int nf;
+  const float* scale_amax;
+  const float* xaug_amax;
+};
+int launch_embed_finish(const EmbedFinish& f, int precision, hipStream_t stream);
 
 constexpr int TN_GROUP_MAX = 26;
 struct TnProblem {
diff --git a/transformerscandobayesianinference_amd/hipops.py b/transformerscandobayesianinference_amd/hipops.py
--- a/transformerscandobayesianinference_amd/hipops.py
+++ b/transformerscandobayesianinference_amd/hipops.py
@@ -42,6 +42,18 @@
     P = I(*[p[0].shape[1] for p in problems]); Q = I(*[p[1].shape[1] for p in problems])
     cs = VP(*[(p[3].data_ptr() if p[3] is not None else None) for p in problems])
     _hip.check(_hip.lib().pfn_op_gemm_tn_group(n, A, lda, B, ldb, C, ldc, P, Q, cs, M, splits, PREC_OF[problems[0][0].dtype], sp()), 'pfn_op_gemm_tn_group')
+
+
+def embed_first_layer(A, P, Z0, Z1, W, deterministic=False):
+    M, w0, w1 = A.shape[0], Z0.shape[1], Z1.shape[1]
+    prec = PREC_OF[A.dtype]
+    lib = _hip.lib()
+    n = _hip.check(lib.pfn_op_embed_first_layer_scratch_floats(prec, M, P, w0, Z0.stride(0), w1, Z1.stride(0), int(deterministic)), 'pfn_op_embed_first_layer_scratch_floats')
+    scratch = torch.empty(n, dtype=torch.float32, device=A.device)
+    G = torch.empty((P + 1, w1), dtype=torch.float32, device=A.device)
+    _hip.check(lib.pfn_op_embed_first_layer(prec, A.data_ptr(), A.stride(0), P, Z0.data_ptr(), Z0.stride(0), w0, Z1.data_ptr(), Z1.stride(0), w1, M,
+                                            W.data_ptr(), W.stride(0), scratch.data_ptr(), n, int(deterministic), G.data_ptr(), sp()), 'pfn_op_embed_first_layer')
+    return scratch[:(P + 1) * (w0 + w1)].view(P + 1, w0 + w1), G
 
 
 SUMS_16BIT = 256
diff --git a/transformerscandobayesianinference_amd/transformer.py b/transformerscandobayesianinference_amd/transformer.py
--- a/transformerscandobayesianinference_amd/transformer.py
+++ b/transformerscandobayesianinference_amd/transformer.py
@@ -147,9 +147,9 @@
                 if dy is not None:
                     dy.zero_()
             else:
-                _hip.check(lib.pfn_stack_input_grads(ctypes.byref(desc), model._flat.data_ptr(), B, S, sep, ws.data_ptr(), ws.numel(),
-                                                     dx.data_ptr(), dx.stride(0), dx.stride(1), _hip.ptr(dy), B, 1, stream),
-                           'pfn_stack_input_grads')
+                _hip.check(lib.pfn_stack_input_grads_shadow(ctypes.byref(desc), model._flat.data_ptr(), shadow.data_ptr(), B, S, sep, ws.data_ptr(), ws.numel(),
+                                                            dx.data_ptr(), dx.stride(0), dx.stride(1), _hip.ptr(dy), B, 1, stream),
+                           'pfn_stack_input_grads_shadow')
         ctx.ws = None
         return (None, None, dx if ctx.needs_input_grad[2] else None, dy, (dsrc if ctx.src_needs_grad else None), None, None, None)
 
```

Result: no change. 2595 datasets/s (median of 6 runs) (+0.6%).
